# yl4579/StyleTTS2

Measured on AMD Instinct MI355X. Metric: audio-seconds/sec (RTF^-1) end-to-end, 10 s utterance batch, higher is better.
Workload: dtype f32 (convs/linears: f16 hi/lo split, 3 MFMA products, fp32 accumulate)

## Files before the change

include/st2.h:

```cpp
#ifndef ST2_H
#define ST2_H

#include <stdint.h>

#ifdef __cplusplus
extern "C" {
#endif

#define ST2_ABI_VERSION 23

int st2_abi_version(void);
const char* st2_last_error(void);
int st2_device_info(int dev, char* name, int cap);

#define ST2_STATUS_F16_RANGE 1
#define ST2_STATUS_LSTM_TIMEOUT 2
#define ST2_STATUS_DURATION_SUM 4
#define ST2_STATUS_LSTM_RECOVERED 8
#define ST2_STATUS_FRAME_CAPACITY 16
int st2_status(int clear);

enum st2_prologue {
  ST2_PRO_NONE = 0,
  ST2_PRO_LEAKY = 1,
  ST2_PRO_ADAIN_LEAKY = 2,
  ST2_PRO_ADAIN_SNAKE = 3,
  ST2_PRO_SNAKE = 4,
  ST2_PRO_COLNORM = 5
};
enum st2_epilogue_act {
  ST2_ACT_NONE = 0,
  ST2_ACT_GELU = 1,
  ST2_ACT_EXP_SIN = 2,
  ST2_ACT_TANH = 3,
  ST2_ACT_LEAKY = 4,
  ST2_ACT_GELU_TANH = 5
};

typedef struct st2_conv_desc {
  int32_t B, C_in, C_out, L_in, L_out, ks, dil, pad_left;
  const float* x; int64_t x_bs; int32_t x_cs;
  const float* wt; int32_t w_ld;
  const float* bias;
  float* y; int64_t y_bs; int32_t y_cs;
  int32_t pro;
  float slope;
  const float* stats;
  const float* gamma; const float* beta;
  int64_t gb_bs; int32_t gamma_plus_one;
  const float* alpha;
  const float* res;  int64_t res_bs;  int32_t res_cs;  int32_t res_shift;
  const float* res2; int64_t res2_bs; int32_t res2_cs;
  float div;
  int32_t act; int32_t act_split; float act_slope;
  const void* wq; int32_t wq_co_pad; int32_t wq_cin_pad;
  float x_scale;
  float out_scale;
  const float* w_row_scale;
  const void* xs; int32_t xs_cg; int32_t xs_lp; int32_t xs_halo;
  float* part; int32_t part_nt;
  int32_t part_cols;
  void* splitk_ws; int64_t splitk_ws_bytes;
  const int32_t* x_len; const int32_t* y_len;
} st2_conv_desc;

int st2_conv1d(const st2_conv_desc* d, void* stream);

int st2_conv1d_f16s(const st2_conv_desc* d, void* stream);
int64_t st2_conv1d_f16s_splitk_bytes(const st2_conv_desc* d);
int st2_conv1d_f16s_chunk(int ks);
int st2_conv1d_f16s_co_block(int C_out);
void st2_conv1d_f16s_set_variant(int variant);
void st2_conv1d_f16s_set_splitk(int max_slices, int min_chunks);
int st2_sizeof_conv_desc(void);

int st2_act_split(const float* x, int64_t x_bs, int32_t x_cs, int32_t B, int32_t C, int32_t L,
                  int32_t pro, float slope, const float* stats, const float* gamma, const float* beta, int64_t gb_bs,
                  int32_t gb_seg, int32_t gamma_plus_one, const float* alpha, float x_scale,
                  void* xs, int32_t xs_cg, int32_t Lp, int32_t halo, void* stream);
int st2_conv1d_xs(const st2_conv_desc* d, void* stream);
int st2_act_split_len(const float* x, int64_t x_bs, int32_t x_cs, int32_t B, int32_t C, int32_t L,
                      int32_t pro, float slope, const float* stats, const float* gamma, const float* beta, int64_t gb_bs,
                      int32_t gb_seg, int32_t gamma_plus_one, const float* alpha, float x_scale,
                      void* xs, int32_t xs_cg, int32_t Lp, int32_t halo, const int32_t* len, void* stream);
int st2_conv1d_xs_part_cols(const st2_conv_desc* d);
int st2_stats_finalize(const float* part, int32_t rows, int32_t nt, int32_t L, float eps, float* stats, int32_t cols, void* stream);
int st2_stats_finalize_len(const float* part, int32_t rows, int32_t nt, int32_t L, float eps, float* stats, int32_t cols,
                           const int32_t* len, int32_t len_div, void* stream);

int st2_conv1d_direct(const float* x, int64_t x_bs, int32_t x_cs,
                      const float* w, const float* bias,
                      float* y, int64_t y_bs, int32_t y_cs,
                      int32_t B, int32_t C_in, int32_t C_out, int32_t L_in, int32_t L_out,
                      int32_t ks, int32_t stride, int32_t pad, void* stream);
int st2_conv1d_direct_len(const float* x, int64_t x_bs, int32_t x_cs, const float* w, const float* bias,
                          float* y, int64_t y_bs, int32_t y_cs, int32_t B, int32_t C_in, int32_t C_out, int32_t L_in,
                          int32_t L_out, int32_t ks, int32_t stride, int32_t pad, const int32_t* x_len,
                          const int32_t* y_len, void* stream);

int st2_phase_split(const float* x, int64_t x_bs, int32_t x_cs, int32_t B, int32_t C, int32_t L_in,
                    int32_t stride, int32_t pad, float* xp, int64_t p_bs, int32_t p_cs, int32_t Lu, void* stream);

int st2_instnorm_stats(const float* x, int64_t x_bs, int32_t x_cs, int32_t B, int32_t C, int32_t L,
                       float eps, float* stats , void* stream);
int st2_instnorm_stats_len(const float* x, int64_t x_bs, int32_t x_cs, int32_t B, int32_t C, int32_t L,
                           float eps, float* stats, const int32_t* len, void* stream);

int st2_colnorm_stats(const float* x, int64_t x_bs, int32_t x_cs, int32_t B, int32_t C, int32_t L,
                      float eps, float* stats , void* stream);

int st2_style_fc(const float* s, int32_t B, int32_t K, const float* wt, const float* bias,
                 int32_t J, int32_t act, float* h, void* stream);

int st2_convt_interleave(const float* phases, int64_t p_bs, int32_t p_cs, int32_t Lq,
                         const float* bias, const float* add, int64_t a_bs, int32_t a_cs,
                         float* out, int64_t o_bs, int32_t o_cs,
                         int32_t B, int32_t C, int32_t stride, int32_t pad, int32_t L_raw,
                         int32_t reflect_left, void* stream);

int st2_convt_interleave_stats(const float* phases, int64_t p_bs, int32_t p_cs, int32_t Lq,
                               const float* bias, const float* add, int64_t a_bs, int32_t a_cs,
                               float* out, int64_t o_bs, int32_t o_cs,
                               int32_t B, int32_t C, int32_t stride, int32_t pad, int32_t L_raw,
                               int32_t reflect_left, float* part, int32_t part_nt, void* stream);
int st2_convt_interleave_stats_len(const float* phases, int64_t p_bs, int32_t p_cs, int32_t Lq,
                                   const float* bias, const float* add, int64_t a_bs, int32_t a_cs,
                                   float* out, int64_t o_bs, int32_t o_cs,
                                   int32_t B, int32_t C, int32_t stride, int32_t pad, int32_t L_raw,
                                   int32_t reflect_left, float* part, int32_t part_nt, const int32_t* q_len,
                                   const int32_t* out_len, void* stream);

int st2_adain_leaky_pool(const float* x, int64_t x_bs, int32_t x_cs,
                         const float* stats, const float* gamma, const float* beta, int64_t gb_bs,
                         float slope, const float* w, const float* bias,
                         float* y, int64_t y_bs, int32_t y_cs,
                         int32_t B, int32_t C, int32_t L, void* stream);
int st2_adain_leaky_pool_len(const float* x, int64_t x_bs, int32_t x_cs,
                             const float* stats, const float* gamma, const float* beta, int64_t gb_bs,
                             float slope, const float* w, const float* bias,
                             float* y, int64_t y_bs, int32_t y_cs,
                             int32_t B, int32_t C, int32_t L, const int32_t* len, void* stream);

int st2_har_source(const float* f0, int32_t B, int32_t F, int32_t U, int32_t H,
                   const float* noise, const float* lin_w, const float* lin_b,
                   float sine_amp, float noise_std, float voiced_threshold, float sample_rate,
                   float* phase_scratch, float* out, void* stream);
int st2_har_source_len(const float* f0, int32_t B, int32_t F, int32_t U, int32_t H,
                       const float* noise, const float* lin_w, const float* lin_b,
                       float sine_amp, float noise_std, float voiced_threshold, float sample_rate,
                       float* phase_scratch, float* out, const int32_t* f_len, void* stream);

int st2_stft_mag_phase(const float* x, int32_t B, int32_t L, int32_t n_fft, int32_t hop,
                       float* har, int64_t har_bs, int32_t har_cs, void* stream);
int st2_stft_mag_phase_len(const float* x, int32_t B, int32_t L, int32_t n_fft, int32_t hop,
                           float* har, int64_t har_bs, int32_t har_cs, const int32_t* len, void* stream);

int st2_istft(const float* sp, int64_t sp_bs, int32_t sp_cs, int32_t B, int32_t M,
              int32_t n_fft, int32_t hop, float* wave, int64_t wave_bs, void* stream);
int st2_istft_len(const float* sp, int64_t sp_bs, int32_t sp_cs, int32_t B, int32_t M,
                  int32_t n_fft, int32_t hop, float* wave, int64_t wave_bs, const int32_t* m_len, void* stream);
int st2_ragged_lengths(const int32_t* frames, int32_t B, int32_t T_max, int32_t n, const int32_t* coef, int32_t* out,
                       void* stream);

int st2_attention(const float* q, const float* k, const float* v, int64_t bs, int32_t cs,
                  float* o, int64_t o_bs, int32_t o_cs,
                  int32_t B, int32_t H, int32_t D, int32_t N, float scale, void* stream);

int st2_attention_keylen(const float* q, const float* k, const float* v, int64_t bs, int32_t cs,
                         float* o, int64_t o_bs, int32_t o_cs,
                         int32_t B, int32_t H, int32_t D, int32_t N, float scale, const int32_t* key_len, void* stream);

int st2_colnorm_apply(const float* x, int64_t x_bs, int32_t x_cs, const float* stats, const float* gamma,
                      const float* beta, int64_t gb_bs, int32_t gamma_plus_one, int32_t act, float slope,
                      const int32_t* len, float* y, int64_t y_bs, int32_t y_cs,
                      int32_t B, int32_t C, int32_t L, void* stream);

int st2_lstm_bidir(const float* G, int64_t g_bs, int32_t g_cs, const float* whh_t, const int32_t* lengths,
                   int32_t B, int32_t H, int32_t N, float* Y, int64_t y_bs, int32_t y_cs, void* stream);

int64_t st2_lstm_coop_scratch_bytes(int32_t B);
int st2_lstm_coop_set_exchange(int mode);
int st2_lstm_coop_set_spin_limit(int polls);
int st2_lstm_coop_set_block(int utterances);
int st2_lstm_bidir_coop(const float* G, int64_t g_bs, int32_t g_cs, const float* whh_t, const int32_t* lengths,
                        int32_t B, int32_t H, int32_t N, float* Y, int64_t y_bs, int32_t y_cs,
                        void* scratch, int64_t scratch_bytes, void* stream);
int st2_lstm_bidir_coop_recovering(const float* G, int64_t g_bs, int32_t g_cs, const float* whh_t, const int32_t* lengths,
                                   int32_t B, int32_t H, int32_t N, float* Y, int64_t y_bs, int32_t y_cs,
                                   void* scratch, int64_t scratch_bytes, void* stream);

int st2_add_chanvec(const float* x, int64_t x_bs, int32_t x_cs, const float* v, int64_t v_bs,
                    float* y, int64_t y_bs, int32_t y_cs, int32_t B, int32_t C, int32_t N, void* stream);
int st2_mean_tokens(const float* x, int64_t x_bs, int32_t x_cs, float* m, int64_t m_bs,
                    int32_t B, int32_t C, int32_t N, void* stream);
int st2_mean_tokens_len(const float* x, int64_t x_bs, int32_t x_cs, float* m, int64_t m_bs,
                        int32_t B, int32_t C, int32_t N, const int32_t* len, void* stream);
int st2_time_features(float t, const float* w, int32_t H2, int32_t B, float* out, void* stream);
int st2_tokens_to_channels(const float* e, int64_t e_bs, int32_t B, int32_t N, int32_t E, float* y, int64_t y_bs,
                           int32_t y_cs, void* stream);
int st2_broadcast_cols(const float* x, int64_t x_bs, float* y, int64_t y_bs, int32_t y_cs, int32_t B, int32_t C,
                       int32_t N, void* stream);
int st2_copy_ncl(const float* x, int64_t x_bs, int32_t x_cs, float* y, int64_t y_bs, int32_t y_cs, int32_t B, int32_t C,
                 int32_t L, void* stream);

int st2_embed_tokens(const int64_t* tokens, int32_t B, int32_t N, const float* table, int32_t V, int32_t E,
                     const float* add, const float* pos, const int32_t* len, float* y, int64_t y_bs, int32_t y_cs,
                     void* stream);
int st2_mask_tail(float* x, int64_t x_bs, int32_t x_cs, int32_t B, int32_t C, int32_t L, const int32_t* len, void* stream);

int st2_duration_head(const float* x, int64_t x_bs, int32_t x_cs, const float* w, const float* bias, int32_t B,
                      int32_t K, int32_t J, int32_t N, const int32_t* len, int32_t tail, int64_t* dur, float* dsum,
                      void* stream);
int st2_expand_by_durations(const float* x, int64_t x_bs, int32_t x_cs, const int64_t* dur, int32_t B, int32_t C,
                            int32_t N, int32_t T, int32_t shift, float* y, int64_t y_bs, int32_t y_cs, void* stream);
int st2_expand_by_durations_len(const float* x, int64_t x_bs, int32_t x_cs, const int64_t* dur, int32_t B, int32_t C,
                                int32_t N, int32_t T, int32_t shift, float* y, int64_t y_bs, int32_t y_cs, const int32_t* len,
                                void* stream);

int st2_frames_from_durations(const int64_t* dur, int32_t B, int32_t N, const int32_t* len, int32_t T_cap, int32_t* frames,
                              void* stream);

enum st2_pack_format { ST2_PACK_F32 = 0, ST2_PACK_S16 = 1 };
int st2_wave_pack(const float* wave, int64_t w_bs, const int32_t* frames, int32_t B, int32_t T_cap,
                  int32_t samples_per_frame, int32_t trim, int32_t fmt, void* out, int64_t out_capacity, int64_t* offsets,
                  void* stream);

int st2_stft_frames(const float* wave, int64_t w_bs, int32_t B, int32_t L, int32_t n_win, int32_t hop, int32_t shift,
                    float* frames, int64_t f_bs, int32_t f_cs, void* stream);
int st2_power_spectrum(const float* y, int64_t y_bs, int32_t y_cs, int32_t B, int32_t K, int32_t M, float* p,
                       int64_t p_bs, int32_t p_cs, void* stream);
int st2_log_norm(float* x, int64_t n, float eps, float mean, float stdv, void* stream);
int st2_dwconv3x3s2(const float* x, int64_t x_bs, int64_t x_hs, int32_t x_cs, const float* w, const float* bias,
                    int32_t B, int32_t C, int32_t H, int32_t W, float* y, int64_t y_bs, int64_t y_hs, int32_t y_cs,
                    void* stream);
int st2_avgpool2x2(const float* x, int64_t x_bs, int64_t x_hs, int32_t x_cs, int32_t B, int32_t C, int32_t H, int32_t W,
                   float* y, int64_t y_bs, int64_t y_hs, int32_t y_cs, void* stream);

int st2_axpbypcz(const float* x, float a, const float* y, float b, const float* z, float c,
                 float* out, int64_t n, void* stream);

typedef struct st2_engine st2_engine;

typedef struct st2_model_config {
  int32_t decoder_kind;
  int32_t dim_in;
  int32_t style_dim;
  int32_t upsample_initial_channel;
  int32_t n_upsamples;  int32_t upsample_rates[4];  int32_t upsample_kernel_sizes[4];
  int32_t n_resblock_kernels;  int32_t resblock_kernel_sizes[4];  int32_t resblock_dilations[4][3];
  int32_t gen_istft_n_fft, gen_istft_hop;
  int32_t multispeaker;
  int32_t dn_layers, dn_heads, dn_head_features, dn_multiplier;
  int32_t dn_channels;
  int32_t dn_embedding;
  int32_t dn_context_features;
  int32_t dn_max_length;
  int32_t pred_hidden;
  int32_t bert_layers;
  float bert_ln_eps;
} st2_model_config;

int st2_create(const st2_model_config* cfg, st2_engine** out);
int st2_destroy(st2_engine* e);
int st2_load_weights(st2_engine* e, const char* name, const float* data, const int64_t* shape, int32_t ndim);
int st2_finalize_weights(st2_engine* e, int32_t which);

typedef struct st2_decoder_taps {
  float* encode;
  float* front;
  float* har_source;
  float* har;
  float* stage[4];
  float* spec_phase;
} st2_decoder_taps;

int64_t st2_decoder_workspace_bytes(st2_engine* e, int32_t B, int32_t T);
int st2_decoder_forward(st2_engine* e, const float* asr, const float* f0, const float* n, const float* s,
                        const float* sine_noise, const float* har_inject, int32_t B, int32_t T, float* wave,
                        void* workspace, int64_t workspace_bytes, const st2_decoder_taps* taps, void* stream);
int st2_decoder_forward_ragged(st2_engine* e, const float* asr, const float* f0, const float* n, const float* s,
                               const float* sine_noise, const float* har_inject, const int32_t* frames, int32_t B,
                               int32_t T_max, float* wave, void* workspace, int64_t workspace_bytes,
                               const st2_decoder_taps* taps, void* stream);

#define ST2_SAMPLER_TABLE_COLS 11
int st2_sampler_table(int32_t steps, double sigma_min, double sigma_max, double rho, double sigma_data, double* table,
                      double* sigma0);
int64_t st2_sampler_workspace_bytes(st2_engine* e, int32_t B, int32_t N, int32_t steps, double embedding_scale);
int st2_sampler_run(st2_engine* e, const float* noise, const float* embedding, const float* features,
                    const float* step_noise, const int32_t* lengths, int32_t B, int32_t N, int32_t steps,
                    double embedding_scale, const double* table, double sigma0, float* out, void* workspace,
                    int64_t workspace_bytes, float* step_taps, void* stream);

int64_t st2_prosody_workspace_bytes(st2_engine* e, int32_t B, int32_t N, int32_t T);
int st2_prosody_forward(st2_engine* e, const float* d_cm, const float* t_en, const int64_t* durations, const float* s,
                        int32_t B, int32_t N, int32_t T, int32_t shift, float* asr, float* f0, float* n, void* workspace,
                        int64_t workspace_bytes, void* stream);
int st2_prosody_forward_ragged(st2_engine* e, const float* d_cm, const float* t_en, const int64_t* durations,
                               const float* s, const int32_t* frames, int32_t B, int32_t N, int32_t T_max, int32_t shift,
                               float* asr, float* f0, float* n, void* workspace, int64_t workspace_bytes, void* stream);

int64_t st2_text_workspace_bytes(st2_engine* e, int32_t B, int32_t N);
int st2_text_forward(st2_engine* e, const int64_t* tokens, const int32_t* lengths, int32_t B, int32_t N, float* t_en,
                     void* workspace, int64_t workspace_bytes, void* stream);

int64_t st2_duration_workspace_bytes(st2_engine* e, int32_t B, int32_t N);
int st2_duration_forward(st2_engine* e, const float* d_en, const float* s, const int32_t* lengths, int32_t B, int32_t N,
                         int32_t tail, float* d_cm, int64_t* durations, void* workspace, int64_t workspace_bytes,
                         void* stream);

int64_t st2_bert_workspace_bytes(st2_engine* e, int32_t B, int32_t N);
int st2_bert_forward(st2_engine* e, const int64_t* tokens, const int32_t* lengths, int32_t B, int32_t N, float* hidden_cm,
                     void* workspace, int64_t workspace_bytes, void* stream);

typedef struct st2_front_args {
  const int64_t* tokens;
  const int32_t* lengths;
  const float* noise;
  const float* step_noise;
  const float* ref_s;
  const float* s_prev;
  int32_t B, N, steps;
  int32_t tail;
  double embedding_scale;
  const double* table;
  double sigma0;
  double alpha, beta, t;
  float* t_en;
  float* d_cm;
  float* s;
  float* ref;
  float* s_pred_out;
  int64_t* durations;
  int32_t carry;
} st2_front_args;
int st2_sizeof_front_args(void);
int64_t st2_front_workspace_bytes(st2_engine* e, const st2_front_args* a);
int st2_front_forward(st2_engine* e, const st2_front_args* a, void* workspace, int64_t workspace_bytes, void* stream);

int64_t st2_style_workspace_bytes(st2_engine* e, int32_t which, int32_t B, int32_t n_mels, int32_t T);
int st2_style_forward(st2_engine* e, int32_t which, const float* mel, int32_t B, int32_t n_mels, int32_t T, float* style,
                      void* workspace, int64_t workspace_bytes, void* stream);

int st2_conv_timing(int enable);
int st2_conv_timing_read(double* rows, int32_t cap_rows);

int st2_conv_tune(int mode);
int st2_conv_tune_set(int32_t ks, int32_t C_in, int32_t C_out, int32_t L_out, int32_t B, int32_t variant);
int st2_conv_tune_read(double* rows, int32_t cap_rows);

#define ST2_HEADROOM_COLS 12
int st2_debug_headroom(int enable);
int st2_debug_headroom_read(double* rows, int32_t cap_rows);

#define ST2_CALIBRATION_COLS 5
int st2_calibrate(st2_engine* e, int32_t margin_bits, int32_t* n_clamped);
int st2_calibration_read(st2_engine* e, double* rows, int32_t cap_rows);
int st2_calibration_site_name(st2_engine* e, int32_t site, char* name, int32_t cap);
int st2_calibration_write(st2_engine* e, const float* scales, int32_t n);
float st2_calibration_scale(float max_abs, int32_t margin_bits);

int st2_probe_box(char* json, int32_t cap, int32_t level);

int st2_probe_cu_health(char* json, int32_t cap, uint32_t* mask_out, int32_t mask_words, int32_t* n_excluded);

int st2_probe_mfma_stream(int32_t kind, int32_t workgroups, int32_t iters, void* stream);

int st2_stream_create_cu_mask(const uint32_t* mask, int32_t n_words, void** stream);
int st2_stream_destroy(void* stream);

enum st2_backend_slot {
  ST2_BE_CONV1D_F16S = 0, ST2_BE_CONV1D_XS, ST2_BE_ACT_SPLIT, ST2_BE_STATS_FINALIZE, ST2_BE_CONV1D_DIRECT,
  ST2_BE_PHASE_SPLIT, ST2_BE_INSTNORM_STATS, ST2_BE_COLNORM_STATS, ST2_BE_STYLE_FC, ST2_BE_CONVT_INTERLEAVE_STATS,
  ST2_BE_ADAIN_LEAKY_POOL, ST2_BE_HAR_SOURCE, ST2_BE_STFT_MAG_PHASE, ST2_BE_ISTFT, ST2_BE_ATTENTION_KEYLEN,
  ST2_BE_ADD_CHANVEC, ST2_BE_MEAN_TOKENS_LEN, ST2_BE_AXPBYPCZ, ST2_BE_TIME_FEATURES, ST2_BE_TOKENS_TO_CHANNELS,
  ST2_BE_BROADCAST_COLS, ST2_BE_COPY_NCL, ST2_BE_EXPAND_BY_DURATIONS,
  ST2_BE_LSTM_BIDIR,
  ST2_BE_COLNORM_APPLY, ST2_BE_DURATION_HEAD, ST2_BE_MASK_TAIL, ST2_BE_EMBED_TOKENS, ST2_BE_DWCONV3X3S2, ST2_BE_AVGPOOL2X2,
  ST2_BE_DEV_ALLOC,
  ST2_BE_DEV_FREE,
  ST2_BE_UPLOAD,
  ST2_BACKEND_ENTRIES_V22,
  ST2_BE_ACT_SPLIT_LEN = ST2_BACKEND_ENTRIES_V22, ST2_BE_INSTNORM_STATS_LEN, ST2_BE_STATS_FINALIZE_LEN,
  ST2_BE_CONV1D_DIRECT_LEN, ST2_BE_ADAIN_LEAKY_POOL_LEN, ST2_BE_CONVT_INTERLEAVE_STATS_LEN, ST2_BE_HAR_SOURCE_LEN,
  ST2_BE_STFT_MAG_PHASE_LEN, ST2_BE_ISTFT_LEN, ST2_BE_RAGGED_LENGTHS, ST2_BE_EXPAND_BY_DURATIONS_LEN,
  ST2_BACKEND_ENTRIES
};
// ... 7 lines not shown
```

styletts2_amd/_lib.py:

```python
import ctypes as C
import os

import torch

_HERE = os.path.dirname(os.path.abspath(__file__))
LIB_PATH = os.path.join(_HERE, "libst2_hip.so")
ABI_VERSION = 23
HEADROOM_COLS, CALIBRATION_COLS = 12, 5

f32p = C.c_void_p

PRO_NONE, PRO_LEAKY, PRO_ADAIN_LEAKY, PRO_ADAIN_SNAKE, PRO_SNAKE, PRO_COLNORM = range(6)
STATUS_F16_RANGE, STATUS_LSTM_TIMEOUT, STATUS_DURATION_SUM, STATUS_LSTM_RECOVERED = 1, 2, 4, 8
STATUS_FRAME_CAPACITY = 16
PACK_F32, PACK_S16 = 0, 1
ACT_NONE, ACT_GELU, ACT_EXP_SIN, ACT_TANH, ACT_LEAKY, ACT_GELU_TANH = range(6)


class ConvDesc(C.Structure):
    _fields_ = [
        ("B", C.c_int32), ("C_in", C.c_int32), ("C_out", C.c_int32), ("L_in", C.c_int32),
        ("L_out", C.c_int32), ("ks", C.c_int32), ("dil", C.c_int32), ("pad_left", C.c_int32),
        ("x", f32p), ("x_bs", C.c_int64), ("x_cs", C.c_int32),
        ("wt", f32p), ("w_ld", C.c_int32),
        ("bias", f32p),
        ("y", f32p), ("y_bs", C.c_int64), ("y_cs", C.c_int32),
        ("pro", C.c_int32),
        ("slope", C.c_float),
        ("stats", f32p),
        ("gamma", f32p), ("beta", f32p),
        ("gb_bs", C.c_int64), ("gamma_plus_one", C.c_int32),
        ("alpha", f32p),
        ("res", f32p), ("res_bs", C.c_int64), ("res_cs", C.c_int32), ("res_shift", C.c_int32),
        ("res2", f32p), ("res2_bs", C.c_int64), ("res2_cs", C.c_int32),
        ("div", C.c_float),
        ("act", C.c_int32), ("act_split", C.c_int32), ("act_slope", C.c_float),
        ("wq", f32p), ("wq_co_pad", C.c_int32), ("wq_cin_pad", C.c_int32),
        ("x_scale", C.c_float), ("out_scale", C.c_float),
        ("w_row_scale", f32p),
        ("xs", f32p), ("xs_cg", C.c_int32), ("xs_lp", C.c_int32), ("xs_halo", C.c_int32),
        ("part", f32p), ("part_nt", C.c_int32), ("part_cols", C.c_int32),
        ("splitk_ws", f32p), ("splitk_ws_bytes", C.c_int64),
        ("x_len", C.c_void_p), ("y_len", C.c_void_p),
    ]


class ModelConfig(C.Structure):
    _fields_ = [
        ("decoder_kind", C.c_int32), ("dim_in", C.c_int32), ("style_dim", C.c_int32),
        ("upsample_initial_channel", C.c_int32),
        ("n_upsamples", C.c_int32), ("upsample_rates", C.c_int32 * 4), ("upsample_kernel_sizes", C.c_int32 * 4),
        ("n_resblock_kernels", C.c_int32), ("resblock_kernel_sizes", C.c_int32 * 4),
        ("resblock_dilations", (C.c_int32 * 3) * 4),
        ("gen_istft_n_fft", C.c_int32), ("gen_istft_hop", C.c_int32),
        ("multispeaker", C.c_int32),
        ("dn_layers", C.c_int32), ("dn_heads", C.c_int32), ("dn_head_features", C.c_int32),
        ("dn_multiplier", C.c_int32), ("dn_channels", C.c_int32), ("dn_embedding", C.c_int32),
        ("dn_context_features", C.c_int32), ("dn_max_length", C.c_int32),
        ("pred_hidden", C.c_int32),
        ("bert_layers", C.c_int32), ("bert_ln_eps", C.c_float),
    ]


class FrontArgs(C.Structure):
    _fields_ = [("tokens", C.c_void_p), ("lengths", C.c_void_p), ("noise", C.c_void_p), ("step_noise", C.c_void_p),
                ("ref_s", C.c_void_p), ("s_prev", C.c_void_p),
                ("B", C.c_int32), ("N", C.c_int32), ("steps", C.c_int32), ("tail", C.c_int32),
                ("embedding_scale", C.c_double), ("table", C.POINTER(C.c_double)), ("sigma0", C.c_double),
                ("alpha", C.c_double), ("beta", C.c_double), ("t", C.c_double),
                ("t_en", C.c_void_p), ("d_cm", C.c_void_p), ("s", C.c_void_p), ("ref", C.c_void_p),
                ("s_pred_out", C.c_void_p), ("durations", C.c_void_p), ("carry", C.c_int32)]


class DecoderTaps(C.Structure):
    _fields_ = [("encode", f32p), ("front", f32p), ("har_source", f32p), ("har", f32p), ("stage", f32p * 4),
                ("spec_phase", f32p)]


SAMPLER_TABLE_COLS = 11
BACKEND_SLOTS = ["conv1d_f16s", "conv1d_xs", "act_split", "stats_finalize", "conv1d_direct", "phase_split",
                 "instnorm_stats", "colnorm_stats", "style_fc", "convt_interleave_stats", "adain_leaky_pool",
                 "har_source", "stft_mag_phase", "istft", "attention_keylen", "add_chanvec", "mean_tokens_len",
                 "axpbypcz", "time_features", "tokens_to_channels", "broadcast_cols", "copy_ncl", "expand_by_durations",
                 "lstm_bidir", "colnorm_apply", "duration_head", "mask_tail", "embed_tokens", "dwconv3x3s2",
                 "avgpool2x2", "dev_alloc", "dev_free", "upload"]
BACKEND_SLOTS_RAGGED = ["act_split_len", "instnorm_stats_len", "stats_finalize_len", "conv1d_direct_len",
                        "adain_leaky_pool_len", "convt_interleave_stats_len", "har_source_len", "stft_mag_phase_len",
                        "istft_len", "ragged_lengths", "expand_by_durations_len"]

_SIGNATURES = {
    "st2_abi_version": (C.c_int, []),
    "st2_last_error": (C.c_char_p, []),
    "st2_device_info": (C.c_int, [C.c_int, C.c_char_p, C.c_int]),
    "st2_sizeof_conv_desc": (C.c_int, []),
    "st2_status": (C.c_int, [C.c_int]),
    "st2_conv1d": (C.c_int, [C.POINTER(ConvDesc), C.c_void_p]),
    "st2_conv1d_f16s": (C.c_int, [C.POINTER(ConvDesc), C.c_void_p]),
    "st2_conv1d_f16s_splitk_bytes": (C.c_int64, [C.POINTER(ConvDesc)]),
    "st2_conv1d_f16s_chunk": (C.c_int, [C.c_int]),
    "st2_conv1d_f16s_co_block": (C.c_int, [C.c_int]),
    "st2_conv1d_f16s_set_variant": (None, [C.c_int]),
    "st2_conv1d_xs": (C.c_int, [C.POINTER(ConvDesc), C.c_void_p]),
    "st2_act_split": (C.c_int, [f32p, C.c_int64, C.c_int32, C.c_int32, C.c_int32, C.c_int32, C.c_int32, C.c_float,
                                f32p, f32p, f32p, C.c_int64, C.c_int32, C.c_int32, f32p, C.c_float, f32p, C.c_int32,
                                C.c_int32, C.c_int32, C.c_void_p]),
    "st2_stats_finalize": (C.c_int, [f32p, C.c_int32, C.c_int32, C.c_int32, C.c_float, f32p, C.c_int32, C.c_void_p]),
    "st2_conv1d_direct": (C.c_int, [f32p, C.c_int64, C.c_int32, f32p, f32p, f32p, C.c_int64, C.c_int32,
                                    C.c_int32, C.c_int32, C.c_int32, C.c_int32, C.c_int32, C.c_int32, C.c_int32,
                                    C.c_int32, C.c_void_p]),
    "st2_phase_split": (C.c_int, [f32p, C.c_int64, C.c_int32, C.c_int32, C.c_int32, C.c_int32, C.c_int32, C.c_int32,
                                  f32p, C.c_int64, C.c_int32, C.c_int32, C.c_void_p]),
    "st2_instnorm_stats": (C.c_int, [f32p, C.c_int64, C.c_int32, C.c_int32, C.c_int32, C.c_int32, C.c_float, f32p,
                                     C.c_void_p]),
    "st2_colnorm_stats": (C.c_int, [f32p, C.c_int64, C.c_int32, C.c_int32, C.c_int32, C.c_int32, C.c_float, f32p,
                                    C.c_void_p]),
    "st2_style_fc": (C.c_int, [f32p, C.c_int32, C.c_int32, f32p, f32p, C.c_int32, C.c_int32, f32p, C.c_void_p]),
    "st2_convt_interleave": (C.c_int, [f32p, C.c_int64, C.c_int32, C.c_int32, f32p, f32p, C.c_int64, C.c_int32,
                                       f32p, C.c_int64, C.c_int32, C.c_int32, C.c_int32, C.c_int32, C.c_int32,
                                       C.c_int32, C.c_int32, C.c_void_p]),
    "st2_convt_interleave_stats": (C.c_int, [f32p, C.c_int64, C.c_int32, C.c_int32, f32p, f32p, C.c_int64, C.c_int32,
                                             f32p, C.c_int64, C.c_int32, C.c_int32, C.c_int32, C.c_int32, C.c_int32,
                                             C.c_int32, C.c_int32, f32p, C.c_int32, C.c_void_p]),
    "st2_adain_leaky_pool": (C.c_int, [f32p, C.c_int64, C.c_int32, f32p, f32p, f32p, C.c_int64, C.c_float, f32p,
                                       f32p, f32p, C.c_int64, C.c_int32, C.c_int32, C.c_int32, C.c_int32,
                                       C.c_void_p]),
    "st2_har_source": (C.c_int, [f32p, C.c_int32, C.c_int32, C.c_int32, C.c_int32, f32p, f32p, f32p, C.c_float,
                                 C.c_float, C.c_float, C.c_float, f32p, f32p, C.c_void_p]),
    "st2_stft_mag_phase": (C.c_int, [f32p, C.c_int32, C.c_int32, C.c_int32, C.c_int32, f32p, C.c_int64, C.c_int32,
                                     C.c_void_p]),
    "st2_istft": (C.c_int, [f32p, C.c_int64, C.c_int32, C.c_int32, C.c_int32, C.c_int32, C.c_int32, f32p, C.c_int64,
                            C.c_void_p]),
    "st2_attention": (C.c_int, [f32p, f32p, f32p, C.c_int64, C.c_int32, f32p, C.c_int64, C.c_int32, C.c_int32,
                                C.c_int32, C.c_int32, C.c_int32, C.c_float, C.c_void_p]),
    "st2_attention_keylen": (C.c_int, [f32p, f32p, f32p, C.c_int64, C.c_int32, f32p, C.c_int64, C.c_int32, C.c_int32,
                                       C.c_int32, C.c_int32, C.c_int32, C.c_float, C.c_void_p, C.c_void_p]),
    "st2_colnorm_apply": (C.c_int, [f32p, C.c_int64, C.c_int32, f32p, f32p, f32p, C.c_int64, C.c_int32, C.c_int32,
                                    C.c_float, C.c_void_p, f32p, C.c_int64, C.c_int32, C.c_int32, C.c_int32, C.c_int32,
                                    C.c_void_p]),
    "st2_lstm_bidir": (C.c_int, [f32p, C.c_int64, C.c_int32, f32p, C.c_void_p, C.c_int32, C.c_int32, C.c_int32, f32p,
                                 C.c_int64, C.c_int32, C.c_void_p]),
    "st2_lstm_coop_scratch_bytes": (C.c_int64, [C.c_int32]),
    "st2_lstm_coop_set_exchange": (C.c_int, [C.c_int]),
    "st2_lstm_coop_set_spin_limit": (C.c_int, [C.c_int]),
    "st2_lstm_coop_set_block": (C.c_int, [C.c_int]),
    "st2_lstm_bidir_coop": (C.c_int, [f32p, C.c_int64, C.c_int32, f32p, C.c_void_p, C.c_int32, C.c_int32, C.c_int32,
                                      f32p, C.c_int64, C.c_int32, C.c_void_p, C.c_int64, C.c_void_p]),
    "st2_lstm_bidir_coop_recovering": (C.c_int, [f32p, C.c_int64, C.c_int32, f32p, C.c_void_p, C.c_int32, C.c_int32, C.c_int32,
                                                 f32p, C.c_int64, C.c_int32, C.c_void_p, C.c_int64, C.c_void_p]),
    "st2_add_chanvec": (C.c_int, [f32p, C.c_int64, C.c_int32, f32p, C.c_int64, f32p, C.c_int64, C.c_int32,
                                  C.c_int32, C.c_int32, C.c_int32, C.c_void_p]),
    "st2_mean_tokens": (C.c_int, [f32p, C.c_int64, C.c_int32, f32p, C.c_int64, C.c_int32, C.c_int32, C.c_int32,
                                  C.c_void_p]),
    "st2_mean_tokens_len": (C.c_int, [f32p, C.c_int64, C.c_int32, f32p, C.c_int64, C.c_int32, C.c_int32, C.c_int32,
                                      C.c_void_p, C.c_void_p]),
    "st2_time_features": (C.c_int, [C.c_float, f32p, C.c_int32, C.c_int32, f32p, C.c_void_p]),
    "st2_tokens_to_channels": (C.c_int, [f32p, C.c_int64, C.c_int32, C.c_int32, C.c_int32, f32p, C.c_int64, C.c_int32,
                                         C.c_void_p]),
    "st2_broadcast_cols": (C.c_int, [f32p, C.c_int64, f32p, C.c_int64, C.c_int32, C.c_int32, C.c_int32, C.c_int32,
                                     C.c_void_p]),
    "st2_copy_ncl": (C.c_int, [f32p, C.c_int64, C.c_int32, f32p, C.c_int64, C.c_int32, C.c_int32, C.c_int32, C.c_int32,
                               C.c_void_p]),
    "st2_duration_head": (C.c_int, [f32p, C.c_int64, C.c_int32, f32p, f32p, C.c_int32, C.c_int32, C.c_int32, C.c_int32,
                                    C.c_void_p, C.c_int32, C.c_void_p, f32p, C.c_void_p]),
    "st2_expand_by_durations": (C.c_int, [f32p, C.c_int64, C.c_int32, C.c_void_p, C.c_int32, C.c_int32, C.c_int32,
                                          C.c_int32, C.c_int32, f32p, C.c_int64, C.c_int32, C.c_void_p]),
    "st2_create": (C.c_int, [C.POINTER(ModelConfig), C.POINTER(C.c_void_p)]),
    "st2_destroy": (C.c_int, [C.c_void_p]),
    "st2_load_weights": (C.c_int, [C.c_void_p, C.c_char_p, C.c_void_p, C.POINTER(C.c_int64), C.c_int32]),
    "st2_finalize_weights": (C.c_int, [C.c_void_p, C.c_int32]),
    "st2_decoder_workspace_bytes": (C.c_int64, [C.c_void_p, C.c_int32, C.c_int32]),
    "st2_decoder_forward": (C.c_int, [C.c_void_p, f32p, f32p, f32p, f32p, f32p, f32p, C.c_int32, C.c_int32, f32p,
                                      C.c_void_p, C.c_int64, C.POINTER(DecoderTaps), C.c_void_p]),
    "st2_embed_tokens": (C.c_int, [C.c_void_p, C.c_int32, C.c_int32, f32p, C.c_int32, C.c_int32, f32p, f32p, C.c_void_p, f32p,
                                   C.c_int64, C.c_int32, C.c_void_p]),
    "st2_bert_workspace_bytes": (C.c_int64, [C.c_void_p, C.c_int32, C.c_int32]),
    "st2_bert_forward": (C.c_int, [C.c_void_p, C.c_void_p, C.c_void_p, C.c_int32, C.c_int32, f32p, C.c_void_p, C.c_int64,
                                   C.c_void_p]),
    "st2_style_workspace_bytes": (C.c_int64, [C.c_void_p, C.c_int32, C.c_int32, C.c_int32, C.c_int32]),
    "st2_style_forward": (C.c_int, [C.c_void_p, C.c_int32, f32p, C.c_int32, C.c_int32, C.c_int32, f32p, C.c_void_p, C.c_int64,
                                    C.c_void_p]),
    "st2_sizeof_front_args": (C.c_int, []),
    "st2_front_workspace_bytes": (C.c_int64, [C.c_void_p, C.POINTER(FrontArgs)]),
    "st2_front_forward": (C.c_int, [C.c_void_p, C.POINTER(FrontArgs), C.c_void_p, C.c_int64, C.c_void_p]),
    "st2_text_workspace_bytes": (C.c_int64, [C.c_void_p, C.c_int32, C.c_int32]),
    "st2_text_forward": (C.c_int, [C.c_void_p, C.c_void_p, C.c_void_p, C.c_int32, C.c_int32, f32p, C.c_void_p, C.c_int64,
                                   C.c_void_p]),
    "st2_mask_tail": (C.c_int, [f32p, C.c_int64, C.c_int32, C.c_int32, C.c_int32, C.c_int32, C.c_void_p, C.c_void_p]),
    "st2_duration_workspace_bytes": (C.c_int64, [C.c_void_p, C.c_int32, C.c_int32]),
    "st2_duration_forward": (C.c_int, [C.c_void_p, f32p, f32p, C.c_void_p, C.c_int32, C.c_int32, C.c_int32, f32p,
                                       C.c_void_p, C.c_void_p, C.c_int64, C.c_void_p]),
    "st2_decoder_forward_ragged": (C.c_int, [C.c_void_p, f32p, f32p, f32p, f32p, f32p, f32p, C.c_void_p, C.c_int32,
                                             C.c_int32, f32p, C.c_void_p, C.c_int64, C.c_void_p, C.c_void_p]),
    "st2_prosody_forward_ragged": (C.c_int, [C.c_void_p, f32p, f32p, C.c_void_p, f32p, C.c_void_p, C.c_int32, C.c_int32,
                                             C.c_int32, C.c_int32, f32p, f32p, f32p, C.c_void_p, C.c_int64, C.c_void_p]),
    "st2_act_split_len": (C.c_int, [f32p, C.c_int64, C.c_int32, C.c_int32, C.c_int32, C.c_int32, C.c_int32, C.c_float,
                                    f32p, f32p, f32p, C.c_int64, C.c_int32, C.c_int32, f32p, C.c_float, f32p, C.c_int32,
                                    C.c_int32, C.c_int32, C.c_void_p, C.c_void_p]),
    "st2_stats_finalize_len": (C.c_int, [f32p, C.c_int32, C.c_int32, C.c_int32, C.c_float, f32p, C.c_int32, C.c_void_p,
                                         C.c_int32, C.c_void_p]),
    "st2_instnorm_stats_len": (C.c_int, [f32p, C.c_int64, C.c_int32, C.c_int32, C.c_int32, C.c_int32, C.c_float, f32p,
                                         C.c_void_p, C.c_void_p]),
    "st2_conv1d_direct_len": (C.c_int, [f32p, C.c_int64, C.c_int32, f32p, f32p, f32p, C.c_int64, C.c_int32, C.c_int32,
                                        C.c_int32, C.c_int32, C.c_int32, C.c_int32, C.c_int32, C.c_int32, C.c_int32,
                                        C.c_void_p, C.c_void_p, C.c_void_p]),
    "st2_convt_interleave_stats_len": (C.c_int, [f32p, C.c_int64, C.c_int32, C.c_int32, f32p, f32p, C.c_int64, C.c_int32,
                                                 f32p, C.c_int64, C.c_int32, C.c_int32, C.c_int32, C.c_int32, C.c_int32,
                                                 C.c_int32, C.c_int32, f32p, C.c_int32, C.c_void_p, C.c_void_p,
                                                 C.c_void_p]),
    "st2_adain_leaky_pool_len": (C.c_int, [f32p, C.c_int64, C.c_int32, f32p, f32p, f32p, C.c_int64, C.c_float, f32p,
                                           f32p, f32p, C.c_int64, C.c_int32, C.c_int32, C.c_int32, C.c_int32, C.c_void_p,
                                           C.c_void_p]),
    "st2_har_source_len": (C.c_int, [f32p, C.c_int32, C.c_int32, C.c_int32, C.c_int32, f32p, f32p, f32p, C.c_float,
                                     C.c_float, C.c_float, C.c_float, f32p, f32p, C.c_void_p, C.c_void_p]),
    "st2_stft_mag_phase_len": (C.c_int, [f32p, C.c_int32, C.c_int32, C.c_int32, C.c_int32, f32p, C.c_int64, C.c_int32,
                                         C.c_void_p, C.c_void_p]),
    "st2_istft_len": (C.c_int, [f32p, C.c_int64, C.c_int32, C.c_int32, C.c_int32, C.c_int32, C.c_int32, f32p, C.c_int64,
                                C.c_void_p, C.c_void_p]),
    "st2_expand_by_durations_len": (C.c_int, [f32p, C.c_int64, C.c_int32, C.c_void_p, C.c_int32, C.c_int32, C.c_int32,
                                              C.c_int32, C.c_int32, f32p, C.c_int64, C.c_int32, C.c_void_p, C.c_void_p]),
    "st2_ragged_lengths": (C.c_int, [C.c_void_p, C.c_int32, C.c_int32, C.c_int32, C.POINTER(C.c_int32), C.c_void_p,
                                     C.c_void_p]),
    "st2_frames_from_durations": (C.c_int, [C.c_void_p, C.c_int32, C.c_int32, C.c_void_p, C.c_int32, C.c_void_p, C.c_void_p]),
    "st2_wave_pack": (C.c_int, [f32p, C.c_int64, C.c_void_p, C.c_int32, C.c_int32, C.c_int32, C.c_int32, C.c_int32, C.c_void_p,
                                C.c_int64, C.c_void_p, C.c_void_p]),
    "st2_prosody_workspace_bytes": (C.c_int64, [C.c_void_p, C.c_int32, C.c_int32, C.c_int32]),
    "st2_prosody_forward": (C.c_int, [C.c_void_p, f32p, f32p, C.c_void_p, f32p, C.c_int32, C.c_int32, C.c_int32, C.c_int32,
                                      f32p, f32p, f32p, C.c_void_p, C.c_int64, C.c_void_p]),
    "st2_sampler_table": (C.c_int, [C.c_int32, C.c_double, C.c_double, C.c_double, C.c_double, C.POINTER(C.c_double),
                                    C.POINTER(C.c_double)]),
    "st2_sampler_workspace_bytes": (C.c_int64, [C.c_void_p, C.c_int32, C.c_int32, C.c_int32, C.c_double]),
    "st2_sampler_run": (C.c_int, [C.c_void_p, f32p, f32p, f32p, f32p, C.c_void_p, C.c_int32, C.c_int32, C.c_int32,
                                  C.c_double, C.POINTER(C.c_double), C.c_double, f32p, C.c_void_p, C.c_int64, f32p,
                                  C.c_void_p]),
    "st2_conv_timing": (C.c_int, [C.c_int]),
    "st2_conv_timing_read": (C.c_int, [C.POINTER(C.c_double), C.c_int32]),
    "st2_conv_tune": (C.c_int, [C.c_int]),
    "st2_conv_tune_set": (C.c_int, [C.c_int32, C.c_int32, C.c_int32, C.c_int32, C.c_int32, C.c_int32]),
    "st2_conv_tune_read": (C.c_int, [C.POINTER(C.c_double), C.c_int32]),
    "st2_probe_box": (C.c_int, [C.c_char_p, C.c_int32, C.c_int32]),
    "st2_probe_cu_health": (C.c_int, [C.c_char_p, C.c_int32, C.POINTER(C.c_uint32), C.c_int32, C.POINTER(C.c_int32)]),
    "st2_probe_mfma_stream": (C.c_int, [C.c_int32, C.c_int32, C.c_int32, C.c_void_p]),
    "st2_debug_headroom": (C.c_int, [C.c_int]),
    "st2_debug_headroom_read": (C.c_int, [C.POINTER(C.c_double), C.c_int32]),
    "st2_conv1d_xs_part_cols": (C.c_int, [C.POINTER(ConvDesc)]),
    "st2_conv1d_f16s_set_splitk": (None, [C.c_int, C.c_int]),
    "st2_calibrate": (C.c_int, [C.c_void_p, C.c_int32, C.POINTER(C.c_int32)]),
    "st2_calibration_read": (C.c_int, [C.c_void_p, C.POINTER(C.c_double), C.c_int32]),
    "st2_calibration_site_name": (C.c_int, [C.c_void_p, C.c_int32, C.c_char_p, C.c_int32]),
    "st2_calibration_write": (C.c_int, [C.c_void_p, C.POINTER(C.c_float), C.c_int32]),
    "st2_calibration_scale": (C.c_float, [C.c_float, C.c_int32]),
    "st2_stream_create_cu_mask": (C.c_int, [C.POINTER(C.c_uint32), C.c_int32, C.POINTER(C.c_void_p)]),
    "st2_stream_destroy": (C.c_int, [C.c_void_p]),
    "st2_debug_set_backend": (C.c_int, [C.POINTER(C.c_void_p), C.c_int32]),
    "st2_stft_frames": (C.c_int, [f32p, C.c_int64, C.c_int32, C.c_int32, C.c_int32, C.c_int32, C.c_int32, f32p,
                                  C.c_int64, C.c_int32, C.c_void_p]),
    "st2_power_spectrum": (C.c_int, [f32p, C.c_int64, C.c_int32, C.c_int32, C.c_int32, C.c_int32, f32p, C.c_int64,
                                     C.c_int32, C.c_void_p]),
    "st2_log_norm": (C.c_int, [f32p, C.c_int64, C.c_float, C.c_float, C.c_float, C.c_void_p]),
    "st2_dwconv3x3s2": (C.c_int, [f32p, C.c_int64, C.c_int64, C.c_int32, f32p, f32p, C.c_int32, C.c_int32, C.c_int32,
                                  C.c_int32, f32p, C.c_int64, C.c_int64, C.c_int32, C.c_void_p]),
    "st2_avgpool2x2": (C.c_int, [f32p, C.c_int64, C.c_int64, C.c_int32, C.c_int32, C.c_int32, C.c_int32, C.c_int32, f32p,
                                 C.c_int64, C.c_int64, C.c_int32, C.c_void_p]),
    "st2_axpbypcz": (C.c_int, [f32p, C.c_float, f32p, C.c_float, f32p, C.c_float, f32p, C.c_int64, C.c_void_p]),
}

EXPORTS = tuple(_SIGNATURES)
_lib = None


class St2Error(RuntimeError):
    pass


def load():
    global _lib
    if _lib is not None:
        return _lib
    if not os.path.exists(LIB_PATH):
        raise St2Error("libst2_hip.so is not built (%s missing). Run `python -m styletts2_amd._build`; "
                       "there is no CPU fallback." % LIB_PATH)
    try:
        lib = C.CDLL(LIB_PATH)
    except OSError as e:
        raise St2Error("cannot load %s: %s" % (LIB_PATH, e)) from e
    for name, (res, args) in _SIGNATURES.items():
        try:
            fn = getattr(lib, name)
        except AttributeError as e:
            raise St2Error("libst2_hip.so does not export %s" % name) from e
        fn.restype = res
        fn.argtypes = args
    if lib.st2_abi_version() != ABI_VERSION:
        raise St2Error("ABI mismatch: library %d, binding %d" % (lib.st2_abi_version(), ABI_VERSION))
    if lib.st2_sizeof_conv_desc() != C.sizeof(ConvDesc):
        raise St2Error("st2_conv_desc layout mismatch: library %d B, binding %d B"
                       % (lib.st2_sizeof_conv_desc(), C.sizeof(ConvDesc)))
    if lib.st2_sizeof_front_args() != C.sizeof(FrontArgs):
        raise St2Error("st2_front_args layout mismatch: library %d B, binding %d B"
                       % (lib.st2_sizeof_front_args(), C.sizeof(FrontArgs)))
    _lib = lib
    return lib


def check(status, what):
    if status != 0:
        msg = load().st2_last_error()
        raise St2Error("%s failed: %s" % (what, msg.decode() if msg else "unknown error"))
```

styletts2_amd/csrc/st2_actsplit.hip:

```cpp
#include "st2_common.h"
#include "st2_act.h"
#include <algorithm>
#include <cstring>
#include <type_traits>
#include <vector>

namespace {

struct ActArgs {
  const float* x; int64_t x_bs; int x_cs;
  int C, L;
  float slope;
  const float* stats; const float* gamma; const float* beta; int64_t gb_bs; int gb_seg; int gamma_plus_one;
  const float* alpha;
  float x_scale;
  st2_h8* xs; int xs_cg, Lp, halo;
  const int32_t* len;
  int* status;
};

#ifndef ST2_ACT_NT
#define ST2_ACT_NT 3
#endif
template <int PRO>
__global__ __launch_bounds__(256) void act_split_kernel(const ActArgs a) {
  const int pos = blockIdx.x * 256 + threadIdx.x;
  if (pos >= a.Lp) return;
  const int cg = blockIdx.y;
  const int b = blockIdx.z;
  const int l = pos - a.halo;
  const int Lb = a.len ? min(a.len[b], a.L) : a.L;
  const bool lok = l >= 0 && l < Lb;
  const int lc = min(max(l, 0), a.L - 1);
  const float* xb = a.x + (int64_t)b * a.x_bs + lc;
  float v[8];
#pragma unroll
  for (int e = 0; e < 8; ++e) {
    const int ci = min(cg * 8 + e, a.C - 1);
#if ST2_ACT_NT & 1
    v[e] = __builtin_nontemporal_load(&xb[(int64_t)ci * a.x_cs]);
#else
    v[e] = xb[(int64_t)ci * a.x_cs];
#endif
  }
  float cmean = 0.f, crstd = 1.f;
  if constexpr (PRO == ST2_PRO_COLNORM) {
    const float* st = a.stats + ((int64_t)b * a.L + lc) * 2;
    cmean = st[0];
    crstd = st[1];
  }
  st2_h8 hi, lo;
  bool sat = false;
#pragma unroll
  for (int e = 0; e < 8; ++e) {
    const int ci = cg * 8 + e;
    const int cc = min(ci, a.C - 1);
    float u = v[e];
    if constexpr (PRO == ST2_PRO_LEAKY) {
      u = leaky(u, a.slope);
    } else if constexpr (PRO == ST2_PRO_ADAIN_LEAKY || PRO == ST2_PRO_ADAIN_SNAKE) {
      const float* st = a.stats + ((int64_t)b * a.C + cc) * 2;
      const float g = 1.0f + a.gamma[(int64_t)b * a.gb_bs + cc];
      const float bt = a.beta[(int64_t)b * a.gb_bs + cc];
      float w = (u - st[0]) * st[1];
      w = g * w + bt;
      if constexpr (PRO == ST2_PRO_ADAIN_LEAKY) {
        u = leaky(w, a.slope);
      } else {
        const float al = a.alpha[cc];
        u = snake(w, al, 1.0f / al);
      }
    } else if constexpr (PRO == ST2_PRO_SNAKE) {
      const float al = a.alpha[cc];
      u = snake(u, al, 1.0f / al);
    } else if constexpr (PRO == ST2_PRO_COLNORM) {
      const int64_t row = a.gb_seg > 0 ? (int64_t)(lc / a.gb_seg) : (int64_t)b;
      const float g0 = a.gamma[row * a.gb_bs + cc];
      const float g = a.gamma_plus_one ? 1.0f + g0 : g0;
      const float bt = a.beta[row * a.gb_bs + cc];
      const float w = (u - cmean) * crstd;
      u = w * g + bt;
    }
    u = (lok && ci < a.C) ? u * a.x_scale : 0.f;
    const float uc = st2_clamp_f16(u);
    sat |= uc != u;
    const _Float16 h = (_Float16)uc;
    hi[e] = h;
    lo[e] = (_Float16)(uc - (float)h);
  }
  if (__any(sat) && (threadIdx.x & 63) == 0) st2_raise_status(a.status, ST2_STATUS_F16_RANGE);
  const int64_t plane = (int64_t)a.xs_cg * a.Lp;
  st2_h8* dst = a.xs + ((int64_t)b * 2 * a.xs_cg + cg) * a.Lp + pos;
#if ST2_ACT_NT & 2
  __builtin_nontemporal_store(hi, &dst[0]);
  __builtin_nontemporal_store(lo, &dst[plane]);
#else
  dst[0] = hi;
  dst[plane] = lo;
#endif
}

__global__ __launch_bounds__(256) void stats_finalize_kernel(const float* __restrict__ part, int rows, int nt, int L_max,
                                                             float eps, float* __restrict__ stats, int cols,
                                                             const int32_t* __restrict__ len, int len_div) {
  const int lane = threadIdx.x & 63;
  const int row = blockIdx.x * 4 + (threadIdx.x >> 6);
  if (row >= rows) return;
  const int L = len ? min(max(len[row / len_div], 1), L_max) : L_max;
  const float2* p = reinterpret_cast<const float2*>(part) + (int64_t)row * nt;
  const float* sh = part + (int64_t)rows * nt * 2 + (int64_t)row * nt;
  const int ns = min(nt, (L + cols - 1) / cols);
  double wsum = 0.0;
  for (int i = lane; i < ns; i += 64) {
    const int n = min(cols, L - i * cols);
    wsum += (double)n * (double)sh[i] + (double)p[i].x;
  }
  wsum = st2_wave_sum(wsum);
  const double mean = __shfl(wsum, 0, 64) / (double)L;
  double m2 = 0.0;
  for (int i = lane; i < ns; i += 64) {
    const int n = min(cols, L - i * cols);
    const double s1 = (double)p[i].x, s2 = (double)p[i].y;
    const double mi = (double)sh[i] + s1 / (double)n;
    m2 += (s2 - s1 * s1 / (double)n) + (double)n * (mi - mean) * (mi - mean);
  }
  m2 = st2_wave_sum(m2);
  if (lane == 0) {
    double var = m2 / (double)L;
    if (var < 0.0) var = 0.0;
    stats[(int64_t)row * 2 + 0] = (float)mean;
    stats[(int64_t)row * 2 + 1] = (float)(1.0 / sqrt(var + (double)eps));
  }
}

struct HeadroomSums {
  unsigned max_bits, pad;
  double su2, se2, ssub;
};
__global__ __launch_bounds__(256) void xs_probe_kernel(const st2_h8* __restrict__ xs, int64_t slots_per_item, int64_t item_stride,
                                                       HeadroomSums* out) {
  const st2_h8* hi_p = xs + (int64_t)blockIdx.y * item_stride;
  const st2_h8* lo_p = hi_p + slots_per_item;
  float m = 0.f;
  double su2 = 0.0, se2 = 0.0, ssub = 0.0;
  for (int64_t i = (int64_t)blockIdx.x * 256 + threadIdx.x; i < slots_per_item; i += (int64_t)gridDim.x * 256) {
    const st2_h8 h = hi_p[i], l = lo_p[i];
#pragma unroll
    for (int e = 0; e < 8; ++e) {
      const float hf = (float)h[e], lf = (float)l[e];
      m = fmaxf(m, fabsf(hf));
      if (hf == 0.f && lf == 0.f) continue;
      const float u = hf + lf;
      const float al = fabsf(lf);
      const bool sub = al < 6.103515625e-05f;
      int ex = -14;
      if (!sub) {
        (void)frexpf(al, &ex);
        ex -= 1;
      }
      const float ulp = ldexpf(1.0f, ex - 10);
      su2 += (double)u * u;
      se2 += (double)ulp * ulp * (1.0 / 12.0);
      if (sub) ssub += (double)u * u;
    }
  }
  for (int off = 32; off > 0; off >>= 1) m = fmaxf(m, __shfl_down(m, off, 64));
  su2 = st2_wave_sum(su2);
  se2 = st2_wave_sum(se2);
  ssub = st2_wave_sum(ssub);
  if ((threadIdx.x & 63) == 0) {
    atomicMax(&out->max_bits, __float_as_uint(m));
    atomicAdd(&out->su2, su2);
    atomicAdd(&out->se2, se2);
    atomicAdd(&out->ssub, ssub);
  }
}

struct HeadroomRecord {
  int kind, pro, B, C, L;
  float x_scale;
  const void* engine;
  int site;
};
bool g_headroom = false;
std::vector<HeadroomRecord> g_hr;
HeadroomSums* g_hr_dev = nullptr;
constexpr int HR_CAP = 4096;
void* g_hr_scratch = nullptr;
size_t g_hr_scratch_bytes = 0;
thread_local const void* t_site_engine = nullptr;
thread_local int t_site = -1;

void headroom_record(int kind, const ActArgs& a, int B, hipStream_t s) {
  if ((int)g_hr.size() >= HR_CAP || !g_hr_dev) return;
  hipStreamCaptureStatus cs = hipStreamCaptureStatusNone;
  if (hipStreamIsCapturing(s, &cs) != hipSuccess || cs != hipStreamCaptureStatusNone) {
    (void)hipGetLastError();
    return;
  }
  const int64_t plane = (int64_t)a.xs_cg * a.Lp;
  hipLaunchKernelGGL(xs_probe_kernel, dim3((unsigned)std::min<int64_t>((plane + 255) / 256, 1024), B), dim3(256), 0, s, a.xs, plane,
                     2 * plane, g_hr_dev + g_hr.size());
  g_hr.push_back({kind, 0, B, a.C, a.L, a.x_scale, t_site_engine, t_site});
}

template <int PRO>
void launch_act(const ActArgs& a, int B, hipStream_t s) {
  hipLaunchKernelGGL((act_split_kernel<PRO>), dim3(st2_cdiv(a.Lp, 256), a.xs_cg, B), dim3(256), 0, s, a);
}

}

extern "C" int st2_act_split(const float* x, int64_t x_bs, int32_t x_cs, int32_t B, int32_t C, int32_t L, int32_t pro,
                             float slope, const float* stats, const float* gamma, const float* beta, int64_t gb_bs,
                             int32_t gb_seg, int32_t gamma_plus_one, const float* alpha, float x_scale, void* xs, int32_t xs_cg,
                             int32_t Lp, int32_t halo, void* stream) {
  return st2_act_split_len(x, x_bs, x_cs, B, C, L, pro, slope, stats, gamma, beta, gb_bs, gb_seg, gamma_plus_one, alpha, x_scale,
                           xs, xs_cg, Lp, halo, nullptr, stream);
}

extern "C" int st2_act_split_len(const float* x, int64_t x_bs, int32_t x_cs, int32_t B, int32_t C, int32_t L, int32_t pro,
                                 float slope, const float* stats, const float* gamma, const float* beta, int64_t gb_bs,
                                 int32_t gb_seg, int32_t gamma_plus_one, const float* alpha, float x_scale, void* xs,
                                 int32_t xs_cg, int32_t Lp, int32_t halo, const int32_t* len, void* stream) {
  ST2_REQUIRE(x && xs && B > 0 && C > 0 && L > 0, "st2_act_split: bad arguments");
  ST2_REQUIRE(B <= 65535 && xs_cg <= 65535, "st2_act_split: grid too large");
  ST2_REQUIRE(xs_cg * 8 >= C, "st2_act_split: xs_cg=%d groups cannot hold C=%d channels", xs_cg, C);
  ST2_REQUIRE(halo >= 0 && Lp >= L + halo, "st2_act_split: Lp=%d too small for L=%d + halo=%d", Lp, L, halo);
  ST2_REQUIRE((reinterpret_cast<uintptr_t>(xs) & 15) == 0, "st2_act_split: xs must be 16-byte aligned");
  ST2_REQUIRE(pro >= ST2_PRO_NONE && pro <= ST2_PRO_COLNORM, "st2_act_split: prologue %d not supported", pro);
  if (pro == ST2_PRO_ADAIN_LEAKY || pro == ST2_PRO_ADAIN_SNAKE || pro == ST2_PRO_COLNORM)
    ST2_REQUIRE(stats && gamma && beta, "st2_act_split: prologue %d needs stats/gamma/beta", pro);
  if (pro == ST2_PRO_ADAIN_SNAKE || pro == ST2_PRO_SNAKE) ST2_REQUIRE(alpha, "st2_act_split: snake needs alpha");
  ST2_REQUIRE(x_scale > 0.f, "st2_act_split: x_scale must be set");
  ST2_REQUIRE(gb_seg >= 0 && (gb_seg == 0 || pro == ST2_PRO_COLNORM), "st2_act_split: gb_seg=%d is for ST2_PRO_COLNORM", gb_seg);
  ActArgs a;
  a.x = x; a.x_bs = x_bs; a.x_cs = x_cs; a.C = C; a.L = L; a.slope = slope;
  a.stats = stats; a.gamma = gamma; a.beta = beta; a.gb_bs = gb_bs; a.gb_seg = gb_seg; a.gamma_plus_one = gamma_plus_one;
  a.alpha = alpha; a.x_scale = x_scale;
  a.xs = reinterpret_cast<st2_h8*>(xs); a.xs_cg = xs_cg; a.Lp = Lp; a.halo = halo;
  a.len = len;
  ST2_REQUIRE(!len || pro != ST2_PRO_COLNORM, "st2_act_split_len: per-row lengths are not defined for ST2_PRO_COLNORM");
  a.status = st2_status_device_ptr();
  hipStream_t s = reinterpret_cast<hipStream_t>(stream);
  switch (pro) {
    case ST2_PRO_LEAKY: launch_act<ST2_PRO_LEAKY>(a, B, s); break;
    case ST2_PRO_ADAIN_LEAKY: launch_act<ST2_PRO_ADAIN_LEAKY>(a, B, s); break;
    case ST2_PRO_ADAIN_SNAKE: launch_act<ST2_PRO_ADAIN_SNAKE>(a, B, s); break;
    case ST2_PRO_SNAKE: launch_act<ST2_PRO_SNAKE>(a, B, s); break;
    case ST2_PRO_COLNORM: launch_act<ST2_PRO_COLNORM>(a, B, s); break;
    default: launch_act<ST2_PRO_NONE>(a, B, s); break;
  }
  ST2_CHECK_LAUNCH("st2_act_split");
  if (g_headroom) {
    headroom_record(0, a, B, s);
    if (!g_hr.empty()) g_hr.back().pro = pro;
  }
  return 0;
}

int st2_headroom_of_fused_conv(const st2_conv_desc& d, hipStream_t s) {
  if (!g_headroom || !d.x) return 0;
  {
    hipStreamCaptureStatus cs = hipStreamCaptureStatusNone;
    if (hipStreamIsCapturing(s, &cs) != hipSuccess || cs != hipStreamCaptureStatusNone) {
      (void)hipGetLastError();
      return 0;
    }
  }
  const int cg = (d.C_in + 31) / 32 * 4, halo = 0;
  const int Lp = (d.L_in + 7) / 8 * 8;
  const size_t bytes = (size_t)d.B * 2 * cg * Lp * 16;
  if (bytes > g_hr_scratch_bytes) {
    if (g_hr_scratch) (void)hipFree(g_hr_scratch);
    g_hr_scratch = nullptr;
    g_hr_scratch_bytes = 0;
    if (hipMalloc(&g_hr_scratch, bytes) != hipSuccess) {
      (void)hipGetLastError();
      return 0;
    }
    g_hr_scratch_bytes = bytes;
  }
  const size_t before = g_hr.size();
  const int rc = st2_act_split(d.x, d.x_bs, d.x_cs, d.B, d.C_in, d.L_in, d.pro, d.slope, d.stats, d.gamma, d.beta, d.gb_bs, 0,
                               d.gamma_plus_one, d.alpha, d.x_scale, g_hr_scratch, cg, Lp, halo, s);
  if (rc == 0 && g_hr.size() == before + 1) g_hr.back().kind = 1;
  return rc;
}

extern "C" int st2_debug_headroom(int enable) {
  if (enable) {
    g_hr.clear();
    if (!g_hr_dev && hipMalloc(&g_hr_dev, HR_CAP * sizeof(HeadroomSums)) != hipSuccess) {
      (void)hipGetLastError();
      g_hr_dev = nullptr;
      st2_set_error("st2_debug_headroom: cannot allocate the record buffer");
      return 1;
    }
    if (hipMemset(g_hr_dev, 0, HR_CAP * sizeof(HeadroomSums)) != hipSuccess) {
      st2_set_error("st2_debug_headroom: %s", hipGetErrorString(hipGetLastError()));
      return 1;
    }
  } else if (g_hr_scratch) {
    (void)hipDeviceSynchronize();
    (void)hipFree(g_hr_scratch);
    g_hr_scratch = nullptr;
    g_hr_scratch_bytes = 0;
  }
  g_headroom = enable != 0;
  return 0;
}

void st2_headroom_set_site(const void* engine, int site) {
  t_site_engine = engine;
  t_site = site;
}

extern "C" int st2_debug_headroom_read(double* rows, int32_t cap_rows) {
  ST2_REQUIRE(!g_headroom, "st2_debug_headroom_read: stop the recording first (st2_debug_headroom(0))");
  const int n = (int)g_hr.size();
  if (!rows || n == 0) return n;
  std::vector<HeadroomSums> h(n);
  if (hipDeviceSynchronize() != hipSuccess ||
      hipMemcpy(h.data(), g_hr_dev, n * sizeof(HeadroomSums), hipMemcpyDeviceToHost) != hipSuccess) {
    st2_set_error("st2_debug_headroom_read: %s", hipGetErrorString(hipGetLastError()));
    return -1;
  }
  for (int i = 0; i < n && i < cap_rows; ++i) {
    float m;
    memcpy(&m, &h[i].max_bits, 4);
    double* r = rows + (int64_t)i * ST2_HEADROOM_COLS;
    r[0] = g_hr[i].kind; r[1] = g_hr[i].pro; r[2] = g_hr[i].B; r[3] = g_hr[i].C; r[4] = g_hr[i].L; r[5] = g_hr[i].x_scale;
    r[6] = m; r[7] = m / 65504.0;
    r[8] = h[i].su2 > 0.0 ? sqrt(h[i].se2 / h[i].su2) : 0.0;
    r[9] = h[i].su2 > 0.0 ? h[i].ssub / h[i].su2 : 0.0;
    r[10] = g_hr[i].site;
    r[11] = (double)(uintptr_t)g_hr[i].engine;
  }
  return n;
}

extern "C" int st2_stats_finalize(const float* part, int32_t rows, int32_t nt, int32_t L, float eps, float* stats, int32_t cols,
                                  void* stream) {
  return st2_stats_finalize_len(part, rows, nt, L, eps, stats, cols, nullptr, 1, stream);
}

extern "C" int st2_stats_finalize_len(const float* part, int32_t rows, int32_t nt, int32_t L, float eps, float* stats,
                                      int32_t cols, const int32_t* len, int32_t len_div, void* stream) {
  ST2_REQUIRE(part && stats && rows > 0 && nt > 0 && L > 0, "st2_stats_finalize: bad arguments");
  ST2_REQUIRE(!len || (len_div > 0 && rows % len_div == 0), "st2_stats_finalize_len: len_div=%d does not divide rows=%d", len_div,
              rows);
  ST2_REQUIRE(cols > 0 && (int64_t)nt * cols >= L, "st2_stats_finalize: %d slots of %d columns do not cover L=%d", nt, cols, L);
  ST2_REQUIRE((reinterpret_cast<uintptr_t>(part) & 7) == 0, "st2_stats_finalize: part must be 8-byte aligned");
  hipStream_t s = reinterpret_cast<hipStream_t>(stream);
  hipLaunchKernelGGL(stats_finalize_kernel, dim3(st2_cdiv(rows, 4)), dim3(256), 0, s, part, rows, nt, L, eps, stats, cols, len,
                     len_div);
  ST2_CHECK_LAUNCH("st2_stats_finalize");
  return 0;
}
```

styletts2_amd/csrc/st2_common.h:

```cpp
#pragma once
#include <hip/hip_runtime.h>
#include <stdint.h>
#include <atomic>
#include "st2.h"

void st2_set_error(const char* fmt, ...);
int st2_stream_cu_count(void* stream);
void st2_headroom_set_site(const void* engine, int site);
int* st2_status_device_ptr();

__device__ __forceinline__ void st2_raise_status(int* status, int bit) {
  if (status) __hip_atomic_store(status + (bit == ST2_STATUS_F16_RANGE ? 0 : (bit == ST2_STATUS_LSTM_TIMEOUT ? 1 :
                                           (bit == ST2_STATUS_DURATION_SUM ? 2 :
                                            (bit == ST2_STATUS_LSTM_RECOVERED ? 3 : 4)))), bit,
                                 __ATOMIC_RELAXED, __HIP_MEMORY_SCOPE_SYSTEM);
}

#define ST2_REQUIRE(cond, ...)            \
  do {                                    \
    if (!(cond)) {                        \
      st2_set_error(__VA_ARGS__);         \
      return 1;                           \
    }                                     \
  } while (0)

#define ST2_CHECK_LAUNCH(name)                                   \
  do {                                                           \
    hipError_t e__ = hipGetLastError();                          \
    if (e__ != hipSuccess) {                                     \
      st2_set_error("%s: %s", name, hipGetErrorString(e__));     \
      return 1;                                                  \
    }                                                            \
  } while (0)

static inline int st2_cdiv(int64_t a, int64_t b) { return (int)((a + b - 1) / b); }

template <class F>
static inline void st2_once_per_device(std::atomic<uint64_t>& mask, F&& set_attr) {
  int dev = 0;
  const bool known = hipGetDevice(&dev) == hipSuccess && dev >= 0 && dev < 64;
  if (known && (mask.load(std::memory_order_acquire) & (1ull << dev))) return;
  set_attr();
  if (known) mask.fetch_or(1ull << dev, std::memory_order_release);
}

__device__ __forceinline__ double st2_wave_sum(double v) {
#pragma unroll
  for (int off = 32; off > 0; off >>= 1) v += __shfl_down(v, off, 64);
  return v;
}
__device__ __forceinline__ float st2_wave_sum(float v) {
#pragma unroll
  for (int off = 32; off > 0; off >>= 1) v += __shfl_down(v, off, 64);
  return v;
}
```

styletts2_amd/csrc/st2_engine.hip:

```cpp
#include <math.h>
#include <stdio.h>
#include <string.h>

#include <algorithm>
#include <cmath>
#include <string>
#include <unordered_map>
#include <vector>

#include "st2_common.h"

namespace {

struct Backend {
  decltype(&st2_conv1d_f16s) conv1d_f16s;
  decltype(&st2_conv1d_xs) conv1d_xs;
  decltype(&st2_act_split) act_split;
  decltype(&st2_stats_finalize) stats_finalize;
  decltype(&st2_conv1d_direct) conv1d_direct;
  decltype(&st2_phase_split) phase_split;
  decltype(&st2_instnorm_stats) instnorm_stats;
  decltype(&st2_colnorm_stats) colnorm_stats;
  decltype(&st2_style_fc) style_fc;
  decltype(&st2_convt_interleave_stats) convt_interleave_stats;
// ... 431 lines not shown
      return -1;
    }
    return blob.add_f32(t->data);
  }
  int64_t lin_t(const std::string& name, int64_t out = -1, int64_t in = -1) {
    const HostTensor* t = get(name, {out, in});
    if (!t) return -1;
    if (t->shape.size() != 2) { fail(name + " (2-D expected)"); return -1; }
    const int64_t O = t->shape[0], I = t->shape[1];
    std::vector<float> v((size_t)(O * I));
    for (int64_t o = 0; o < O; ++o)
      for (int64_t i = 0; i < I; ++i) v[(size_t)(i * O + o)] = t->data[(size_t)(o * I + i)];
    return blob.add_f32(v);
  }
  SplitW conv_w(const std::string& name, int co = -1, int ci = -1, int ks = -1) {
    const HostTensor* t = get(name, {co, ci, ks});
    if (!t) return SplitW();
    if (t->shape.size() < 2) { fail(name + " has shape " + shape_str(t->shape) + ", a conv / linear weight is at least 2-D"); return SplitW(); }
    const int C_out = (int)t->shape[0], C_in = (int)t->shape[1], k = t->shape.size() > 2 ? (int)t->shape[2] : 1;
    return pack_split(blob, name, t->data.data(), C_out, C_in, k);
  }
  PConv conv(const std::string& prefix, bool bias = true, int co = -1, int ci = -1, int ks = -1) {
    PConv c;
    c.w = conv_w(prefix + ".weight", co, ci, ks);
    c.c_out = c.w.C_out;
    c.ks = c.w.ks;
    if (bias && has(prefix + ".bias")) c.bias = vec(prefix + ".bias", c.w.C_out > 0 ? c.w.C_out : -1);
    return c;
  }
};

struct Bank {
  std::vector<const HostTensor*> ws, bs;
  std::vector<int> chans;
  std::vector<std::string> names;
  int J = 0;
  int add(Packer& pk, const std::string& prefix, int channels) {
    names.push_back(prefix + ".fc.weight");
    ws.push_back(pk.get(prefix + ".fc.weight"));
    bs.push_back(pk.get(prefix + ".fc.bias"));
    chans.push_back(channels);
    const int off = J;
    J += 2 * channels;
    return off;
  }
  void pack(Packer& pk, int style_dim, int64_t* wt_off, int64_t* b_off) {
    std::vector<float> wt((size_t)style_dim * J), b((size_t)J);
    int off = 0;
    for (size_t m = 0; m < ws.size(); ++m) {
      const int n = 2 * chans[m];
      if (!ws[m] || !bs[m]) return;
      if (ws[m]->numel() != (int64_t)n * style_dim || bs[m]->numel() != n) {
        pk.fail("AdaIN fc " + names[m] + " has shape " + Packer::shape_str(ws[m]->shape) + " / bias " + Packer::shape_str(bs[m]->shape) +
                ", the model configuration needs [" + std::to_string(n) + ", " + std::to_string(style_dim) + "]");
        return;
      }
      for (int j = 0; j < n; ++j) {
        for (int k = 0; k < style_dim; ++k) wt[(size_t)k * J + off + j] = ws[m]->data[(size_t)j * style_dim + k];
        b[(size_t)off + j] = bs[m]->data[(size_t)j];
      }
      off += n;
    }
    *wt_off = pk.blob.add_f32(wt);
    *b_off = pk.blob.add_f32(b);
  }
};

PResBlock1 pack_resblock1(Packer& pk, const std::string& prefix, int channels, int ks, const int* dil) {
  PResBlock1 r;
  r.channels = channels;
  r.ks = ks;
  for (int i = 0; i < 3; ++i) {
    const std::string si = std::to_string(i);
    r.dil[i] = dil[i];
    r.c1[i] = pk.conv(prefix + ".convs1." + si, true, channels, channels, ks);
    r.c2[i] = pk.conv(prefix + ".convs2." + si, true, channels, channels, ks);
    r.a1[i] = pk.vec(prefix + ".alpha1." + si, channels);
    r.a2[i] = pk.vec(prefix + ".alpha2." + si, channels);
  }
  return r;
}

PAdainResBlk pack_adain_resblk(Packer& pk, const std::string& prefix, int dim_in, int dim_out, bool upsample) {
  PAdainResBlk r;
  r.dim_in = dim_in; r.dim_out = dim_out; r.upsample = upsample; r.learned_sc = dim_in != dim_out;
  r.conv1 = pk.conv(prefix + ".conv1", true, dim_out, dim_in, 3);
  r.conv2 = pk.conv(prefix + ".conv2", true, dim_out, dim_out, 3);
  if (r.learned_sc) r.sc = pk.conv(prefix + ".conv1x1", false, dim_out, dim_in, 1);
  if (upsample) {
    r.pool_w = pk.vec(prefix + ".pool.weight", (int64_t)dim_in * 3);
    r.pool_b = pk.vec(prefix + ".pool.bias", dim_in);
  }
  return r;
}

int prod_from(const int32_t* v, int lo, int hi) {
  int p = 1;
  for (int i = lo; i < hi; ++i) p *= v[i];
  return p;
}

int pack_decoder(st2_engine& e, Blob& blob, std::string* err) {
  const st2_model_config& cfg = e.cfg;
  Packer pk{e, blob};
  PDecoder d;
  Bank bank;
  const std::string D = "decoder.";
  const int sty = cfg.style_dim, Cin = cfg.dim_in;
  d.encode = pack_adain_resblk(pk, D + "encode", Cin + 2, 1024, false);
  d.encode.n1 = bank.add(pk, D + "encode.norm1", Cin + 2);
  d.encode.n2 = bank.add(pk, D + "encode.norm2", 1024);
  for (int i = 0; i < 4; ++i) {
    const std::string p = D + "decode." + std::to_string(i);
    const bool up = i == 3;
    d.decode[i] = pack_adain_resblk(pk, p, 1024 + 2 + 64, up ? 512 : 1024, up);
    d.decode[i].n1 = bank.add(pk, p + ".norm1", 1024 + 2 + 64);
    d.decode[i].n2 = bank.add(pk, p + ".norm2", up ? 512 : 1024);
  }
  d.f0_w = pk.vec(D + "F0_conv.weight", 3); d.f0_b = pk.vec(D + "F0_conv.bias", 1);
  d.n_w = pk.vec(D + "N_conv.weight", 3);   d.n_b = pk.vec(D + "N_conv.bias", 1);
  d.asr_res = pk.conv(D + "asr_res.0", true, 64, Cin, 1);

  PGenerator& g = d.gen;
  const std::string G = D + "generator.";
  const int nu = cfg.n_upsamples, nk = cfg.n_resblock_kernels;
  const bool ist = cfg.decoder_kind == 0;
  const int c0 = cfg.upsample_initial_channel;
  g.lin_w = pk.vec(G + "m_source.l_linear.weight", 9);
  g.lin_b = pk.vec(G + "m_source.l_linear.bias", 1);
  static const int dil135[3] = {1, 3, 5};
  for (int i = 0; i < nu; ++i) g.channels.push_back(c0 >> (i + 1));
  for (int i = 0; i < nu; ++i) {
    const bool last = i + 1 == nu;
    PResBlock1 r = pack_resblock1(pk, G + "noise_res." + std::to_string(i), g.channels[i], last ? 11 : 7, dil135);
    g.noise_res.push_back(r);
  }
  for (int i = 0; i < nu; ++i)
    for (int k = 0; k < nk; ++k) {
      PResBlock1 r = pack_resblock1(pk, G + "resblocks." + std::to_string(i * nk + k), g.channels[i],
                                    cfg.resblock_kernel_sizes[k], cfg.resblock_dilations[k]);
      g.resblocks.push_back(r);
    }
  for (auto* list : {&g.noise_res, &g.resblocks}) {
    const std::string pre = list == &g.noise_res ? G + "noise_res." : G + "resblocks.";
    for (size_t i = 0; i < list->size(); ++i) {
      PResBlock1& r = (*list)[i];
      for (int j = 0; j < 3; ++j) r.ad1[j] = bank.add(pk, pre + std::to_string(i) + ".adain1." + std::to_string(j), r.channels);
      for (int j = 0; j < 3; ++j) r.ad2[j] = bank.add(pk, pre + std::to_string(i) + ".adain2." + std::to_string(j), r.channels);
    }
  }
  if (pk.ok) bank.pack(pk, sty, &d.bank_wt, &d.bank_b);
  d.J = bank.J;
  for (int i = 0; i < nu; ++i) {
    const int stride_f0 = i + 1 < nu ? prod_from(cfg.upsample_rates, i + 1, nu) : 1;
    const HostTensor* w = pk.get(G + "noise_convs." + std::to_string(i) + ".weight", {g.channels[i], -1, -1});
    g.noise_stride.push_back(stride_f0);
    if (w && w->shape.size() != 3) { pk.fail(G + "noise_convs." + std::to_string(i) + ".weight must be 3-D"); w = nullptr; }
    if (w) {
      const int C_out = (int)w->shape[0], C_in = (int)w->shape[1], K = (int)w->shape[2];
      if (stride_f0 > 1) {
        if (K != 2 * stride_f0) { *err = "noise_convs kernel must be 2*stride"; return 1; }
        std::vector<float> wp = polyphase_strided(w->data.data(), C_out, C_in, stride_f0);
        g.noise_wt.push_back(pack_split(blob, G + "noise_convs." + std::to_string(i) + ".weight", wp.data(), C_out, C_in * stride_f0, 2));
      } else {
        g.noise_wt.push_back(pack_split(blob, G + "noise_convs." + std::to_string(i) + ".weight", w->data.data(), C_out, C_in, K));
      }
    } else {
      g.noise_wt.push_back(SplitW());
    }
    g.noise_b.push_back(pk.vec(G + "noise_convs." + std::to_string(i) + ".bias", g.channels[i]));
  }
  for (int i = 0; i < nu; ++i) {
    const int u = cfg.upsample_rates[i];
    const HostTensor* w = pk.get(G + "ups." + std::to_string(i) + ".weight", {c0 >> i, c0 >> (i + 1), -1});
    if (w && w->shape.size() != 3) { pk.fail(G + "ups." + std::to_string(i) + ".weight must be 3-D"); w = nullptr; }
    if (w) {
      const int C_in = (int)w->shape[0], C_out = (int)w->shape[1], K = (int)w->shape[2];
      if (K != 2 * u) { *err = "ups kernel must be 2*stride"; return 1; }
      std::vector<float> wp = polyphase_convt(w->data.data(), C_in, C_out, u);
      g.ups_wt.push_back(pack_split(blob, G + "ups." + std::to_string(i) + ".weight", wp.data(), u * C_out, C_in, 2));
    } else {
      g.ups_wt.push_back(SplitW());
    }
    g.ups_b.push_back(pk.vec(G + "ups." + std::to_string(i) + ".bias", c0 >> (i + 1)));
  }
  g.post = pk.conv(G + "conv_post", true, ist ? cfg.gen_istft_n_fft + 2 : 1, g.channels.back(), 7);
  if (!ist)
    for (int i = 0; i <= nu; ++i) g.alphas.push_back(pk.vec(G + "alphas." + std::to_string(i), c0 >> i));
  if (!pk.ok) {
    *err = "decoder weights (missing or malformed): " + pk.missing;
    return 1;
  }
  d.ready = true;
  e.dec = d;
  return 0;
}

int pack_denoiser(st2_engine& e, Blob& blob, std::string* err) {
  const st2_model_config& cfg = e.cfg;
  Packer pk{e, blob};
  PDenoiser d;
  const std::string N = "denoiser.";
  d.features = cfg.dn_channels + cfg.dn_embedding;
  d.time_w = pk.vec(N + "to_time.0.0.weights");
  d.time_lin = pk.lin_t(N + "to_time.0.1.weight"); d.time_b = pk.vec(N + "to_time.0.1.bias");
  d.map0 = pk.lin_t(N + "to_mapping.0.weight");    d.map0_b = pk.vec(N + "to_mapping.0.bias");
  d.map2 = pk.lin_t(N + "to_mapping.2.weight");    d.map2_b = pk.vec(N + "to_mapping.2.bias");
  const int F = d.features;
  if (cfg.multispeaker) {
    d.feat = pk.lin_t(N + "to_features.0.weight"); d.feat_b = pk.vec(N + "to_features.0.bias");
    const int Fc = cfg.dn_context_features, J = cfg.dn_layers * 4 * F;
    std::vector<float> wt((size_t)Fc * J), b((size_t)J);
    int off = 0;
    for (int i = 0; i < cfg.dn_layers; ++i)
      for (const char* nm : {".attention.norm", ".attention.norm_context"}) {
        const HostTensor* w = pk.get(N + "blocks." + std::to_string(i) + nm + ".fc.weight", {2 * F, Fc});
        const HostTensor* bb = pk.get(N + "blocks." + std::to_string(i) + nm + ".fc.bias", {2 * F});
        if (w && bb)
          for (int j = 0; j < 2 * F; ++j) {
            for (int k = 0; k < Fc; ++k) wt[(size_t)k * J + off + j] = w->data[(size_t)j * Fc + k];
            b[(size_t)off + j] = bb->data[(size_t)j];
          }
        off += 2 * F;
      }
    d.ada_wt = blob.add_f32(wt);
    d.ada_b = blob.add_f32(b);
  }
  for (int i = 0; i < cfg.dn_layers; ++i) {
    const std::string B = N + "blocks." + std::to_string(i);
    PBlock b;
    if (!cfg.multispeaker) {
      b.n_w = pk.vec(B + ".attention.norm.weight", F);          b.n_b = pk.vec(B + ".attention.norm.bias", F);
      b.nc_w = pk.vec(B + ".attention.norm_context.weight", F); b.nc_b = pk.vec(B + ".attention.norm_context.bias", F);
    }
    const int HD = cfg.dn_heads * cfg.dn_head_features, FM = F * cfg.dn_multiplier;
    b.q = pk.conv_w(B + ".attention.to_q.weight", HD, F, 1);
    b.kv = pk.conv_w(B + ".attention.to_kv.weight", 2 * HD, F, 1);
    b.o = pk.conv_w(B + ".attention.attention.to_out.weight", F, HD, 1); b.o_b = pk.vec(B + ".attention.attention.to_out.bias", F);
    b.f1 = pk.conv_w(B + ".feed_forward.0.weight", FM, F, 1);            b.f1_b = pk.vec(B + ".feed_forward.0.bias", FM);
    b.f1_out = b.f1.C_out;
    b.f2 = pk.conv_w(B + ".feed_forward.2.weight", F, FM, 1);            b.f2_b = pk.vec(B + ".feed_forward.2.bias", F);
    d.blocks.push_back(b);
  }
  {
    const HostTensor* w = pk.get(N + "to_out.1.weight", {cfg.dn_channels, F, 1});
    if (w) {
      const int O = (int)w->shape[0], I = (int)w->shape[1];
      std::vector<float> v((size_t)O * I);
      for (int o = 0; o < O; ++o)
        for (int i = 0; i < I; ++i) v[(size_t)i * O + o] = w->data[(size_t)o * I + i];
      d.out_t = blob.add_f32(v);
    }
    d.out_b = pk.vec(N + "to_out.1.bias", cfg.dn_channels);
  }
  d.fixed = pk.vec(N + "fixed_embedding.embedding.weight", (int64_t)cfg.dn_max_length * cfg.dn_embedding);
  if (!pk.ok) {
    *err = "denoiser weights (missing or malformed): " + pk.missing;
    return 1;
  }
  d.ready = true;
  e.dn = d;
  return 0;
}

struct ConvOpt {
  int dil = 1, pad_left = 0;
  const float* bias = nullptr;
  int pro = ST2_PRO_NONE;
  float slope = 0.f;
  const float* stats = nullptr;
  const float* gamma = nullptr;
  const float* beta = nullptr;
  int64_t gb_bs = 0;
  int gb_seg = 0;
  int gamma_plus_one = 0;
  const float* alpha = nullptr;
  View res; int res_shift = 0;
  View res2;
  float div = 1.0f;
  int act = ST2_ACT_NONE, act_split = 0;
  float act_slope = 0.f;
  float* stats_out = nullptr;
};

float x_scale_for(int pro) {
  return (pro == ST2_PRO_ADAIN_LEAKY || pro == ST2_PRO_ADAIN_SNAKE || pro == ST2_PRO_COLNORM) ? 8.0f : 1.0f;
}
int xs_row_slots(int L) { return XS_HALO + (std::max(L, 1) + 1 + 511) / 512 * 512 + 96; }

void finalize_stats(Ctx& c, float* part, const View& y, int nt, float* stats, int cols) {
  if (y.len)
    RUN(c, g_be.stats_finalize_len(part, y.B * y.C, nt, y.L, 1e-5f, stats, cols, y.len, y.C, c.stream));
  else
    RUN(c, g_be.stats_finalize(part, y.B * y.C, nt, y.L, 1e-5f, stats, cols, c.stream));
}

void instnorm_stats(Ctx& c, const View& x, float* stats) {
  if (x.len)
    RUN(c, g_be.instnorm_stats_len(x.p, x.bs, x.cs, x.B, x.C, x.L, 1e-5f, stats, x.len, c.stream));
  else
    RUN(c, g_be.instnorm_stats(x.p, x.bs, x.cs, x.B, x.C, x.L, 1e-5f, stats, c.stream));
}

void conv(Ctx& c, const st2_engine& e, const View& x, const SplitW& w, const View& y, const ConvOpt& o) {
  st2_conv_desc d;
  memset(&d, 0, sizeof(d));
  d.B = x.B; d.C_in = x.C; d.C_out = y.C; d.L_in = x.L; d.L_out = y.L; d.ks = w.ks; d.dil = o.dil; d.pad_left = o.pad_left;
  d.wq = e.P<const void>(w.wq); d.wq_co_pad = w.co_pad; d.wq_cin_pad = w.cin_pad;
  d.x_scale = e.x_scale(w.site, x_scale_for(o.pro));
  d.out_scale = 1.0f / d.x_scale;
  if (!c.dry) st2_headroom_set_site(&e, w.site);
  d.w_row_scale = e.F(w.row_scale);
  d.bias = o.bias;
  d.y = y.p; d.y_bs = y.bs; d.y_cs = y.cs;
  if (o.res.ok()) { d.res = o.res.p; d.res_bs = o.res.bs; d.res_cs = o.res.cs; d.res_shift = o.res_shift; }
  if (o.res2.ok()) { d.res2 = o.res2.p; d.res2_bs = o.res2.bs; d.res2_cs = o.res2.cs; }
  d.div = o.div;
  d.act = o.act; d.act_split = o.act_split; d.act_slope = o.act_slope;
  d.x_len = x.len; d.y_len = y.len;
  if (w.C_in != x.C || w.C_out != y.C) {
    if (c.rc == 0) { st2_set_error("engine: conv weight is %d->%d, call has %d->%d", w.C_in, w.C_out, x.C, y.C); c.rc = 1; }
    return;
  }
  const bool prefer_fused = o.pro != ST2_PRO_NONE && (x.C <= FUSED_MAX_C || (w.ks <= 3 && x.C <= FUSED_K3_MAX_C));
  const bool use_xs = o.pad_left <= XS_HALO && x.L >= XS_MIN_L && (o.pro != ST2_PRO_NONE || x.C >= XS_MIN_C_PLAIN) &&
                      !prefer_fused;
  const int64_t mark = c.a.off;
  if (use_xs) {
    const int cg = (x.C + 31) / 32 * 32 / 8;
    const int Lp = xs_row_slots(x.L);
    void* xs = c.a.alloc((int64_t)x.B * 2 * cg * Lp * 16);
    if (x.len)
      RUN(c, g_be.act_split_len(x.p, x.bs, x.cs, x.B, x.C, x.L, o.pro, o.slope, o.stats, o.gamma, o.beta, o.gb_bs, o.gb_seg,
                                o.gamma_plus_one, o.alpha, d.x_scale, xs, cg, Lp, XS_HALO, x.len, c.stream));
    else
      RUN(c, g_be.act_split(x.p, x.bs, x.cs, x.B, x.C, x.L, o.pro, o.slope, o.stats, o.gamma, o.beta, o.gb_bs, o.gb_seg,
                            o.gamma_plus_one, o.alpha, d.x_scale, xs, cg, Lp, XS_HALO, c.stream));
    d.xs = xs; d.xs_cg = cg; d.xs_lp = Lp; d.xs_halo = XS_HALO;
    float* part = nullptr;
    int nt = 0;
    if (o.stats_out) {
      const int pc = st2_conv1d_xs_part_cols(&d);
      nt = (y.L + pc - 1) / pc;
      part = c.a.f32((int64_t)y.B * y.C * nt * 3);
      d.part = part; d.part_nt = nt; d.part_cols = pc;
    }
    RUN(c, g_be.conv1d_xs(&d, c.stream));
    if (o.stats_out) finalize_stats(c, part, y, nt, o.stats_out, d.part_cols);
  } else {
    if (o.gb_seg > 0) {
      if (c.rc == 0) { st2_set_error("engine: a per-segment affine (gb_seg) needs the act_split + xs path"); c.rc = 1; }
      return;
    }
    d.x = x.p; d.x_bs = x.bs; d.x_cs = x.cs;
    d.pro = o.pro; d.slope = o.slope;
    d.stats = o.stats; d.gamma = o.gamma; d.beta = o.beta; d.gb_bs = o.gb_bs; d.gamma_plus_one = o.gamma_plus_one;
    d.alpha = o.alpha;
    float* part = nullptr;
    int nt = 0;
    if (o.stats_out) {
      nt = (y.L + 127) / 128;
      part = c.a.f32((int64_t)y.B * y.C * nt * 3);
      d.part = part; d.part_nt = nt;
    } else {
      const int64_t skb = st2_conv1d_f16s_splitk_bytes(&d);
      if (skb > 0) {
        d.splitk_ws = c.a.alloc(skb);
        d.splitk_ws_bytes = skb;
      }
    }
    RUN(c, g_be.conv1d_f16s(&d, c.stream));
    if (o.stats_out) finalize_stats(c, part, y, nt, o.stats_out, 128);
  }
  c.a.off = mark;
  if (!c.dry) st2_headroom_set_site(nullptr, -1);
}

float* new_stats(Ctx& c, int B, int C) { return c.a.f32((int64_t)B * C * 2); }

int64_t ragged_table_bytes(int B, int n) { return ((int64_t)n * B * 4 + 255) & ~(int64_t)255; }

#include "st2_plan_decoder.inc"
#include "st2_plan_sampler.inc"
#include "st2_plan_prosody.inc"
#include "st2_plan_duration.inc"
#include "st2_plan_text.inc"
#include "st2_plan_front.inc"
#include "st2_plan_style.inc"

}

extern "C" int st2_debug_set_backend(void* const* table, int32_t entries) {
  if (!table) {
    g_be = kHipBackend;
    return 0;
  }
  ST2_REQUIRE(entries == ST2_BACKEND_ENTRIES || entries == ST2_BACKEND_ENTRIES_V22,
              "st2_debug_set_backend: %d entries, expected %d (or %d: the slots before ABI v23)", entries,
              (int)ST2_BACKEND_ENTRIES, (int)ST2_BACKEND_ENTRIES_V22);
  for (int i = 0; i < entries; ++i) ST2_REQUIRE(table[i] != nullptr, "st2_debug_set_backend: entry %d is null", i);
#define SLOT(field, slot) g_be.field = reinterpret_cast<decltype(g_be.field)>(table[slot])
  SLOT(conv1d_f16s, ST2_BE_CONV1D_F16S); SLOT(conv1d_xs, ST2_BE_CONV1D_XS); SLOT(act_split, ST2_BE_ACT_SPLIT);
  SLOT(stats_finalize, ST2_BE_STATS_FINALIZE); SLOT(conv1d_direct, ST2_BE_CONV1D_DIRECT);
  SLOT(phase_split, ST2_BE_PHASE_SPLIT); SLOT(instnorm_stats, ST2_BE_INSTNORM_STATS);
  SLOT(colnorm_stats, ST2_BE_COLNORM_STATS); SLOT(style_fc, ST2_BE_STYLE_FC);
  SLOT(convt_interleave_stats, ST2_BE_CONVT_INTERLEAVE_STATS); SLOT(adain_leaky_pool, ST2_BE_ADAIN_LEAKY_POOL);
  SLOT(har_source, ST2_BE_HAR_SOURCE); SLOT(stft_mag_phase, ST2_BE_STFT_MAG_PHASE); SLOT(istft, ST2_BE_ISTFT);
  SLOT(attention_keylen, ST2_BE_ATTENTION_KEYLEN); SLOT(add_chanvec, ST2_BE_ADD_CHANVEC);
  SLOT(mean_tokens_len, ST2_BE_MEAN_TOKENS_LEN); SLOT(axpbypcz, ST2_BE_AXPBYPCZ);
  SLOT(time_features, ST2_BE_TIME_FEATURES); SLOT(tokens_to_channels, ST2_BE_TOKENS_TO_CHANNELS);
  SLOT(broadcast_cols, ST2_BE_BROADCAST_COLS); SLOT(copy_ncl, ST2_BE_COPY_NCL);
  SLOT(expand_by_durations, ST2_BE_EXPAND_BY_DURATIONS); SLOT(lstm_bidir, ST2_BE_LSTM_BIDIR);
  SLOT(colnorm_apply, ST2_BE_COLNORM_APPLY); SLOT(duration_head, ST2_BE_DURATION_HEAD); SLOT(mask_tail, ST2_BE_MASK_TAIL);
  SLOT(embed_tokens, ST2_BE_EMBED_TOKENS); SLOT(dwconv3x3s2, ST2_BE_DWCONV3X3S2); SLOT(avgpool2x2, ST2_BE_AVGPOOL2X2);
  SLOT(dev_alloc, ST2_BE_DEV_ALLOC); SLOT(dev_free, ST2_BE_DEV_FREE); SLOT(upload, ST2_BE_UPLOAD);
  const Backend& h = kHipBackend;
  g_be.act_split_len = h.act_split_len; g_be.instnorm_stats_len = h.instnorm_stats_len;
  g_be.stats_finalize_len = h.stats_finalize_len; g_be.conv1d_direct_len = h.conv1d_direct_len;
  g_be.adain_leaky_pool_len = h.adain_leaky_pool_len; g_be.convt_interleave_stats_len = h.convt_interleave_stats_len;
  g_be.har_source_len = h.har_source_len; g_be.stft_mag_phase_len = h.stft_mag_phase_len; g_be.istft_len = h.istft_len;
  g_be.ragged_lengths = h.ragged_lengths; g_be.expand_by_durations_len = h.expand_by_durations_len;
  if (entries == ST2_BACKEND_ENTRIES) {
    SLOT(act_split_len, ST2_BE_ACT_SPLIT_LEN); SLOT(instnorm_stats_len, ST2_BE_INSTNORM_STATS_LEN);
    SLOT(stats_finalize_len, ST2_BE_STATS_FINALIZE_LEN); SLOT(conv1d_direct_len, ST2_BE_CONV1D_DIRECT_LEN);
    SLOT(adain_leaky_pool_len, ST2_BE_ADAIN_LEAKY_POOL_LEN);
    SLOT(convt_interleave_stats_len, ST2_BE_CONVT_INTERLEAVE_STATS_LEN); SLOT(har_source_len, ST2_BE_HAR_SOURCE_LEN);
    SLOT(stft_mag_phase_len, ST2_BE_STFT_MAG_PHASE_LEN); SLOT(istft_len, ST2_BE_ISTFT_LEN);
    SLOT(ragged_lengths, ST2_BE_RAGGED_LENGTHS); SLOT(expand_by_durations_len, ST2_BE_EXPAND_BY_DURATIONS_LEN);
  }
#undef SLOT
  return 0;
}

extern "C" int st2_create(const st2_model_config* cfg, st2_engine** out) {
  ST2_REQUIRE(cfg && out, "st2_create: null argument");
  ST2_REQUIRE(check_cfg(*cfg), "st2_create: invalid model configuration");
  st2_engine* e = new (std::nothrow) st2_engine();
  ST2_REQUIRE(e, "st2_create: out of memory");
  e->cfg = *cfg;
  *out = e;
  return 0;
}

extern "C" int st2_destroy(st2_engine* e) {
  if (!e) return 0;
  if (e->wbase) g_be.dev_free(e->wbase);
  delete e;
  return 0;
}

extern "C" int st2_load_weights(st2_engine* e, const char* name, const float* data, const int64_t* shape, int32_t ndim) {
  ST2_REQUIRE(e && name && data && shape && ndim >= 0 && ndim <= 4, "st2_load_weights: bad arguments");
  HostTensor t;
  int64_t n = 1;
  for (int i = 0; i < ndim; ++i) {
    ST2_REQUIRE(shape[i] > 0, "st2_load_weights: %s has a non-positive dimension", name);
    t.shape.push_back(shape[i]);
    n *= shape[i];
  }
  t.data.assign(data, data + n);
  e->host[std::string(name)] = std::move(t);
  return 0;
}

struct PackedSet {
  PDecoder dec;
  PDenoiser dn;
  PPredictor pred;
  PDuration dur;
  PText text;
  PBert bert;
  PStyleEnc style[2];
  int64_t zeros = -1;
  std::vector<ConvSite> sites;
  std::vector<float> site_scale, site_seen;
};

namespace {
PackedSet packed_of(const st2_engine& e) {
  PackedSet p;
  p.sites = e.sites; p.site_scale = e.site_scale; p.site_seen = e.site_seen;
  p.dec = e.dec; p.dn = e.dn; p.pred = e.pred; p.dur = e.dur; p.text = e.text; p.bert = e.bert;
  p.style[0] = e.style[0]; p.style[1] = e.style[1]; p.zeros = e.zeros;
  return p;
}
void commit_packed(st2_engine& e, const PackedSet& p) {
  e.sites = p.sites; e.site_scale = p.site_scale; e.site_seen = p.site_seen;
  e.dec = p.dec; e.dn = p.dn; e.pred = p.pred; e.dur = p.dur; e.text = p.text; e.bert = p.bert;
  e.style[0] = p.style[0]; e.style[1] = p.style[1]; e.zeros = p.zeros;
}
}

extern "C" int st2_finalize_weights(st2_engine* e, int32_t which) {
  ST2_REQUIRE(e && (which & 63) != 0, "st2_finalize_weights: bad arguments");
  const PackedSet saved = packed_of(*e);
  Blob blob;
  std::string err;
  auto pack_all = [&]() -> int {
    if (which & 1) { if (pack_decoder(*e, blob, &err)) return 1; }
    else e->dec.ready = false;
    if (which & 2) { if (pack_denoiser(*e, blob, &err)) return 1; }
    else e->dn.ready = false;
    if (which & 4) { if (pack_predictor(*e, blob, &err)) return 1; }
    else e->pred.ready = false;
    e->dur.ready = false;
    if ((which & 4) && e->host.count("predictor.text_encoder.lstms.0.weight_ih_l0"))
      if (pack_duration(*e, blob, &err)) return 1;
    if (which & 8) { if (pack_text(*e, blob, &err)) return 1; }
    else e->text.ready = false;
    if (which & 16) { if (pack_bert(*e, blob, &err)) return 1; }
    else e->bert.ready = false;
    e->style[0].ready = e->style[1].ready = false;
    if (which & 32) {
      int found = 0;
      for (int k = 0; k < 2; ++k)
        if (e->host.count(std::string(k == 0 ? "style_encoder." : "predictor_encoder.") + "shared.0.weight")) {
          if (pack_style(*e, blob, k, &err)) return 1;
          ++found;
        }
      if (!found) { err = "no style_encoder.* / predictor_encoder.* parameters were loaded"; return 1; }
      e->zeros = blob.add_f32(std::vector<float>((size_t)STYLE_ZEROS, 0.0f));
    }
    return 0;
  };
  if (pack_all() != 0) {
    commit_packed(*e, saved);
    st2_set_error("st2_finalize_weights: %s", err.c_str());
    return 1;
  }
  const int64_t bytes = (int64_t)blob.host.size();
  void* p = g_be.dev_alloc(bytes);
  if (!p) {
    commit_packed(*e, saved);
    st2_set_error("st2_finalize_weights: device allocation of %lld B failed", (long long)bytes);
    return 1;
  }
  if (g_be.upload(p, blob.host.data(), bytes) != 0) {
    g_be.dev_free(p);
    commit_packed(*e, saved);
    st2_set_error("st2_finalize_weights: upload failed");
    return 1;
  }
  if (e->wbase) g_be.dev_free(e->wbase);
  e->wbase = static_cast<char*>(p);
  e->wbytes = bytes;
  e->sites = blob.sites;
  e->site_scale.assign(e->sites.size(), 0.f);
  e->site_seen.assign(e->sites.size(), 0.f);
  return 0;
}

extern "C" float st2_calibration_scale(float max_abs, int32_t margin_bits) {
  if (!(max_abs > 0.f) || !std::isfinite(max_abs)) return 0.f;
  margin_bits = std::min(std::max(margin_bits, 0), 10);
  int ex = 0;
  (void)frexpf(max_abs, &ex);
  return ldexpf(1.0f, std::min(std::max(16 - margin_bits - ex, -60), 60));
}

extern "C" int st2_calibrate(st2_engine* e, int32_t margin_bits, int32_t* n_clamped) {
  if (!e) { st2_set_error("st2_calibrate: null engine"); return -1; }
  const int n = st2_debug_headroom_read(nullptr, 0);
  if (n < 0) return -1;
  std::vector<double> rows((size_t)std::max(n, 1) * ST2_HEADROOM_COLS);
  if (n > 0 && st2_debug_headroom_read(rows.data(), n) < 0) return -1;
  const double me = (double)(uintptr_t)e;
  std::vector<float> seen(e->sites.size(), 0.f);
  std::vector<char> free_range(e->sites.size(), 0);
  int clamped = 0;
  for (int i = 0; i < n; ++i) {
    const double* r = rows.data() + (size_t)i * ST2_HEADROOM_COLS;
    const int site = (int)r[10];
    if (r[11] != me || site < 0 || site >= (int)seen.size() || !(r[5] > 0.0)) continue;
    if (r[6] >= 65504.0) ++clamped;
    seen[(size_t)site] = std::max(seen[(size_t)site], (float)(r[6] / r[5]));
    if (x_scale_for((int)r[1]) == 1.0f) free_range[(size_t)site] = 1;
  }
  e->site_scale.resize(e->sites.size(), 0.f);
  e->site_seen.resize(e->sites.size(), 0.f);
  int set = 0;
  for (size_t i = 0; i < seen.size(); ++i) {
    if (!(seen[i] > 0.f)) continue;
    e->site_seen[i] = std::max(e->site_seen[i], seen[i]);
    e->site_scale[i] = st2_calibration_scale(e->site_seen[i], margin_bits + (free_range[i] ? 2 : 0));
    ++set;
  }
  if (n_clamped) *n_clamped = clamped;
  return set;
}

extern "C" int st2_calibration_read(st2_engine* e, double* rows, int32_t cap_rows) {
  if (!e) return -1;
  const int n = (int)e->sites.size();
  for (int i = 0; rows && i < n && i < cap_rows; ++i) {
    double* r = rows + (size_t)i * ST2_CALIBRATION_COLS;
    r[0] = e->sites[(size_t)i].C_in; r[1] = e->sites[(size_t)i].C_out; r[2] = e->sites[(size_t)i].ks;
    r[3] = i < (int)e->site_scale.size() ? e->site_scale[(size_t)i] : 0.0;
    r[4] = i < (int)e->site_seen.size() ? e->site_seen[(size_t)i] : 0.0;
  }
  return n;
}

extern "C" int st2_calibration_site_name(st2_engine* e, int32_t site, char* name, int32_t cap) {
  ST2_REQUIRE(e && name && cap > 0 && site >= 0 && site < (int)e->sites.size(), "st2_calibration_site_name: bad arguments");
  snprintf(name, (size_t)cap, "%s", e->sites[(size_t)site].name.c_str());
  return 0;
}

extern "C" int st2_calibration_write(st2_engine* e, const float* scales, int32_t n) {
  ST2_REQUIRE(e && (n == 0 || scales) && n >= 0, "st2_calibration_write: bad arguments");
  if (n == 0) {
    e->site_scale.assign(e->sites.size(), 0.f);
    e->site_seen.assign(e->sites.size(), 0.f);
    return 0;
  }
  ST2_REQUIRE(n == (int)e->sites.size(), "st2_calibration_write: %d scales for %d conv sites (another model layout?)", n,
              (int)e->sites.size());
  for (int i = 0; i < n; ++i) {
    int ex = 0;
    const bool pow2 = scales[i] == 0.f || (scales[i] > 0.f && std::isfinite(scales[i]) && frexpf(scales[i], &ex) == 0.5f);
    ST2_REQUIRE(pow2, "st2_calibration_write: scale %d = %g is not a power of two (0 = by rule)", i, (double)scales[i]);
  }
  e->site_scale.assign(scales, scales + n);
  e->site_seen.assign(e->sites.size(), 0.f);
  return 0;
}

extern "C" int64_t st2_decoder_workspace_bytes(st2_engine* e, int32_t B, int32_t T) {
  if (!e || !e->dec.ready || B <= 0 || T <= 0) return -1;
  Ctx c;
  c.dry = true;
  c.a.dry = true;
  decoder_plan(c, *e, nullptr, nullptr, nullptr, nullptr, nullptr, nullptr, B, T, nullptr, nullptr);
  return c.a.peak + 256 + ragged_table_bytes(B, 16);
}

extern "C" int st2_decoder_forward(st2_engine* e, const float* asr, const float* f0, const float* n, const float* s,
                                   const float* sine_noise, const float* har_inject, int32_t B, int32_t T, float* wave,
                                   void* workspace, int64_t workspace_bytes, const st2_decoder_taps* taps, void* stream) {
  ST2_REQUIRE(e && e->dec.ready, "st2_decoder_forward: decoder weights not finalized");
  ST2_REQUIRE(asr && f0 && n && s && wave && workspace && B > 0 && T > 0, "st2_decoder_forward: bad arguments");
  ST2_REQUIRE(sine_noise || har_inject, "st2_decoder_forward: sine_noise (or har_inject) is required");
  ST2_REQUIRE((reinterpret_cast<uintptr_t>(workspace) & 255) == 0, "st2_decoder_forward: workspace must be 256-byte aligned");
  Ctx c;
  c.stream = stream;
  c.a.base = static_cast<char*>(workspace);
  c.a.cap = workspace_bytes;
  const int rc = decoder_plan(c, *e, asr, f0, n, s, sine_noise, har_inject, B, T, wave, taps);
  ST2_REQUIRE(!c.a.overflow, "st2_decoder_forward: workspace of %lld B is too small (need %lld B, see "
              "st2_decoder_workspace_bytes)", (long long)workspace_bytes, (long long)c.a.peak);
  return rc;
}

extern "C" int st2_decoder_forward_ragged(st2_engine* e, const float* asr, const float* f0, const float* n, const float* s,
                                          const float* sine_noise, const float* har_inject, const int32_t* frames, int32_t B,
                                          int32_t T_max, float* wave, void* workspace, int64_t workspace_bytes,
                                          const st2_decoder_taps* taps, void* stream) {
  ST2_REQUIRE(frames, "st2_decoder_forward_ragged: frames (int32 [B] on the device) is required");
  ST2_REQUIRE(B > 0 && T_max > 0, "st2_decoder_forward_ragged: bad geometry B=%d T_max=%d", B, T_max);
  ST2_REQUIRE(e && e->dec.ready, "st2_decoder_forward_ragged: decoder weights not finalized");
  ST2_REQUIRE(asr && f0 && n && s && wave && workspace, "st2_decoder_forward_ragged: bad arguments");
  ST2_REQUIRE(sine_noise || har_inject, "st2_decoder_forward_ragged: sine_noise (or har_inject) is required");
  ST2_REQUIRE(!taps, "st2_decoder_forward_ragged: taps are not supported (pass NULL)");
  ST2_REQUIRE((reinterpret_cast<uintptr_t>(workspace) & 255) == 0,
              "st2_decoder_forward_ragged: workspace must be 256-byte aligned");
  Ctx c;
  c.stream = stream;
  c.a.base = static_cast<char*>(workspace);
  c.a.cap = workspace_bytes;
  const int rc = decoder_plan(c, *e, asr, f0, n, s, sine_noise, har_inject, B, T_max, wave, taps, frames);
  ST2_REQUIRE(!c.a.overflow, "st2_decoder_forward_ragged: workspace of %lld B is too small (need %lld B, see "
              "st2_decoder_workspace_bytes)", (long long)workspace_bytes, (long long)c.a.peak);
  return rc;
}

extern "C" int64_t st2_text_workspace_bytes(st2_engine* e, int32_t B, int32_t N) {
  if (!e || !e->text.ready || B <= 0 || N <= 0) return -1;
  Ctx c;
  c.dry = true;
  c.a.dry = true;
  text_plan(c, *e, nullptr, nullptr, B, N, nullptr);
  return c.a.peak + 256;
}

extern "C" int st2_text_forward(st2_engine* e, const int64_t* tokens, const int32_t* lengths, int32_t B, int32_t N,
                                float* t_en, void* workspace, int64_t workspace_bytes, void* stream) {
  ST2_REQUIRE(e && e->text.ready, "st2_text_forward: text-encoder weights not finalized");
  ST2_REQUIRE(tokens && t_en && workspace && B > 0 && N > 0, "st2_text_forward: bad arguments");
  ST2_REQUIRE((reinterpret_cast<uintptr_t>(workspace) & 255) == 0, "st2_text_forward: workspace must be 256-byte aligned");
  Ctx c;
  c.stream = stream;
  c.a.base = static_cast<char*>(workspace);
  c.a.cap = workspace_bytes;
  const int rc = text_plan(c, *e, tokens, lengths, B, N, t_en);
  ST2_REQUIRE(!c.a.overflow, "st2_text_forward: workspace of %lld B is too small (need %lld B, see st2_text_workspace_bytes)",
              (long long)workspace_bytes, (long long)c.a.peak);
  return rc;
}

extern "C" int64_t st2_bert_workspace_bytes(st2_engine* e, int32_t B, int32_t N) {
  if (!e || !e->bert.ready || B <= 0 || N <= 0) return -1;
  Ctx c;
  c.dry = true;
// ... 242 lines not shown
```

styletts2_amd/csrc/st2_plan_decoder.inc:

```

struct DecRun {
  Ctx& c;
  const st2_engine& e;
  const float* h;
  int J;
  const int32_t* lenT = nullptr;
  const int32_t* len2T = nullptr;
  const float* gamma(int off) const { return h + off; }
  const float* beta(int off, int channels) const { return h + off + channels; }
};

View run_resblock1(DecRun& r, const PResBlock1& p, View x, const float* x_stats, View mrf_acc, bool mrf_last, int n_mrf,
                   View out) {
  Ctx& c = r.c;
  const int C = p.channels, ks = p.ks, B = x.B, L = x.L;
  const float* st = x_stats;
  if (!st) {
    float* s0 = new_stats(c, B, C);
    instnorm_stats(c, x, s0);
    st = s0;
  }
  View xt = new_ncl(c, B, C, L).with_len(x.len);
  View ping[2] = {new_ncl(c, B, C, L).with_len(x.len), new_ncl(c, B, C, L).with_len(x.len)};
  float* st2 = new_stats(c, B, C);
  float* stn[2] = {new_stats(c, B, C), new_stats(c, B, C)};
  for (int i = 0; i < 3; ++i) {
    const int d = p.dil[i];
    ConvOpt o1;
    o1.dil = d; o1.pad_left = (ks * d - d) / 2; o1.bias = r.e.F(p.c1[i].bias); o1.pro = ST2_PRO_ADAIN_SNAKE;
    o1.stats = st; o1.gamma = r.gamma(p.ad1[i]); o1.beta = r.beta(p.ad1[i], C); o1.gb_bs = r.J;
    o1.alpha = r.e.F(p.a1[i]); o1.stats_out = st2;
    conv(c, r.e, x, p.c1[i].w, xt, o1);
    const bool last = i == 2;
    ConvOpt o2;
    o2.dil = 1; o2.pad_left = (ks - 1) / 2; o2.bias = r.e.F(p.c2[i].bias); o2.pro = ST2_PRO_ADAIN_SNAKE;
    o2.stats = st2; o2.gamma = r.gamma(p.ad2[i]); o2.beta = r.beta(p.ad2[i], C); o2.gb_bs = r.J;
    o2.alpha = r.e.F(p.a2[i]); o2.res = x;
    if (last) {
      o2.res2 = mrf_acc;
      o2.div = mrf_last ? (float)n_mrf : 1.0f;
      conv(c, r.e, xt, p.c2[i].w, out, o2);
      x = out;
    } else {
      o2.stats_out = stn[i & 1];
      conv(c, r.e, xt, p.c2[i].w, ping[i & 1], o2);
      x = ping[i & 1];
      st = stn[i & 1];
    }
  }
  return x;
}

void run_adain_resblk(DecRun& r, const PAdainResBlk& p, const View& x, const View& out_in) {
  Ctx& c = r.c;
  const int B = x.B, L = x.L;
  const int64_t mark = c.a.off;
  const int32_t* len_o = x.len;
  if (x.len && p.upsample) {
    if (x.len != r.lenT && c.rc == 0) { st2_set_error("engine: ragged up-sampling block on rows of unknown length"); c.rc = 1; }
    len_o = r.len2T;
  }
  const View out = out_in.with_len(len_o);
  float* st1 = new_stats(c, B, p.dim_in);
  instnorm_stats(c, x.rows(0, p.dim_in), st1);
  float* st2 = new_stats(c, B, p.dim_out);
  const int Lo = p.upsample ? 2 * L : L;
  View t1 = new_ncl(c, B, p.dim_out, Lo).with_len(len_o);
  if (p.upsample) {
    View u = new_ncl(c, B, p.dim_in, 2 * L).with_len(len_o);
    if (x.len)
      RUN(c, g_be.adain_leaky_pool_len(x.p, x.bs, x.cs, st1, r.gamma(p.n1), r.beta(p.n1, p.dim_in), r.J, 0.2f,
                                       r.e.F(p.pool_w), r.e.F(p.pool_b), u.p, u.bs, u.cs, B, p.dim_in, L, x.len, c.stream));
    else
      RUN(c, g_be.adain_leaky_pool(x.p, x.bs, x.cs, st1, r.gamma(p.n1), r.beta(p.n1, p.dim_in), r.J, 0.2f,
                                   r.e.F(p.pool_w), r.e.F(p.pool_b), u.p, u.bs, u.cs, B, p.dim_in, L, c.stream));
    ConvOpt o;
    o.pad_left = 1; o.bias = r.e.F(p.conv1.bias); o.stats_out = st2;
    conv(c, r.e, u, p.conv1.w, t1, o);
  } else {
    ConvOpt o;
    o.pad_left = 1; o.bias = r.e.F(p.conv1.bias); o.pro = ST2_PRO_ADAIN_LEAKY; o.slope = 0.2f; o.stats = st1;
    o.gamma = r.gamma(p.n1); o.beta = r.beta(p.n1, p.dim_in); o.gb_bs = r.J; o.stats_out = st2;
    conv(c, r.e, x, p.conv1.w, t1, o);
  }
  View sc = x;
  if (p.learned_sc) {
    sc = new_ncl(c, B, p.dim_out, L).with_len(x.len);
    ConvOpt o;
    conv(c, r.e, x, p.sc.w, sc, o);
  }
  ConvOpt o;
  o.pad_left = 1; o.bias = r.e.F(p.conv2.bias); o.pro = ST2_PRO_ADAIN_LEAKY; o.slope = 0.2f; o.stats = st2;
  o.gamma = r.gamma(p.n2); o.beta = r.beta(p.n2, p.dim_out); o.gb_bs = r.J; o.res = sc;
  o.res_shift = p.upsample ? 1 : 0;
  o.div = (float)sqrt(2.0);
  conv(c, r.e, t1, p.conv2.w, out, o);
  c.a.off = mark;
}

void tap(Ctx& c, const View& v, float* dst) {
  if (!dst) return;
  RUN(c, g_be.copy_ncl(v.p, v.bs, v.cs, dst, (int64_t)v.C * v.L, v.L, v.B, v.C, v.L, c.stream));
}

struct DecLens {
  enum { T1 = 0, T2, SAMPLES, HAR, STAGE0 };
  std::vector<int32_t> coef;
  int add(long long mul, long long a, long long div = 1) {
    coef.push_back((int32_t)mul); coef.push_back((int32_t)a); coef.push_back((int32_t)div);
    return (int)coef.size() / 3 - 1;
  }
};

int decoder_plan(Ctx& c, const st2_engine& e, const float* asr_p, const float* f0_p, const float* n_p, const float* s_p,
                 const float* sine_noise, const float* har_inject, int B, int T, float* wave,
                 const st2_decoder_taps* taps, const int32_t* frames = nullptr) {
  const st2_model_config& cfg = e.cfg;
  const PDecoder& d = e.dec;
  const PGenerator& g = d.gen;
  const bool ist = cfg.decoder_kind == 0;
  const int Cin = cfg.dim_in, nu = cfg.n_upsamples, nk = cfg.n_resblock_kernels;
  const int T2 = 2 * T;
  st2_decoder_taps notaps;
  memset(&notaps, 0, sizeof(notaps));
  if (!taps) taps = &notaps;

  const int hop_ = cfg.gen_istft_hop;
  const int up_ = prod_from(cfg.upsample_rates, 0, nu) * (ist ? hop_ : 1);
  const int32_t* lens = nullptr;
  auto len_of = [&](int i) -> const int32_t* { return lens ? lens + (int64_t)i * B : nullptr; };
  if (frames) {
    if (nu > 4) { st2_set_error("engine: ragged decoder supports up to 4 up-sampling stages"); return 1; }
    static_assert(DecLens::STAGE0 + 3 * 4 <= 16, "st2_decoder_workspace_bytes sizes a table of 16 lengths");
    DecLens dl;
    dl.add(1, 0); dl.add(2, 0); dl.add(2LL * up_, 0);
    if (ist) dl.add(2LL * up_, hop_, hop_);
    else dl.add(2LL * up_, 0);
    long long m = 2, a = 0;
    long long hm = 2LL * up_ / (ist ? hop_ : 1), ha = ist ? 1 : 0;
    for (int i = 0; i < nu; ++i) {
      const int u = cfg.upsample_rates[i], k = cfg.upsample_kernel_sizes[i];
      const int pad = ist ? (k - u) / 2 : u / 2 + u % 2;
      const int extra = ist ? 0 : u % 2;
      const int refl = (ist && i + 1 == nu) ? 1 : 0;
      const long long m_o = m * u, a_o = (a - 1) * u - 2 * pad + k + extra + refl;
      dl.add(m_o, a_o);
      dl.add(m, a + 1);
      const int sf = g.noise_stride[i];
      if (sf > 1) {
        const int pf = (sf + 1) / 2;
        dl.add(hm, ha + 2 * pf - 2 * sf + sf + sf, sf);
      } else {
        dl.add(hm, ha);
      }
      m = m_o; a = a_o;
    }
    int32_t* tab = static_cast<int32_t*>(c.a.alloc((int64_t)dl.coef.size() / 3 * B * 4));
    RUN(c, g_be.ragged_lengths(frames, B, T, (int)dl.coef.size() / 3, dl.coef.data(), tab, c.stream));
    lens = tab;
  }

  float* h = c.a.f32((int64_t)B * d.J);
  RUN(c, g_be.style_fc(s_p, B, cfg.style_dim, e.F(d.bank_wt), e.F(d.bank_b), d.J, ST2_ACT_NONE, h, c.stream));
  DecRun r{c, e, h, d.J};
  r.lenT = len_of(DecLens::T1);
  r.len2T = len_of(DecLens::T2);

  View asr = wrap(asr_p, B, Cin, T).with_len(r.lenT);
  View f0 = wrap(f0_p, B, 1, T2).with_len(r.len2T), nn = wrap(n_p, B, 1, T2).with_len(r.len2T);
  View cat = new_ncl(c, B, 1024 + 64 + 2, T, false).with_len(r.lenT);
  View cat0 = new_ncl(c, B, Cin + 2, T, false).with_len(r.lenT);
  RUN(c, g_be.copy_ncl(asr.p, asr.bs, asr.cs, cat0.p, cat0.bs, cat0.cs, B, Cin, T, c.stream));
  {
    View a = cat0.rows(Cin, Cin + 1), b = cat0.rows(Cin + 1, Cin + 2);
    if (frames) {
      RUN(c, g_be.conv1d_direct_len(f0.p, f0.bs, f0.cs, e.F(d.f0_w), e.F(d.f0_b), a.p, a.bs, a.cs, B, 1, 1, T2, T, 3, 2, 1,
                                    f0.len, nullptr, c.stream));
      RUN(c, g_be.conv1d_direct_len(nn.p, nn.bs, nn.cs, e.F(d.n_w), e.F(d.n_b), b.p, b.bs, b.cs, B, 1, 1, T2, T, 3, 2, 1,
                                    nn.len, nullptr, c.stream));
    } else {
      RUN(c, g_be.conv1d_direct(f0.p, f0.bs, f0.cs, e.F(d.f0_w), e.F(d.f0_b), a.p, a.bs, a.cs, B, 1, 1, T2, T, 3, 2, 1, c.stream));
      RUN(c, g_be.conv1d_direct(nn.p, nn.bs, nn.cs, e.F(d.n_w), e.F(d.n_b), b.p, b.bs, b.cs, B, 1, 1, T2, T, 3, 2, 1, c.stream));
    }
    View src = cat0.rows(Cin, Cin + 2), dst = cat.rows(1088, 1090);
    RUN(c, g_be.copy_ncl(src.p, src.bs, src.cs, dst.p, dst.bs, dst.cs, B, 2, T, c.stream));
  }
  {
    ConvOpt o;
    o.bias = e.F(d.asr_res.bias);
    conv(c, e, asr, d.asr_res.w, cat.rows(1024, 1088), o);
  }
  run_adain_resblk(r, d.encode, cat0, cat.rows(0, 1024));
  tap(c, cat.rows(0, 1024), taps->encode);
  View x = new_ncl(c, B, 512, T2).with_len(r.len2T);
  for (int i = 0; i < 4; ++i) {
    if (d.decode[i].upsample)
      run_adain_resblk(r, d.decode[i], cat, x);
    else
      run_adain_resblk(r, d.decode[i], cat, cat.rows(0, 1024));
  }
  tap(c, x, taps->front);

  int up_scale = prod_from(cfg.upsample_rates, 0, nu) * (ist ? cfg.gen_istft_hop : 1);
  const int L = T2 * up_scale;
  const int n_fft = cfg.gen_istft_n_fft, hop = cfg.gen_istft_hop;
  View har;
  if (har_inject) {
    har = ist ? wrap(har_inject, B, n_fft + 2, L / hop + 1) : wrap(har_inject, B, 1, L);
  } else {
    float* scratch = c.a.f32((int64_t)B * 9 * T2);
    float* hs = c.a.f32((int64_t)B * L);
    if (frames)
      RUN(c, g_be.har_source_len(f0_p, B, T2, up_scale, 9, sine_noise, e.F(g.lin_w), e.F(g.lin_b), 0.1f, 0.003f, 10.0f,
                                 24000.0f, scratch, hs, r.len2T, c.stream));
    else
      RUN(c, g_be.har_source(f0_p, B, T2, up_scale, 9, sine_noise, e.F(g.lin_w), e.F(g.lin_b), 0.1f, 0.003f, 10.0f,
                             24000.0f, scratch, hs, c.stream));
    if (taps->har_source) RUN(c, g_be.copy_ncl(hs, L, L, taps->har_source, L, L, B, 1, L, c.stream));
    if (ist) {
      har = new_ncl(c, B, n_fft + 2, L / hop + 1, false);
      if (frames)
        RUN(c, g_be.stft_mag_phase_len(hs, B, L, n_fft, hop, har.p, har.bs, har.cs, len_of(DecLens::SAMPLES), c.stream));
      else
        RUN(c, g_be.stft_mag_phase(hs, B, L, n_fft, hop, har.p, har.bs, har.cs, c.stream));
    } else {
      har = wrap(hs, B, 1, L);
    }
  }
  har = har.with_len(len_of(DecLens::HAR));
  if (ist) tap(c, har, taps->har);

  for (int i = 0; i < nu; ++i) {
    const int u = cfg.upsample_rates[i], k = cfg.upsample_kernel_sizes[i], C = g.channels[i];
    const bool last = i + 1 == nu;
    const int L_in = x.L;
    int pad, L_raw;
    if (ist) {
      pad = (k - u) / 2;
      L_raw = (L_in - 1) * u - 2 * ((k - u) / 2) + k;
    } else {
      pad = u / 2 + u % 2;
      L_raw = (L_in - 1) * u - 2 * (u / 2 + u % 2) + k + u % 2;
    }
    const bool reflect = ist && last;
    const int L_out = L_raw + (reflect ? 1 : 0);
    const int32_t* len_o = len_of(DecLens::STAGE0 + 3 * i);
    View x_next = new_ncl(c, B, C, L_out).with_len(len_o);
    const int64_t stage_mark = c.a.off;
    View xs_src = new_ncl(c, B, C, L_out).with_len(len_o);
    {
      const int64_t m = c.a.off;
      View xs0 = new_ncl(c, B, C, L_out).with_len(len_o);
      const int stride_f0 = g.noise_stride[i];
      ConvOpt o;
      o.bias = e.F(g.noise_b[i]);
      if (stride_f0 > 1) {
        const int pad_f0 = (stride_f0 + 1) / 2;
        const int L_ns = (har.L + 2 * pad_f0 - 2 * stride_f0) / stride_f0 + 1;
        View harp = new_ncl(c, B, har.C * stride_f0, L_ns + 1, false).with_len(len_of(DecLens::STAGE0 + 3 * i + 2));
        RUN(c, g_be.phase_split(har.p, har.bs, har.cs, B, har.C, har.L, stride_f0, pad_f0, harp.p, harp.bs, harp.cs,
                                L_ns + 1, c.stream));
        if (L_ns != L_out && c.rc == 0) { st2_set_error("engine: noise conv length %d != stage length %d", L_ns, L_out); c.rc = 1; }
        conv(c, e, harp, g.noise_wt[i], xs0, o);
      } else {
        conv(c, e, har, g.noise_wt[i], xs0, o);
      }
      View nul;
      run_resblock1(r, g.noise_res[i], xs0, nullptr, nul, false, nk, xs_src);
      c.a.off = m;
    }
    View xu = new_ncl(c, B, C, L_out).with_len(len_o);
    float* st = new_stats(c, B, C);
    {
      const int64_t m = c.a.off;
      View Y = new_ncl(c, B, u * C, L_in + 1).with_len(len_of(DecLens::STAGE0 + 3 * i + 1));
      ConvOpt o;
      o.pad_left = 1;
      if (ist) { o.pro = ST2_PRO_LEAKY; o.slope = 0.1f; } else { o.pro = ST2_PRO_SNAKE; o.alpha = e.F(g.alphas[i]); }
      conv(c, e, x, g.ups_wt[i], Y, o);
      const int nt = (L_out + CVT_TILE - 1) / CVT_TILE;
      float* part = c.a.f32((int64_t)B * C * nt * 3);
      if (frames)
        RUN(c, g_be.convt_interleave_stats_len(Y.p, Y.bs, Y.cs, L_in + 1, e.F(g.ups_b[i]), xs_src.p, xs_src.bs, xs_src.cs,
                                               xu.p, xu.bs, xu.cs, B, C, u, pad, L_raw, reflect ? 1 : 0, part, nt, Y.len,
                                               len_o, c.stream));
      else
        RUN(c, g_be.convt_interleave_stats(Y.p, Y.bs, Y.cs, L_in + 1, e.F(g.ups_b[i]), xs_src.p, xs_src.bs, xs_src.cs,
                                           xu.p, xu.bs, xu.cs, B, C, u, pad, L_raw, reflect ? 1 : 0, part, nt, c.stream));
      finalize_stats(c, part, xu, nt, st, CVT_TILE);
      c.a.off = m;
    }
    View acc[2] = {new_ncl(c, B, C, L_out).with_len(len_o), new_ncl(c, B, C, L_out).with_len(len_o)};
    View prev;
    for (int j = 0; j < nk; ++j) {
      const int64_t m = c.a.off;
      const bool lastk = j + 1 == nk;
      View out = lastk ? x_next : acc[j & 1];
      run_resblock1(r, g.resblocks[(size_t)i * nk + j], xu, st, prev, lastk, nk, out);
      prev = out;
      c.a.off = m;
    }
    x = x_next;
    c.a.off = stage_mark;
    if (i < 4) tap(c, x, taps->stage[i]);
  }
  if (ist) {
    const int nb = n_fft / 2 + 1;
    View sp = new_ncl(c, B, n_fft + 2, x.L, false).with_len(x.len);
    ConvOpt o;
    o.pad_left = 3; o.bias = e.F(g.post.bias); o.pro = ST2_PRO_LEAKY; o.slope = 0.01f; o.act = ST2_ACT_EXP_SIN;
    o.act_split = nb;
    conv(c, e, x, g.post.w, sp, o);
    tap(c, sp, taps->spec_phase);
    if (frames)
      RUN(c, g_be.istft_len(sp.p, sp.bs, sp.cs, B, x.L, n_fft, hop, wave, (int64_t)hop * (x.L - 1), x.len, c.stream));
    else
      RUN(c, g_be.istft(sp.p, sp.bs, sp.cs, B, x.L, n_fft, hop, wave, (int64_t)hop * (x.L - 1), c.stream));
  } else {
    View w = wrap(wave, B, 1, x.L).with_len(x.len);
    ConvOpt o;
    o.pad_left = 3; o.bias = e.F(g.post.bias); o.pro = ST2_PRO_SNAKE; o.alpha = e.F(g.alphas[(size_t)nu]);
    o.act = ST2_ACT_TANH;
    conv(c, e, x, g.post.w, w, o);
    if (frames) RUN(c, g_be.mask_tail(w.p, w.bs, w.cs, B, 1, w.L, w.len, c.stream));
  }
  return c.rc;
}
```

styletts2_amd/csrc/st2_plan_sampler.inc:

```

struct Sess {
  Ctx& c;
  const st2_engine& e;
  int B, N;
  bool merged;
  const int32_t* key_len;
  View bases[2];
  int nbases;
  const float* feat_map;
  const float* ada;
  double scale;
};

View dn_alloc(Sess& s, int C) {
  View v;
  v.B = s.B; v.C = C; v.L = s.N;
  v.p = s.c.a.f32((int64_t)s.B * C * s.N);
  if (s.merged) { v.bs = s.N; v.cs = s.B * s.N; } else { v.bs = (int64_t)C * s.N; v.cs = s.N; }
  return v;
}
View dn_cv(const Sess& s, const View& t) {
  if (!s.merged) return t;
  View v = t;
  v.B = 1; v.L = s.B * s.N; v.bs = (int64_t)t.C * v.L; v.cs = v.L;
  return v;
}

const float* dn_mapping(Sess& s, float c_noise) {
  Ctx& c = s.c;
  const st2_engine& e = s.e;
  const PDenoiser& d = e.dn;
  const int F = d.features, H2 = e.cfg.dn_channels / 2;
  float* four = c.a.f32((int64_t)s.B * (1 + 2 * H2));
  RUN(c, g_be.time_features(c_noise, e.F(d.time_w), H2, s.B, four, c.stream));
  float* m = c.a.f32((int64_t)s.B * F);
  RUN(c, g_be.style_fc(four, s.B, 1 + 2 * H2, e.F(d.time_lin), e.F(d.time_b), F, ST2_ACT_GELU, m, c.stream));
  if (s.feat_map) {
    float* m2 = c.a.f32((int64_t)s.B * F);
    RUN(c, g_be.axpbypcz(m, 1.0f, s.feat_map, 1.0f, nullptr, 0.0f, m2, (int64_t)s.B * F, c.stream));
    m = m2;
  }
  float* m3 = c.a.f32((int64_t)s.B * F);
  RUN(c, g_be.style_fc(m, s.B, F, e.F(d.map0), e.F(d.map0_b), F, ST2_ACT_GELU, m3, c.stream));
  float* m4 = c.a.f32((int64_t)s.B * F);
  RUN(c, g_be.style_fc(m3, s.B, F, e.F(d.map2), e.F(d.map2_b), F, ST2_ACT_GELU, m4, c.stream));
  return m4;
}

void dn_run(Sess& s, View base, const float* x, const float* m, float* out) {
  Ctx& c = s.c;
  const st2_engine& e = s.e;
  const PDenoiser& d = e.dn;
  const st2_model_config& cfg = e.cfg;
  const int B = s.B, N = s.N, Fz = d.features, C = cfg.dn_channels;
  const int mid = cfg.dn_heads * cfg.dn_head_features;
  const int64_t mark = c.a.off;
  View b0 = base.rows(0, C);
  RUN(c, g_be.broadcast_cols(x, C, b0.p, b0.bs, b0.cs, B, C, N, c.stream));
  View X = dn_alloc(s, Fz);
  RUN(c, g_be.add_chanvec(base.p, base.bs, base.cs, m, Fz, X.p, X.bs, X.cs, B, Fz, N, c.stream));
  const int nblk = (int)d.blocks.size();
  for (int i = 0; i < nblk; ++i) {
    const PBlock& b = d.blocks[(size_t)i];
    float* st = c.a.f32((int64_t)B * N * 2);
    RUN(c, g_be.colnorm_stats(X.p, X.bs, X.cs, B, Fz, N, 1e-5f, st, c.stream));
    View qkv = dn_alloc(s, 3 * mid);
    ConvOpt o1, o2;
    o1.pro = o2.pro = ST2_PRO_COLNORM;
    o1.stats = o2.stats = st;
    if (cfg.multispeaker) {
      const int64_t J = (int64_t)nblk * 4 * Fz;
      const float* a = s.ada + (int64_t)4 * Fz * i;
      o1.gamma = a;          o1.beta = a + Fz;     o1.gb_bs = J; o1.gamma_plus_one = 1;
      o2.gamma = a + 2 * Fz; o2.beta = a + 3 * Fz; o2.gb_bs = J; o2.gamma_plus_one = 1;
    } else {
      o1.gamma = e.F(b.n_w);  o1.beta = e.F(b.n_b);
      o2.gamma = e.F(b.nc_w); o2.beta = e.F(b.nc_b);
    }
    const bool seg = cfg.multispeaker && s.merged && B > 1 && (int64_t)B * N >= XS_MIN_L && Fz > FUSED_K3_MAX_C;
    if (seg) o1.gb_seg = o2.gb_seg = N;
    const bool per_utt = cfg.multispeaker && !seg;
    View Xv = per_utt ? X : dn_cv(s, X), qv = per_utt ? qkv : dn_cv(s, qkv);
    conv(c, e, Xv, b.q, qv.rows(0, mid), o1);
    conv(c, e, Xv, b.kv, qv.rows(mid, 3 * mid), o2);
    View att = dn_alloc(s, mid);
    View q = qkv.rows(0, mid), k = qkv.rows(mid, 2 * mid), v = qkv.rows(2 * mid, 3 * mid);
    RUN(c, g_be.attention_keylen(q.p, k.p, v.p, q.bs, q.cs, att.p, att.bs, att.cs, B, cfg.dn_heads, cfg.dn_head_features,
                                 N, (float)pow((double)cfg.dn_head_features, -0.5), s.key_len, c.stream));
    View X1 = dn_alloc(s, Fz), hmid = dn_alloc(s, b.f1_out), X2 = dn_alloc(s, Fz);
    ConvOpt oo;
    oo.bias = e.F(b.o_b); oo.res = dn_cv(s, X);
    conv(c, e, dn_cv(s, att), b.o, dn_cv(s, X1), oo);
    ConvOpt of1;
    of1.bias = e.F(b.f1_b); of1.act = ST2_ACT_GELU;
    conv(c, e, dn_cv(s, X1), b.f1, dn_cv(s, hmid), of1);
    ConvOpt of2;
    of2.bias = e.F(b.f2_b); of2.res = dn_cv(s, X1);
    conv(c, e, dn_cv(s, hmid), b.f2, dn_cv(s, X2), of2);
    if (i + 1 < nblk) {
      View Xn = dn_alloc(s, Fz);
      RUN(c, g_be.add_chanvec(X2.p, X2.bs, X2.cs, m, Fz, Xn.p, Xn.bs, Xn.cs, B, Fz, N, c.stream));
      X = Xn;
    } else {
      X = X2;
    }
  }
  float* mean = c.a.f32((int64_t)B * Fz);
  RUN(c, g_be.mean_tokens_len(X.p, X.bs, X.cs, mean, Fz, B, Fz, N, s.key_len, c.stream));
  RUN(c, g_be.style_fc(mean, B, Fz, e.F(d.out_t), e.F(d.out_b), C, ST2_ACT_NONE, out, c.stream));
  c.a.off = mark;
}

void dn_denoise(Sess& s, const float* x, const double* w4, float* out) {
  Ctx& c = s.c;
  const int C = s.e.cfg.dn_channels;
  const int64_t n = (int64_t)s.B * C;
  const int64_t mark = c.a.off;
  const float c_skip = (float)w4[0], c_out = (float)w4[1], c_in = (float)w4[2], c_noise = (float)w4[3];
  float* x_in = c.a.f32(n);
  RUN(c, g_be.axpbypcz(x, c_in, nullptr, 0.f, nullptr, 0.f, x_in, n, c.stream));
  const float* m = dn_mapping(s, c_noise);
  float* pred = c.a.f32(n);
  dn_run(s, s.bases[0], x_in, m, pred);
  if (s.nbases > 1) {
    float* pm = c.a.f32(n);
    dn_run(s, s.bases[1], x_in, m, pm);
    float* mix = c.a.f32(n);
    RUN(c, g_be.axpbypcz(pm, (float)(1.0 - s.scale), pred, (float)s.scale, nullptr, 0.f, mix, n, c.stream));
    pred = mix;
  }
  RUN(c, g_be.axpbypcz(x, c_skip, pred, c_out, nullptr, 0.f, out, n, c.stream));
  c.a.off = mark;
}

int sampler_plan(Ctx& c, const st2_engine& e, const float* noise, const float* embedding, const View* emb_cm,
                 const float* features, const float* step_noise, const int32_t* lengths, int B, int N, int steps, double scale,
                 const double* table, double sigma0, float* out, float* step_taps) {
  const st2_model_config& cfg = e.cfg;
  const PDenoiser& d = e.dn;
  const int C = cfg.dn_channels, E = cfg.dn_embedding, Fz = d.features;
  Sess s{c, e, B, N, true, lengths, {}, 1, nullptr, nullptr, scale};
  s.bases[0] = dn_alloc(s, Fz);
  {
    View dst = s.bases[0].rows(C, Fz);
    if (emb_cm)
      RUN(c, g_be.copy_ncl(emb_cm->p, emb_cm->bs, emb_cm->cs, dst.p, dst.bs, dst.cs, B, E, N, c.stream));
    else
      RUN(c, g_be.tokens_to_channels(embedding, (int64_t)N * E, B, N, E, dst.p, dst.bs, dst.cs, c.stream));
  }
  if (scale != 1.0) {
    s.nbases = 2;
    s.bases[1] = dn_alloc(s, Fz);
    View dst = s.bases[1].rows(C, Fz);
    RUN(c, g_be.tokens_to_channels(e.F(d.fixed), 0, B, N, E, dst.p, dst.bs, dst.cs, c.stream));
  }
  if (cfg.multispeaker) {
    if (!features) { st2_set_error("st2_sampler_run: the multispeaker denoiser needs `features`"); return 1; }
    float* fm = c.a.f32((int64_t)B * Fz);
    RUN(c, g_be.style_fc(features, B, cfg.dn_context_features, e.F(d.feat), e.F(d.feat_b), Fz, ST2_ACT_GELU, fm, c.stream));
    const int J = cfg.dn_layers * 4 * Fz;
    float* ada = c.a.f32((int64_t)B * J);
    RUN(c, g_be.style_fc(features, B, cfg.dn_context_features, e.F(d.ada_wt), e.F(d.ada_b), J, ST2_ACT_NONE, ada, c.stream));
    s.feat_map = fm;
    s.ada = ada;
  }
  const int64_t n = (int64_t)B * C;
  float* xa = c.a.f32(n);
  float* xb = c.a.f32(n);
  float* x = xa;
  RUN(c, g_be.axpbypcz(noise, (float)sigma0, nullptr, 0.f, nullptr, 0.f, x, n, c.stream));
  for (int i = 0; i + 1 < steps; ++i) {
    const double* row = table + (int64_t)i * ST2_SAMPLER_TABLE_COLS;
    const int64_t mark = c.a.off;
    float* den = c.a.f32(n);
    dn_denoise(s, x, row + 0, den);
    const double k = row[8];
    float* x_mid = c.a.f32(n);
    RUN(c, g_be.axpbypcz(x, (float)(1.0 + k), den, (float)(-k), nullptr, 0.f, x_mid, n, c.stream));
    float* den_mid = c.a.f32(n);
    dn_denoise(s, x_mid, row + 4, den_mid);
    const double k2 = row[9];
    float* d_mid = c.a.f32(n);
    RUN(c, g_be.axpbypcz(x_mid, (float)k2, den_mid, (float)(-k2), nullptr, 0.f, d_mid, n, c.stream));
    float* xn = (x == xa) ? xb : xa;
    RUN(c, g_be.axpbypcz(x, 1.0f, d_mid, 1.0f, step_noise + (int64_t)i * n, (float)row[10], xn, n, c.stream));
    x = xn;
    if (step_taps) RUN(c, g_be.axpbypcz(x, 1.0f, nullptr, 0.f, nullptr, 0.f, step_taps + (int64_t)i * n, n, c.stream));
    c.a.off = mark;
  }
  RUN(c, g_be.axpbypcz(x, 1.0f, nullptr, 0.f, nullptr, 0.f, out, n, c.stream));
  return c.rc;
}
```

styletts2_amd/decoder.py:

```python
import math

import torch
import torch.nn as nn

from .layers import transient_state
from . import ops
from . import weights as W
from .layers import (AdaINParams, AdaINResBlock1Params, AdainResBlk1dParams, PlainConv1d, PlainLinear, WNConv1d,
                     WNConvTranspose1d)

LRELU_SLOPE = 0.1


class StyleBank:

    def __init__(self):
        self._mods, self._off = [], {}
        self.J = 0

    def add(self, adain: AdaINParams):
        self._off[id(adain)] = (self.J, adain.channels)
        self._mods.append(adain)
        self.J += 2 * adain.channels

    def pack(self, device):
        self.wt = torch.cat([m.fc.weight.detach().t() for m in self._mods], dim=1).contiguous().float().to(device)
        self.bias = torch.cat([m.fc.bias.detach() for m in self._mods]).contiguous().float().to(device)

    def run(self, s):
        return ops.style_fc(s.contiguous(), self.wt, self.bias)

    def gb(self, h, adain):
        off, c = self._off[id(adain)]
        return h[:, off:off + c], h[:, off + c:off + 2 * c]


def _dev(t, device):
    return t.detach().float().contiguous().to(device)


class _PackedConv:
    def __init__(self, conv: WNConv1d, device):
        self.wt = W.pack_conv_auto(conv.folded().float()).to(device)
        self.bias = _dev(conv.bias, device) if conv.bias is not None else None
        self.c_out, self.ks = conv.c_out, conv.ks


class _PackedResBlock1:
    def __init__(self, p: AdaINResBlock1Params, device):
        self.p = p
        self.c1 = [_PackedConv(c, device) for c in p.convs1]
        self.c2 = [_PackedConv(c, device) for c in p.convs2]
        self.a1 = [_dev(a.reshape(-1), device) for a in p.alpha1]
        self.a2 = [_dev(a.reshape(-1), device) for a in p.alpha2]


def run_resblock1(pk: _PackedResBlock1, bank: StyleBank, h, x, x_stats=None, mrf_acc=None, mrf_last=False,
                  n_mrf=3, out=None):
    p = pk.p
    C, ks = p.channels, p.ks
    nsteps = len(p.dilation)
    st = x_stats if x_stats is not None else ops.instnorm_stats(x)
    for i, d in enumerate(p.dilation):
        g1, b1 = bank.gb(h, p.adain1[i])
        xt, st2 = ops.conv1d(x, pk.c1[i].wt, C, ks, dil=d, pad_left=(ks * d - d) // 2, bias=pk.c1[i].bias,
                             pro=ops.PRO_ADAIN_SNAKE, stats=st, gamma=g1, beta=b1, alpha=pk.a1[i], want_stats=True)
        g2, b2 = bank.gb(h, p.adain2[i])
        last = i == nsteps - 1
        kw = dict(dil=1, pad_left=(ks - 1) // 2, bias=pk.c2[i].bias, pro=ops.PRO_ADAIN_SNAKE, stats=st2, gamma=g2,
                  beta=b2, alpha=pk.a2[i], res=x)
        if last:
            x = ops.conv1d(xt, pk.c2[i].wt, C, ks, res2=mrf_acc, div=float(n_mrf) if mrf_last else 1.0, out=out, **kw)
        else:
            x, st = ops.conv1d(xt, pk.c2[i].wt, C, ks, want_stats=True, **kw)
    return x


class _PackedAdainResBlk:
    def __init__(self, p: AdainResBlk1dParams, device):
        self.p = p
        self.conv1 = _PackedConv(p.conv1, device)
        self.conv2 = _PackedConv(p.conv2, device)
        self.sc = _PackedConv(p.conv1x1, device) if p.learned_sc else None
        if p.upsample:
            self.pool_w = _dev(p.pool.folded().reshape(p.dim_in, 3), device)
            self.pool_b = _dev(p.pool.bias, device)


def run_adain_resblk(pk: _PackedAdainResBlk, bank: StyleBank, h, x, out=None):
    p = pk.p
    st1 = ops.instnorm_stats(x)
    g1, b1 = bank.gb(h, p.norm1)
    if p.upsample:
        u = ops.adain_leaky_pool(x, st1, g1, b1, 0.2, pk.pool_w, pk.pool_b)
        t1, st2 = ops.conv1d(u, pk.conv1.wt, p.dim_out, 3, pad_left=1, bias=pk.conv1.bias, want_stats=True)
    else:
        t1, st2 = ops.conv1d(x, pk.conv1.wt, p.dim_out, 3, pad_left=1, bias=pk.conv1.bias, pro=ops.PRO_ADAIN_LEAKY,
                             slope=0.2, stats=st1, gamma=g1, beta=b1, want_stats=True)
    g2, b2 = bank.gb(h, p.norm2)
    sc = ops.conv1d(x, pk.sc.wt, p.dim_out, 1) if pk.sc is not None else x
    return ops.conv1d(t1, pk.conv2.wt, p.dim_out, 3, pad_left=1, bias=pk.conv2.bias, pro=ops.PRO_ADAIN_LEAKY,
                      slope=0.2, stats=st2, gamma=g2, beta=b2, res=sc, res_shift=1 if p.upsample else 0,
                      div=math.sqrt(2), out=out)


class _SourceModule(nn.Module):

    def __init__(self, harmonics):
        super().__init__()
        self.l_linear = PlainLinear(harmonics, 1)


class Generator(nn.Module):

    HARMONICS = 9

    def __init__(self, kind, style_dim, resblock_kernel_sizes, upsample_rates, upsample_initial_channel,
                 resblock_dilation_sizes, upsample_kernel_sizes, gen_istft_n_fft=None, gen_istft_hop_size=None):
        super().__init__()
        assert kind in ("istftnet", "hifigan")
        self.kind = kind
        self.rates, self.up_ks = list(upsample_rates), list(upsample_kernel_sizes)
        self.num_kernels, self.num_upsamples = len(resblock_kernel_sizes), len(upsample_rates)
        self.n_fft, self.hop = gen_istft_n_fft, gen_istft_hop_size
        c0 = upsample_initial_channel
        self.channels = [c0 // (2 ** (i + 1)) for i in range(self.num_upsamples)]
        self.m_source = _SourceModule(self.HARMONICS)
        src_ch = (self.n_fft + 2) if kind == "istftnet" else 1
        self.noise_convs, self.noise_res, self.ups, self.resblocks = (nn.ModuleList(), nn.ModuleList(),
                                                                      nn.ModuleList(), nn.ModuleList())
        for i, (u, k) in enumerate(zip(self.rates, self.up_ks)):
            c_cur = self.channels[i]
            self.ups.append(WNConvTranspose1d(c0 // (2 ** i), c_cur, k, c_cur))
            if i + 1 < self.num_upsamples:
                stride_f0 = int(math.prod(self.rates[i + 1:]))
                self.noise_convs.append(PlainConv1d(src_ch, c_cur, stride_f0 * 2))
                self.noise_res.append(AdaINResBlock1Params(c_cur, 7, (1, 3, 5), style_dim))
            else:
                self.noise_convs.append(PlainConv1d(src_ch, c_cur, 1))
                self.noise_res.append(AdaINResBlock1Params(c_cur, 11, (1, 3, 5), style_dim))
        if kind == "hifigan":
            self.alphas = nn.ParameterList([nn.Parameter(torch.ones(1, c0, 1))] +
                                           [nn.Parameter(torch.ones(1, c, 1)) for c in self.channels])
        for i in range(self.num_upsamples):
            for k, d in zip(resblock_kernel_sizes, resblock_dilation_sizes):
                self.resblocks.append(AdaINResBlock1Params(self.channels[i], k, tuple(d), style_dim))
        self.conv_post = WNConv1d(self.channels[-1], (self.n_fft + 2) if kind == "istftnet" else 1, 7)
        self.upsample_scale = int(math.prod(self.rates)) * (self.hop if kind == "istftnet" else 1)

    def register(self, bank: StyleBank):
        for rb in list(self.noise_res) + list(self.resblocks):
            for a in list(rb.adain1) + list(rb.adain2):
                bank.add(a)

    def pack(self, device):
        pk = type("PackedGenerator", (), {})()
        pk.lin_w = _dev(self.m_source.l_linear.weight.reshape(-1), device)
        pk.lin_b = _dev(self.m_source.l_linear.bias.reshape(-1), device)
        pk.noise_wt, pk.noise_stride = [], []
        for i, c in enumerate(self.noise_convs):
            stride_f0 = int(math.prod(self.rates[i + 1:])) if i + 1 < self.num_upsamples else 1
            w = c.weight.detach().float()
            if stride_f0 > 1:
                w = W.polyphase_strided_conv(w, stride_f0)
            pk.noise_wt.append(W.pack_conv_auto(w).to(device))
            pk.noise_stride.append(stride_f0)
        pk.noise_b = [_dev(c.bias, device) for c in self.noise_convs]
        pk.noise_res = [_PackedResBlock1(r, device) for r in self.noise_res]
        pk.resblocks = [_PackedResBlock1(r, device) for r in self.resblocks]
        pk.ups_wt = [W.pack_conv_auto(W.polyphase_convt(u.folded().float(), r)).to(device)
                     for u, r in zip(self.ups, self.rates)]
        pk.ups_b = [_dev(u.bias, device) for u in self.ups]
        pk.post = _PackedConv(self.conv_post, device)
        if self.kind == "hifigan":
            pk.alphas = [_dev(a.reshape(-1), device) for a in self.alphas]
        return pk

    def _mrf(self, pk, bank, h, x, st, i):
        n = self.num_kernels
        blocks = pk.resblocks[i * n:(i + 1) * n]
        acc = None
        for j in range(n):
            acc = run_resblock1(blocks[j], bank, h, x, x_stats=st, mrf_acc=acc, mrf_last=(j == n - 1), n_mrf=n)
        return acc

    def run(self, pk, bank, h, x, f0_curve, noise=None, har=None, taps=None):
        B = x.shape[0]
        L = f0_curve.shape[1] * self.upsample_scale
        ist = self.kind == "istftnet"
        if har is None:
            if noise is None:
                noise = torch.randn(B, L, self.HARMONICS, device=x.device, dtype=torch.float32)
            har_source = ops.har_source(f0_curve.contiguous(), self.upsample_scale, noise, pk.lin_w, pk.lin_b,
                                        sine_amp=0.1, noise_std=0.003, voiced_threshold=10.0, sample_rate=24000.0)
            har = ops.stft_mag_phase(har_source, self.n_fft, self.hop) if ist else har_source.unsqueeze(1)
            if taps is not None:
                taps["har_source"] = har_source
        if taps is not None:
            taps["har"] = har
        for i in range(self.num_upsamples):
            u, k, C = self.rates[i], self.up_ks[i], self.channels[i]
            last = i == self.num_upsamples - 1
            stride_f0 = pk.noise_stride[i]
            if stride_f0 > 1:
                pad_f0 = (stride_f0 + 1) // 2
                L_ns = (har.shape[2] + 2 * pad_f0 - 2 * stride_f0) // stride_f0 + 1
                harp = ops.phase_split(har, stride_f0, pad_f0, L_ns + 1)
                xs = ops.conv1d(harp, pk.noise_wt[i], C, 2, pad_left=0, L_out=L_ns, bias=pk.noise_b[i])
            else:
                xs = ops.conv1d(har, pk.noise_wt[i], C, 1, bias=pk.noise_b[i])
            xs = run_resblock1(pk.noise_res[i], bank, h, xs)
            L_in = x.shape[2]
            if ist:
                pad, L_raw = (k - u) // 2, (L_in - 1) * u - 2 * ((k - u) // 2) + k
                pro = dict(pro=ops.PRO_LEAKY, slope=LRELU_SLOPE)
            else:
                pad, L_raw = u // 2 + u % 2, (L_in - 1) * u - 2 * (u // 2 + u % 2) + k + u % 2
                pro = dict(pro=ops.PRO_SNAKE, alpha=pk.alphas[i])
            Y = ops.conv1d(x, pk.ups_wt[i], u * C, 2, pad_left=1, L_out=L_in + 1, **pro)
            x, st = ops.convt_interleave(Y, C, u, pad, L_raw, bias=pk.ups_b[i], add=xs, reflect_left=(ist and last),
                                         want_stats=True)
            x = self._mrf(pk, bank, h, x, st, i)
            if taps is not None:
                taps["stage%d" % i] = x
        if ist:
            nb = self.n_fft // 2 + 1
            sp = ops.conv1d(x, pk.post.wt, self.n_fft + 2, 7, pad_left=3, bias=pk.post.bias, pro=ops.PRO_LEAKY,
                            slope=0.01, act=ops.ACT_EXP_SIN, act_split=nb)
            if taps is not None:
                taps["spec_phase"] = sp
            return ops.istft(sp, self.n_fft, self.hop)
        return ops.conv1d(x, pk.post.wt, 1, 7, pad_left=3, bias=pk.post.bias, pro=ops.PRO_SNAKE,
                          alpha=pk.alphas[self.num_upsamples], act=ops.ACT_TANH)


@transient_state
class Decoder(nn.Module):

    def __init__(self, dim_in=512, F0_channel=512, style_dim=64, dim_out=80, resblock_kernel_sizes=(3, 7, 11),
                 upsample_rates=(10, 6), upsample_initial_channel=512,
                 resblock_dilation_sizes=((1, 3, 5), (1, 3, 5), (1, 3, 5)), upsample_kernel_sizes=(20, 12),
                 gen_istft_n_fft=20, gen_istft_hop_size=5, kind="istftnet"):
        super().__init__()
        self.kind, self.dim_in = kind, dim_in
        self.encode = AdainResBlk1dParams(dim_in + 2, 1024, style_dim)
        self.decode = nn.ModuleList([AdainResBlk1dParams(1024 + 2 + 64, 1024, style_dim) for _ in range(3)] +
                                    [AdainResBlk1dParams(1024 + 2 + 64, 512, style_dim, upsample=True)])
        self.F0_conv = WNConv1d(1, 1, 3)
        self.N_conv = WNConv1d(1, 1, 3)
        self.asr_res = nn.Sequential(WNConv1d(dim_in, 64, 1))
        if kind == "istftnet":
            self.generator = Generator(kind, style_dim, resblock_kernel_sizes, upsample_rates,
                                       upsample_initial_channel, resblock_dilation_sizes, upsample_kernel_sizes,
                                       gen_istft_n_fft, gen_istft_hop_size)
        else:
            self.generator = Generator(kind, style_dim, resblock_kernel_sizes, upsample_rates,
                                       upsample_initial_channel, resblock_dilation_sizes, upsample_kernel_sizes)
        self._pk = None

    def __setattr__(self, name, value):
        if name == "_pk" and value is None:
            old = self.__dict__.get("_eng")
            if old is not None:
                from . import engine
                engine.replaced(old, "decoder")
            object.__setattr__(self, "_eng", None)
        super().__setattr__(name, value)

    def _apply(self, fn, *a, **k):
        self._pk = None
        return super()._apply(fn, *a, **k)

    def load_state_dict(self, state_dict, *a, **k):
        self._pk = None
        return super().load_state_dict(W.strip_module_prefix(state_dict), *a, **k)

    def _load_from_state_dict(self, *a, **k):
        self._pk = None
        return super()._load_from_state_dict(*a, **k)

    def refresh(self):
        self._pk = None

    def _prepare(self, device):
        pk = type("PackedDecoder", (), {})()
        pk.device = device
        bank = StyleBank()
        for blk in [self.encode] + list(self.decode):
            bank.add(blk.norm1)
            bank.add(blk.norm2)
        self.generator.register(bank)
        bank.pack(device)
        pk.bank = bank
        pk.encode = _PackedAdainResBlk(self.encode, device)
        pk.decode = [_PackedAdainResBlk(b, device) for b in self.decode]
        pk.f0_w, pk.f0_b = _dev(self.F0_conv.folded(), device), _dev(self.F0_conv.bias, device)
        pk.n_w, pk.n_b = _dev(self.N_conv.folded(), device), _dev(self.N_conv.bias, device)
        pk.asr_res = _PackedConv(self.asr_res[0], device)
        pk.gen = self.generator.pack(device)
        self._pk = pk
        return pk

    @torch.no_grad()
    def forward(self, asr, F0_curve, N, s, noise=None, har=None, taps=None, frames=None):
        if self.training:
            raise RuntimeError("the MI355X engine is inference-only; call .eval() (reference: istftnet.py:500-508 "
                               "is the training-only F0/N smoothing)")
        dev = asr.device
        from . import engine
        if asr.is_cuda and engine.plan_mode() == "engine" and W.conv_precision() == "f16s":
            eng = self._eng
            if eng is None or not engine.same_device(eng, dev):
                engine.replaced(eng, "decoder")
                eng = self._eng = engine.build_decoder_engine(self, dev)
            return eng.decoder_forward(asr, F0_curve, N, s, noise=noise, har=har, taps=taps, frames=frames)
        if frames is not None:
            raise RuntimeError("Decoder.forward(frames=...): the ragged decoder exists only in the C++ engine "
                               "(plan_mode 'engine', f16s convs on a HIP device)")
        pk = self._pk if (self._pk is not None and self._pk.device == dev) else self._prepare(dev)
        bank = pk.bank
        asr = asr.float().contiguous()
        B, Cin, T = asr.shape
        h = bank.run(s.float())
        F0_curve = F0_curve.float().contiguous()
        N = N.float().contiguous()
        cat = torch.empty((B, 1024 + 64 + 2, T), device=dev, dtype=torch.float32)
        cat0 = torch.empty((B, Cin + 2, T), device=dev, dtype=torch.float32)
        ops.copy_ncl(asr, cat0[:, :Cin])
        ops.conv1d_direct(F0_curve.unsqueeze(1), pk.f0_w, pk.f0_b, 2, 1, out=cat0[:, Cin:Cin + 1])
        ops.conv1d_direct(N.unsqueeze(1), pk.n_w, pk.n_b, 2, 1, out=cat0[:, Cin + 1:Cin + 2])
        ops.copy_ncl(cat0[:, Cin:Cin + 2], cat[:, 1088:1090])
        ops.conv1d(asr, pk.asr_res.wt, 64, 1, bias=pk.asr_res.bias, out=cat[:, 1024:1088])
        run_adain_resblk(pk.encode, bank, h, cat0, out=cat[:, :1024])
        if taps is not None:
            taps["encode"] = cat[:, :1024].clone()
        x = None
        for i, blk in enumerate(pk.decode):
            if blk.p.upsample:
                x = run_adain_resblk(blk, bank, h, cat)
            else:
                run_adain_resblk(blk, bank, h, cat, out=cat[:, :1024])
        if taps is not None:
            taps["front"] = x
        return self.generator.run(pk.gen, bank, h, x, F0_curve, noise=noise, har=har, taps=taps)
```

styletts2_amd/ops.py:

```python
import ctypes as C
import json
import warnings

import torch

from . import _hooks, _lib
from .weights import F16S_X_SCALE, SplitConvWeight
from ._lib import (ACT_EXP_SIN, ACT_GELU, ACT_GELU_TANH, ACT_LEAKY, ACT_NONE, ACT_TANH, PRO_ADAIN_LEAKY, PRO_ADAIN_SNAKE,
                   PRO_COLNORM, PRO_LEAKY, PRO_NONE, PRO_SNAKE, ConvDesc)


def _stream():
    return C.c_void_p(torch.cuda.current_stream().cuda_stream)


_AUX_STREAMS = {}


def aux_stream(dev, priority=0, index=0):
    dev = torch.device(dev)
    key = (dev.index if dev.index is not None else torch.cuda.current_device(), int(priority), int(index))
    if key not in _AUX_STREAMS:
        _AUX_STREAMS[key] = torch.cuda.Stream(dev, priority=int(priority))
    return _AUX_STREAMS[key]


_PROBE_BUF = {}


def wait_blocks(waiter, victim, spin_cycles=3_000_000, mode="wait"):
    dev = victim.device
    key = dev.index
    if key not in _PROBE_BUF:
        _PROBE_BUF[key] = (torch.zeros(64, device=dev), torch.cuda.Stream(dev))
    buf, spin = _PROBE_BUF[key]
    for st in (waiter, victim, spin):
        with torch.cuda.stream(st):
            buf.add_(0.0)
    torch.cuda.synchronize(dev)
    e_spin, e_tiny = torch.cuda.Event(), torch.cuda.Event()
    src = waiter if mode == "kernel" else spin
    with torch.cuda.stream(src):
        torch.cuda._sleep(int(spin_cycles))
        e_spin.record(src)
    if mode != "kernel":
        waiter.wait_event(e_spin)
    with torch.cuda.stream(victim):
        buf.add_(1.0)
        e_tiny.record(victim)
    while not e_tiny.query():
        pass
    blocked = e_spin.query()
    torch.cuda.synchronize(dev)
    return bool(blocked)


def _chk(t, name, ndim=None):
    if t is None:
        return
    if not t.is_cuda:
        raise _lib.St2Error("%s must live on a HIP device (got %s); the engine has no CPU path" % (name, t.device))
    if t.dtype != torch.float32:
        raise _lib.St2Error("%s must be float32 (got %s)" % (name, t.dtype))
    if ndim is not None and t.dim() != ndim:
        raise _lib.St2Error("%s must be %d-D (got shape %s)" % (name, ndim, tuple(t.shape)))
    if t.dim() > 0 and t.shape[-1] > 1 and t.stride(-1) != 1:
        raise _lib.St2Error("%s must have unit stride along its last axis" % name)


def _ptr(t):
    return 0 if t is None else t.data_ptr()


def _chk_len(t, name, n, like):
    if t is None:
        return 0
    if not torch.is_tensor(t) or t.dtype != torch.int32:
        raise _lib.St2Error("%s must be an int32 tensor (got %s)" % (name, t.dtype if torch.is_tensor(t) else type(t).__name__))
    if t.numel() != n or not t.is_contiguous():
        raise _lib.St2Error("%s must be a contiguous tensor of %d entries (got shape %s)" % (name, n, tuple(t.shape)))
    if not t.is_cuda or not torch.is_tensor(like) or t.device != like.device:
        raise _lib.St2Error("%s must live on the device of the tensor it describes (%s, got %s)" % (
            name, like.device if torch.is_tensor(like) else None, t.device))
    return t.data_ptr()


def _nb(t, ndim=3):
    return t.shape[0] if torch.is_tensor(t) and t.dim() == ndim else -1


def _bs_cs(t):
    return t.stride(0), t.stride(1)


_PRO_NORM = (PRO_ADAIN_LEAKY, PRO_ADAIN_SNAKE, PRO_COLNORM)
_PRO_SNAKE = (PRO_ADAIN_SNAKE, PRO_SNAKE)


def _chk_prologue(pro, B, Cc, L, stats, gamma, beta, alpha, gb_seg):
    gbs = 0
    if pro in _PRO_NORM:
        _chk(stats, "stats", 3)
        _chk(gamma, "gamma", 2)
        _chk(beta, "beta", 2)
        want = (B, L, 2) if pro == PRO_COLNORM else (B, Cc, 2)
        assert tuple(stats.shape) == want and stats.is_contiguous(), (stats.shape, want)
        assert gamma.shape[1] == Cc and beta.shape[1] == Cc
        gbs = gamma.stride(0) if gamma.shape[0] > 1 else 0
        bbs = beta.stride(0) if beta.shape[0] > 1 else 0
        if gb_seg:
            assert pro == PRO_COLNORM and B == 1 and gamma.shape[0] * gb_seg >= L and beta.shape[0] == gamma.shape[0]
            assert gbs == bbs
        else:
            assert gamma.shape[0] in (1, B) and beta.shape[0] == gamma.shape[0] and gbs == bbs
    if pro in _PRO_SNAKE:
        _chk(alpha, "alpha", 1)
        assert alpha.numel() == Cc and alpha.is_contiguous()
    return gbs


def _chk_split_weight(wt, C_in, C_out, ks):
    if (wt.C_in, wt.C_out, wt.ks) != (C_in, C_out, ks) or not wt.wq.is_cuda or not wt.wq.is_contiguous():
        raise _lib.St2Error("split weight is for (C_in=%d, C_out=%d, ks=%d) on %s, call has (%d, %d, %d)" % (
            wt.C_in, wt.C_out, wt.ks, wt.wq.device, C_in, C_out, ks))


def x_scale_for(pro):
    return F16S_X_SCALE if pro in _PRO_NORM else 1.0


def calibrated_x_scale(max_abs, margin_bits=3):
    return float(_lib.load().st2_calibration_scale(float(max_abs), int(margin_bits)))


def status(clear=False):
    return _lib.load().st2_status(1 if clear else 0)


lstm_recoveries = 0
frame_capacity_hits = 0


def check_status(ignore=0):
    st = status(clear=True)
    if st > 0:
        st &= ~int(ignore)
    if st > 0 and st & _lib.STATUS_LSTM_RECOVERED:
        global lstm_recoveries
        lstm_recoveries += 1
        warnings.warn("a cooperative BiLSTM group was not co-resident in time; the call was re-run on the single-CU kernel "
                      "in-stream (results valid; ST2_STATUS_LSTM_RECOVERED)", RuntimeWarning, stacklevel=2)
        st &= ~_lib.STATUS_LSTM_RECOVERED
    if st > 0 and st & _lib.STATUS_FRAME_CAPACITY:
        global frame_capacity_hits
        frame_capacity_hits += 1
        warnings.warn("an utterance needed more frames than the capacity given with the call (`max_frames`) and was synthesised "
                      "truncated to it; the other rows of its batch are unaffected; retry that row with a larger capacity "
                      "(ST2_STATUS_FRAME_CAPACITY)", RuntimeWarning, stacklevel=2)
        st &= ~(_lib.STATUS_FRAME_CAPACITY | _lib.STATUS_DURATION_SUM)
    if st <= 0:
        return
    msgs = []
    if st & _lib.STATUS_F16_RANGE:
        msgs.append("a split-f16 conv operand exceeded the f16 range (|x * x_scale| > 65504) and was clamped: the "
                    "result is finite but wrong; calibrate the operand scales for this checkpoint (pipeline.calibrate / st2_calibrate) and "
                    "check it with tools/validate_checkpoint.py, which names the conv site and its headroom")
    if st & _lib.STATUS_LSTM_TIMEOUT:
        msgs.append("a cooperative BiLSTM group timed out (its workgroups were not co-resident in time) on a launch without "
                    "the recovery pass: outputs of that call are invalid")
    if st & _lib.STATUS_DURATION_SUM:
        msgs.append("a row of the supplied durations does not sum to the frame count given with it (`total_frames`): the "
                    "alignment of that call repeated its last phoneme")
    raise _lib.St2Error("device-side status 0x%x: %s" % (st, "; ".join(msgs)))


class conv_autotune:

    def __init__(self, reset=False):
        self.reset = reset

    def __enter__(self):
        lib = _lib.load()
        if self.reset:
            _lib.check(lib.st2_conv_tune(-1), "st2_conv_tune")
        _lib.check(lib.st2_conv_tune(1), "st2_conv_tune")
        return self

    def __exit__(self, *exc):
        torch.cuda.synchronize()
        _lib.check(_lib.load().st2_conv_tune(0), "st2_conv_tune")
        return False


TUNE_VARIANT_BITS = {1: "128x256 tiles, 2 wg/CU", 2: "XCD-aware tile order"}


def tune_variant_name(v):
    if v < 0:
        return "rule"
    names = [n for b, n in TUNE_VARIANT_BITS.items() if v & b]
    return " + ".join(names) if names else "128x128 tiles, 3 wg/CU, dispatch order"


def conv_tune_table():
    lib = _lib.load()
    n = lib.st2_conv_tune_read(None, 0)
    rows = (C.c_double * (24 * max(n, 1)))()
    n = min(n, lib.st2_conv_tune_read(rows, n))
    out = []
    for i in range(n):
        r = rows[24 * i:24 * i + 24]
        cands = [{"variant": int(r[8 + 2 * j]), "name": tune_variant_name(int(r[8 + 2 * j])), "ms": round(r[9 + 2 * j], 5)}
                 for j in range(int(r[7]))]
        out.append({"ks": int(r[0]), "C_in": int(r[1]), "C_out": int(r[2]), "L": int(r[3]), "B": int(r[4]),
                    "chosen": int(r[6]), "chosen_name": tune_variant_name(int(r[6])), "candidates": cands})
    return out


def conv_tune_set(ks, C_in, C_out, L_out, B, variant):
    _lib.check(_lib.load().st2_conv_tune_set(ks, C_in, C_out, L_out, B, variant), "st2_conv_tune_set")


def probe_cu_health():
    buf = C.create_string_buffer(16384)
    mask = (C.c_uint32 * 16)()
    n = C.c_int32(0)
    _lib.check(_lib.load().st2_probe_cu_health(buf, len(buf), mask, 16, C.byref(n)), "st2_probe_cu_health")
    rep = json.loads(buf.value.decode())
    words = (rep["cus"] + 31) // 32
    return rep, [int(mask[i]) for i in range(words)], int(n.value)


class headroom:

    def __enter__(self):
        _lib.check(_lib.load().st2_debug_headroom(1), "st2_debug_headroom")
        self.rows = []
        return self

    def __exit__(self, *exc):
        lib = _lib.load()
        torch.cuda.synchronize()
        _lib.check(lib.st2_debug_headroom(0), "st2_debug_headroom")
        n = lib.st2_debug_headroom_read(None, 0)
        W = _lib.HEADROOM_COLS
        buf = (C.c_double * (W * max(n, 1)))()
        n = min(n, lib.st2_debug_headroom_read(buf, n))
        pro_names = ["none", "leaky", "adain+leaky", "adain+snake", "snake", "layernorm"]
        for i in range(max(n, 0)):
            r = buf[W * i:W * i + W]
            self.rows.append({"index": i, "kind": "fused conv" if int(r[0]) else "act_split", "pro": pro_names[int(r[1])],
                              "B": int(r[2]), "C": int(r[3]), "L": int(r[4]), "x_scale": r[5], "max_abs": r[6], "frac": r[7],
                              "rel_err": r[8], "sub_share": r[9], "site": int(r[10]), "engine": int(r[11])})
        return False


def probe_box(level=0):
    buf = C.create_string_buffer(16384)
    _lib.check(_lib.load().st2_probe_box(buf, len(buf), level), "st2_probe_box")
    return json.loads(buf.value.decode())


XS_HALO = 32
FUSED_MAX_C, FUSED_K3_MAX_C = 64, 128
XS_MIN_L = 256
XS_MIN_C_PLAIN = 64


def prefer_fused(pro, C_in, ks):
    return pro != PRO_NONE and (C_in <= FUSED_MAX_C or (ks <= 3 and C_in <= FUSED_K3_MAX_C))


def conv_path():
    return _hooks.conv_path


class XsTensor:

    def __init__(self, data, C, L, halo, x_scale=F16S_X_SCALE):
        self.data, self.C, self.L, self.halo, self.x_scale = data, C, L, halo, x_scale

    @property
    def cg(self):
        return self.data.shape[2]

    @property
    def Lp(self):
        return self.data.shape[3]


def xs_row_slots(L):
    return XS_HALO + (max(L, 1) + 1 + 511) // 512 * 512 + 96


def activate(x, *, pro=PRO_NONE, slope=0.0, stats=None, gamma=None, beta=None, gamma_plus_one=False, alpha=None,
              c_pad=32, gb_seg=0, x_scale=None, lengths=None):
    lp = _chk_len(lengths, "lengths", _nb(x), x)
    if lengths is not None and pro == PRO_COLNORM:
        raise _lib.St2Error("activate: per-row lengths are not defined for PRO_COLNORM (st2_act_split_len)")
    lib = _lib.load()
    _chk(x, "x", 3)
    B, Cc, L = x.shape
    cg = (Cc + c_pad - 1) // c_pad * c_pad // 8
    Lp = xs_row_slots(L)
    data = torch.empty((B, 2, cg, Lp, 8), device=x.device, dtype=torch.float16)
    gbs = _chk_prologue(pro, B, Cc, L, stats, gamma, beta, alpha, gb_seg)
    xsc = float(x_scale) if x_scale else x_scale_for(pro)
    _lib.check(lib.st2_act_split_len(x.data_ptr(), x.stride(0), x.stride(1), B, Cc, L, pro, slope, _ptr(stats),
                                     _ptr(gamma), _ptr(beta), gbs, int(gb_seg), 1 if gamma_plus_one else 0, _ptr(alpha),
                                     xsc, data.data_ptr(), cg, Lp, XS_HALO, lp, _stream()), "st2_act_split_len")
    return XsTensor(data, Cc, L, XS_HALO, xsc)


def new_part(B, C, nt, device):
    return torch.empty((B * C * nt * 3,), device=device, dtype=torch.float32)


def stats_finalize(part, B, C, nt, L, cols=128, eps=1e-5, out=None, lengths=None, len_div=1):
    if lengths is None:
        len_div = 1
    elif len_div <= 0 or (B * C) % len_div:
        raise _lib.St2Error("stats_finalize: len_div=%d does not divide the %d rows" % (len_div, B * C))
    lp = _chk_len(lengths, "lengths", B * C // len_div, part)
    lib = _lib.load()
    assert part.numel() >= B * C * nt * 3 and part.is_contiguous()
    if out is None:
        out = torch.empty((B, C, 2), device=part.device, dtype=torch.float32)
    _lib.check(lib.st2_stats_finalize_len(part.data_ptr(), B * C, nt, L, eps, out.data_ptr(), int(cols), lp, int(len_div),
                                          _stream()), "st2_stats_finalize_len")
    return out


def conv1d_xs(xs, wt, C_out, ks, *, dil=1, pad_left=0, L_out=None, bias=None, out=None, res=None, res_shift=0,
              res2=None, div=1.0, act=ACT_NONE, act_split=0, act_slope=0.0, want_stats=False, part_cols=None, y_len=None):
    if y_len is not None:
        _chk_len(y_len, "y_len", xs.data.shape[0] if isinstance(xs, XsTensor) else -1, xs.data if isinstance(xs, XsTensor) else None)
    lib = _lib.load()
    assert isinstance(xs, XsTensor) and isinstance(wt, SplitConvWeight)
    B, C_in, L_in = xs.data.shape[0], xs.C, xs.L
    _chk_split_weight(wt, C_in, C_out, ks)
    if L_out is None:
        L_out = L_in
    if out is None:
        out = torch.empty((B, C_out, L_out), device=xs.data.device, dtype=torch.float32)
    _chk(out, "out", 3)
    assert out.shape == (B, C_out, L_out), (out.shape, (B, C_out, L_out))
    d = ConvDesc()
    d.B, d.C_in, d.C_out, d.L_in, d.L_out, d.ks, d.dil, d.pad_left = B, C_in, C_out, L_in, L_out, ks, dil, pad_left
    d.xs, d.xs_cg, d.xs_lp, d.xs_halo = xs.data.data_ptr(), xs.cg, xs.Lp, xs.halo
    d.wq, d.wq_co_pad, d.wq_cin_pad = wt.wq.data_ptr(), wt.co_pad, wt.cin_pad
    d.x_scale, d.out_scale, d.w_row_scale = xs.x_scale, 1.0 / xs.x_scale, wt.row_scale.data_ptr()
    _chk(bias, "bias", 1)
    d.bias = _ptr(bias)
    d.y, d.y_bs, d.y_cs = out.data_ptr(), out.stride(0), out.stride(1)
    d.y_len = _ptr(y_len)
    _fill_epilogue(d, B, C_out, L_out, res, res_shift, res2, div, act, act_split, act_slope)
    part = None
    if want_stats:
        pc = part_cols or lib.st2_conv1d_xs_part_cols(C.byref(d))
        nt = (L_out + pc - 1) // pc
        part = new_part(B, C_out, nt, out.device)
        d.part, d.part_nt, d.part_cols = part.data_ptr(), nt, pc
    _launch_conv(lib.st2_conv1d_xs, "st2_conv1d_xs", d)
    if want_stats:
        return out, stats_finalize(part, B, C_out, nt, L_out, cols=d.part_cols or 128, lengths=y_len, len_div=C_out)
    return out


def _fill_epilogue(d, B, C_out, L_out, res, res_shift, res2, div, act, act_split, act_slope):
    if res is not None:
        _chk(res, "res", 3)
        assert res.shape[0] == B and res.shape[1] == C_out and res.shape[2] == (L_out + (1 << res_shift) - 1 >> res_shift)
        d.res, d.res_bs, d.res_cs, d.res_shift = res.data_ptr(), res.stride(0), res.stride(1), res_shift
    if res2 is not None:
        _chk(res2, "res2", 3)
        assert res2.shape == (B, C_out, L_out)
        d.res2, d.res2_bs, d.res2_cs = res2.data_ptr(), res2.stride(0), res2.stride(1)
    d.div = div
    d.act, d.act_split, d.act_slope = act, act_split, act_slope


def _launch_conv(fn, fname, d):
    _lib.check(fn(C.byref(d), _stream()), fname)


def conv1d(x, wt, C_out, ks, *, dil=1, pad_left=0, L_out=None, bias=None, out=None,
           pro=PRO_NONE, slope=0.0, stats=None, gamma=None, beta=None, gamma_plus_one=False, alpha=None,
           res=None, res_shift=0, res2=None, div=1.0, act=ACT_NONE, act_split=0, act_slope=0.0, want_stats=False,
           gb_seg=0, x_scale=None, x_len=None, y_len=None):
    _chk_len(x_len, "x_len", _nb(x), x)
    _chk_len(y_len, "y_len", _nb(x), x)
    lib = _lib.load()
    _chk(x, "x", 3)
    B, C_in, L_in = x.shape
    split = isinstance(wt, SplitConvWeight)
    if (split and pad_left <= XS_HALO and L_in >= XS_MIN_L and (pro != PRO_NONE or C_in >= XS_MIN_C_PLAIN)
            and conv_path() == "xs" and not prefer_fused(pro, C_in, ks)):
        xs = activate(x, pro=pro, slope=slope, stats=stats, gamma=gamma, beta=beta,
                      gamma_plus_one=gamma_plus_one, alpha=alpha, gb_seg=gb_seg, x_scale=x_scale, lengths=x_len)
        return conv1d_xs(xs, wt, C_out, ks, dil=dil, pad_left=pad_left, L_out=L_out, bias=bias, out=out, res=res,
                         res_shift=res_shift, res2=res2, div=div, act=act, act_split=act_split, act_slope=act_slope,
                         want_stats=want_stats, y_len=y_len)
    if gb_seg:
        raise _lib.St2Error("gb_seg (per-segment affine of a token-merged view) exists on the st2_act_split + "
                            "st2_conv1d_xs path only; this call routes to the fused kernel")
    if split:
        _chk_split_weight(wt, C_in, C_out, ks)
    else:
        _chk(wt, "wt", 2)
        if wt.shape[0] != C_in * ks or not wt.is_contiguous():
            raise _lib.St2Error("packed weight has shape %s, expected [%d, >=%d]" % (tuple(wt.shape), C_in * ks,
                                                                                      C_out))
    if L_out is None:
        L_out = L_in
    if out is None:
        out = torch.empty((B, C_out, L_out), device=x.device, dtype=torch.float32)
    _chk(out, "out", 3)
    assert out.shape == (B, C_out, L_out), (out.shape, (B, C_out, L_out))
    d = ConvDesc()
    d.B, d.C_in, d.C_out, d.L_in, d.L_out, d.ks, d.dil, d.pad_left = B, C_in, C_out, L_in, L_out, ks, dil, pad_left
    d.x, d.x_bs, d.x_cs = x.data_ptr(), x.stride(0), x.stride(1)
    if split:
        d.wq, d.wq_co_pad, d.wq_cin_pad = wt.wq.data_ptr(), wt.co_pad, wt.cin_pad
        d.x_scale = float(x_scale) if x_scale else x_scale_for(pro)
        d.out_scale, d.w_row_scale = 1.0 / d.x_scale, wt.row_scale.data_ptr()
        fn, fname = lib.st2_conv1d_f16s, "st2_conv1d_f16s"
    else:
        d.wt, d.w_ld = wt.data_ptr(), wt.shape[1]
        fn, fname = lib.st2_conv1d, "st2_conv1d"
    _chk(bias, "bias", 1)
    d.bias = _ptr(bias)
    d.y, d.y_bs, d.y_cs = out.data_ptr(), out.stride(0), out.stride(1)
    d.x_len, d.y_len = _ptr(x_len), _ptr(y_len)
    d.pro, d.slope = pro, slope
    gbs = _chk_prologue(pro, B, C_in, L_in, stats, gamma, beta, alpha, 0)
    if pro in _PRO_NORM:
        d.stats, d.gamma, d.beta, d.gb_bs = stats.data_ptr(), gamma.data_ptr(), beta.data_ptr(), gbs
        d.gamma_plus_one = 1 if gamma_plus_one else 0
    if pro in _PRO_SNAKE:
        d.alpha = alpha.data_ptr()
    _fill_epilogue(d, B, C_out, L_out, res, res_shift, res2, div, act, act_split, act_slope)
    ws = part = None
    if split and want_stats:
        nt = (L_out + 127) // 128
        part = new_part(B, C_out, nt, out.device)
        d.part, d.part_nt = part.data_ptr(), nt
    elif split:
        nb = lib.st2_conv1d_f16s_splitk_bytes(C.byref(d))
        if nb > 0:
            ws = torch.empty((nb,), device=x.device, dtype=torch.uint8)
            d.splitk_ws, d.splitk_ws_bytes = ws.data_ptr(), nb
    _launch_conv(fn, fname, d)
    if want_stats:
        if part is not None:
            return out, stats_finalize(part, B, C_out, nt, L_out, lengths=y_len, len_div=C_out)
        return out, instnorm_stats(out, lengths=y_len)
    return out


def conv1d_direct(x, w, bias, stride, pad, L_out=None, out=None, x_len=None, y_len=None):
    xlp = _chk_len(x_len, "x_len", _nb(x), x)
    ylp = _chk_len(y_len, "y_len", _nb(x), x)
    lib = _lib.load()
    _chk(x, "x", 3)
    _chk(w, "w", 3)
    _chk(bias, "bias", 1)
    assert w.is_contiguous()
    B, C_in, L_in = x.shape
    C_out, C_in_w, ks = w.shape
    assert C_in_w == C_in
    if L_out is None:
        L_out = (L_in + 2 * pad - ks) // stride + 1
    if out is None:
        out = torch.empty((B, C_out, L_out), device=x.device, dtype=torch.float32)
    _chk(out, "out", 3)
    _lib.check(lib.st2_conv1d_direct_len(x.data_ptr(), x.stride(0), x.stride(1), w.data_ptr(), _ptr(bias), out.data_ptr(),
                                         out.stride(0), out.stride(1), B, C_in, C_out, L_in, L_out, ks, stride, pad,
                                         xlp, ylp, _stream()), "st2_conv1d_direct_len")
    return out


def phase_split(x, stride, pad, Lu):
    lib = _lib.load()
    _chk(x, "x", 3)
    B, Cc, L = x.shape
    xp = torch.empty((B, Cc * stride, Lu), device=x.device, dtype=torch.float32)
    _lib.check(lib.st2_phase_split(x.data_ptr(), x.stride(0), x.stride(1), B, Cc, L, stride, pad, xp.data_ptr(),
                                   xp.stride(0), xp.stride(1), Lu, _stream()), "st2_phase_split")
    return xp


def instnorm_stats(x, eps=1e-5, out=None, lengths=None):
    lp = _chk_len(lengths, "lengths", _nb(x), x)
    lib = _lib.load()
    _chk(x, "x", 3)
    B, Cc, L = x.shape
    if out is None:
        out = torch.empty((B, Cc, 2), device=x.device, dtype=torch.float32)
    _lib.check(lib.st2_instnorm_stats_len(x.data_ptr(), x.stride(0), x.stride(1), B, Cc, L, eps, out.data_ptr(), lp,
                                          _stream()), "st2_instnorm_stats_len")
    return out


def colnorm_stats(x, eps=1e-5, out=None):
    lib = _lib.load()
    _chk(x, "x", 3)
    B, Cc, L = x.shape
    if out is None:
        out = torch.empty((B, L, 2), device=x.device, dtype=torch.float32)
    _lib.check(lib.st2_colnorm_stats(x.data_ptr(), x.stride(0), x.stride(1), B, Cc, L, eps, out.data_ptr(),
                                     _stream()), "st2_colnorm_stats")
    return out


def style_fc(s, wt, bias, act=ACT_NONE, out=None):
    lib = _lib.load()
    _chk(s, "s", 2)
    _chk(wt, "wt", 2)
    _chk(bias, "bias", 1)
    assert s.is_contiguous() and wt.is_contiguous()
    B, K = s.shape
    assert wt.shape[0] == K
    J = wt.shape[1]
    if out is None:
        out = torch.empty((B, J), device=s.device, dtype=torch.float32)
    _lib.check(lib.st2_style_fc(s.data_ptr(), B, K, wt.data_ptr(), _ptr(bias), J, act, out.data_ptr(), _stream()),
               "st2_style_fc")
    return out


CVT_TILE = 1024


def convt_interleave(phases, C_out, stride, pad, L_raw, bias=None, add=None, reflect_left=False, out=None,
                     want_stats=False, q_len=None, out_len=None):
    if (q_len is None) != (out_len is None):
        raise _lib.St2Error("convt_interleave: q_len and out_len go together")
    qlp = _chk_len(q_len, "q_len", _nb(phases), phases)
    olp = _chk_len(out_len, "out_len", _nb(phases), phases)
    lib = _lib.load()
    _chk(phases, "phases", 3)
    _chk(bias, "bias", 1)
    _chk(add, "add", 3)
    B, RC, Lq = phases.shape
    assert RC == stride * C_out
    L_out = L_raw + (1 if reflect_left else 0)
    if out is None:
        out = torch.empty((B, C_out, L_out), device=phases.device, dtype=torch.float32)
    if add is not None:
        assert add.shape == (B, C_out, L_out), (add.shape, (B, C_out, L_out))
    a_bs, a_cs = (add.stride(0), add.stride(1)) if add is not None else (0, 0)
    part, nt = None, 0
    if want_stats:
        nt = (L_out + CVT_TILE - 1) // CVT_TILE
        part = new_part(B, C_out, nt, phases.device)
    _lib.check(lib.st2_convt_interleave_stats_len(phases.data_ptr(), phases.stride(0), phases.stride(1), Lq, _ptr(bias),
                                                  _ptr(add), a_bs, a_cs, out.data_ptr(), out.stride(0), out.stride(1), B,
                                                  C_out, stride, pad, L_raw, 1 if reflect_left else 0, _ptr(part), nt,
                                                  qlp, olp, _stream()), "st2_convt_interleave_stats_len")
    if want_stats:
        return out, stats_finalize(part, B, C_out, nt, L_out, cols=CVT_TILE, lengths=out_len, len_div=C_out)
    return out


def adain_leaky_pool(x, stats, gamma, beta, slope, w, bias, out=None, lengths=None):
    lp = _chk_len(lengths, "lengths", _nb(x), x)
    lib = _lib.load()
    _chk(x, "x", 3)
    _chk(stats, "stats", 3)
    _chk(gamma, "gamma", 2)
    _chk(beta, "beta", 2)
    _chk(w, "w", 2)
    _chk(bias, "bias", 1)
    B, Cc, L = x.shape
    assert w.shape == (Cc, 3) and w.is_contiguous() and gamma.stride(0) == beta.stride(0)
    if out is None:
        out = torch.empty((B, Cc, 2 * L), device=x.device, dtype=torch.float32)
    _lib.check(lib.st2_adain_leaky_pool_len(x.data_ptr(), x.stride(0), x.stride(1), stats.data_ptr(), gamma.data_ptr(),
                                            beta.data_ptr(), gamma.stride(0), slope, w.data_ptr(), _ptr(bias),
                                            out.data_ptr(), out.stride(0), out.stride(1), B, Cc, L, lp, _stream()),
               "st2_adain_leaky_pool_len")
    return out


def har_source(f0, U, noise, lin_w, lin_b, sine_amp=0.1, noise_std=0.003, voiced_threshold=10.0,
               sample_rate=24000.0, f_len=None, out=None):
    lp = _chk_len(f_len, "f_len", _nb(f0, 2), f0)
    lib = _lib.load()
    _chk(f0, "f0", 2)
    _chk(noise, "noise", 3)
    _chk(lin_w, "lin_w")
    _chk(lin_b, "lin_b")
    B, F = f0.shape
    H = noise.shape[2]
    assert f0.is_contiguous() and noise.is_contiguous() and noise.shape == (B, F * U, H)
    assert lin_w.numel() == H and lin_w.is_contiguous()
    scratch = torch.empty((B, H, F), device=f0.device, dtype=torch.float32)
    if out is None:
        out = torch.empty((B, F * U), device=f0.device, dtype=torch.float32)
    _chk(out, "out", 2)
    assert out.shape == (B, F * U) and out.is_contiguous()
    _lib.check(lib.st2_har_source_len(f0.data_ptr(), B, F, U, H, noise.data_ptr(), lin_w.data_ptr(), lin_b.data_ptr(),
                                      sine_amp, noise_std, voiced_threshold, sample_rate, scratch.data_ptr(),
                                      out.data_ptr(), lp, _stream()), "st2_har_source_len")
    return out


def stft_mag_phase(x, n_fft, hop, lengths=None, out=None):
    lp = _chk_len(lengths, "lengths", _nb(x, 2), x)
    lib = _lib.load()
    _chk(x, "x", 2)
    assert x.is_contiguous()
    B, L = x.shape
    M = L // hop + 1
# ... 345 lines not shown
```

Before: 5155.

## Fuse act_split passes sharing one input into a multi-set kernel

Adds a multi-set act_split kernel that reads the input activation once and writes 2-3 prologue-transformed hi/lo f16 plane sets with different gamma/beta/alpha. The decoder MRF resblock heads and the diffusion sampler's q/kv convs now use it instead of separate act_split launches. This cuts repeated input reads and kernel launches. The noise branch also computes instance-norm stats in the noise conv epilogue so the resblock can take precomputed stats. The cost is holding several plane buffers at once, which raises peak workspace.

```diff
diff --git a/include/st2.h b/include/st2.h
--- a/include/st2.h
+++ b/include/st2.h
@@ -83,6 +83,15 @@
                       int32_t pro, float slope, const float* stats, const float* gamma, const float* beta, int64_t gb_bs,
                       int32_t gb_seg, int32_t gamma_plus_one, const float* alpha, float x_scale,
                       void* xs, int32_t xs_cg, int32_t Lp, int32_t halo, const int32_t* len, void* stream);
+typedef struct st2_act_set {
+  const float* gamma; const float* beta; const float* alpha;
+  float x_scale;
+  void* xs;
+} st2_act_set;
+int st2_act_split_multi(const float* x, int64_t x_bs, int32_t x_cs, int32_t B, int32_t C, int32_t L,
+                        int32_t pro, float slope, const float* stats, int64_t gb_bs, int32_t gb_seg, int32_t gamma_plus_one,
+                        int32_t xs_cg, int32_t Lp, int32_t halo, const int32_t* len, int32_t n, const st2_act_set* sets,
+                        void* stream);
 int st2_conv1d_xs_part_cols(const st2_conv_desc* d);
 int st2_stats_finalize(const float* part, int32_t rows, int32_t nt, int32_t L, float eps, float* stats, int32_t cols, void* stream);
 int st2_stats_finalize_len(const float* part, int32_t rows, int32_t nt, int32_t L, float eps, float* stats, int32_t cols,
diff --git a/styletts2_amd/_lib.py b/styletts2_amd/_lib.py
--- a/styletts2_amd/_lib.py
+++ b/styletts2_amd/_lib.py
@@ -75,6 +75,10 @@
 class DecoderTaps(C.Structure):
     _fields_ = [("encode", f32p), ("front", f32p), ("har_source", f32p), ("har", f32p), ("stage", f32p * 4),
                 ("spec_phase", f32p)]
+
+
+class ActSet(C.Structure):
+    _fields_ = [("gamma", f32p), ("beta", f32p), ("alpha", f32p), ("x_scale", C.c_float), ("xs", C.c_void_p)]
 
 
 SAMPLER_TABLE_COLS = 11
@@ -196,6 +200,9 @@
     "st2_act_split_len": (C.c_int, [f32p, C.c_int64, C.c_int32, C.c_int32, C.c_int32, C.c_int32, C.c_int32, C.c_float,
                                     f32p, f32p, f32p, C.c_int64, C.c_int32, C.c_int32, f32p, C.c_float, f32p, C.c_int32,
                                     C.c_int32, C.c_int32, C.c_void_p, C.c_void_p]),
+    "st2_act_split_multi": (C.c_int, [f32p, C.c_int64, C.c_int32, C.c_int32, C.c_int32, C.c_int32, C.c_int32, C.c_float,
+                                      f32p, C.c_int64, C.c_int32, C.c_int32, C.c_int32, C.c_int32, C.c_int32, C.c_void_p,
+                                      C.c_int32, C.POINTER(ActSet), C.c_void_p]),
     "st2_stats_finalize_len": (C.c_int, [f32p, C.c_int32, C.c_int32, C.c_int32, C.c_float, f32p, C.c_int32, C.c_void_p,
                                          C.c_int32, C.c_void_p]),
     "st2_instnorm_stats_len": (C.c_int, [f32p, C.c_int64, C.c_int32, C.c_int32, C.c_int32, C.c_int32, C.c_float, f32p,
diff --git a/styletts2_amd/csrc/st2_actsplit.hip b/styletts2_amd/csrc/st2_actsplit.hip
--- a/styletts2_amd/csrc/st2_actsplit.hip
+++ b/styletts2_amd/csrc/st2_actsplit.hip
@@ -22,18 +22,8 @@
 #ifndef ST2_ACT_NT
 #define ST2_ACT_NT 3
 #endif
-template <int PRO>
-__global__ __launch_bounds__(256) void act_split_kernel(const ActArgs a) {
-  const int pos = blockIdx.x * 256 + threadIdx.x;
-  if (pos >= a.Lp) return;
-  const int cg = blockIdx.y;
-  const int b = blockIdx.z;
-  const int l = pos - a.halo;
-  const int Lb = a.len ? min(a.len[b], a.L) : a.L;
-  const bool lok = l >= 0 && l < Lb;
-  const int lc = min(max(l, 0), a.L - 1);
+static __device__ __forceinline__ void act_load_slot(const ActArgs& a, int b, int cg, int lc, float (&v)[8]) {
   const float* xb = a.x + (int64_t)b * a.x_bs + lc;
-  float v[8];
 #pragma unroll
   for (int e = 0; e < 8; ++e) {
     const int ci = min(cg * 8 + e, a.C - 1);
@@ -43,12 +33,11 @@
     v[e] = xb[(int64_t)ci * a.x_cs];
 #endif
   }
-  float cmean = 0.f, crstd = 1.f;
-  if constexpr (PRO == ST2_PRO_COLNORM) {
-    const float* st = a.stats + ((int64_t)b * a.L + lc) * 2;
-    cmean = st[0];
-    crstd = st[1];
-  }
+}
+
+template <int PRO>
+static __device__ __forceinline__ bool act_split_store_slot(const ActArgs& a, const float (&v)[8], int b, int cg, int pos, int lc,
+                                                            bool lok, float cmean, float crstd) {
   st2_h8 hi, lo;
   bool sat = false;
 #pragma unroll
@@ -88,7 +77,6 @@
     hi[e] = h;
     lo[e] = (_Float16)(uc - (float)h);
   }
-  if (__any(sat) && (threadIdx.x & 63) == 0) st2_raise_status(a.status, ST2_STATUS_F16_RANGE);
   const int64_t plane = (int64_t)a.xs_cg * a.Lp;
   st2_h8* dst = a.xs + ((int64_t)b * 2 * a.xs_cg + cg) * a.Lp + pos;
 #if ST2_ACT_NT & 2
@@ -98,6 +86,69 @@
   dst[0] = hi;
   dst[plane] = lo;
 #endif
+  return sat;
+}
+
+template <int PRO>
+__global__ __launch_bounds__(256) void act_split_kernel(const ActArgs a) {
+  const int pos = blockIdx.x * 256 + threadIdx.x;
+  if (pos >= a.Lp) return;
+  const int cg = blockIdx.y;
+  const int b = blockIdx.z;
+  const int l = pos - a.halo;
+  const int Lb = a.len ? min(a.len[b], a.L) : a.L;
+  const bool lok = l >= 0 && l < Lb;
+  const int lc = min(max(l, 0), a.L - 1);
+  float v[8];
+  act_load_slot(a, b, cg, lc, v);
+  float cmean = 0.f, crstd = 1.f;
+  if constexpr (PRO == ST2_PRO_COLNORM) {
+    const float* st = a.stats + ((int64_t)b * a.L + lc) * 2;
+    cmean = st[0];
+    crstd = st[1];
+  }
+  const bool sat = act_split_store_slot<PRO>(a, v, b, cg, pos, lc, lok, cmean, crstd);
+  if (__any(sat) && (threadIdx.x & 63) == 0) st2_raise_status(a.status, ST2_STATUS_F16_RANGE);
+}
+
+struct ActSetDev {
+  const float* gamma; const float* beta; const float* alpha;
+  float x_scale;
+  st2_h8* xs;
+};
+template <int N>
+struct ActArgsMulti {
+  ActArgs a;
+  ActSetDev set[N];
+};
+
+template <int PRO, int N>
+__global__ __launch_bounds__(256) void act_split_multi_kernel(const ActArgsMulti<N> m) {
+  const ActArgs& a = m.a;
+  const int pos = blockIdx.x * 256 + threadIdx.x;
+  if (pos >= a.Lp) return;
+  const int cg = blockIdx.y;
+  const int b = blockIdx.z;
+  const int l = pos - a.halo;
+  const int Lb = a.len ? min(a.len[b], a.L) : a.L;
+  const bool lok = l >= 0 && l < Lb;
+  const int lc = min(max(l, 0), a.L - 1);
+  float v[8];
+  act_load_slot(a, b, cg, lc, v);
+  float cmean = 0.f, crstd = 1.f;
+  if constexpr (PRO == ST2_PRO_COLNORM) {
+    const float* st = a.stats + ((int64_t)b * a.L + lc) * 2;
+    cmean = st[0];
+    crstd = st[1];
+  }
+  bool sat = false;
+#pragma unroll
+  for (int i = 0; i < N; ++i) {
+    ActArgs s = a;
+    s.gamma = m.set[i].gamma; s.beta = m.set[i].beta; s.alpha = m.set[i].alpha; s.x_scale = m.set[i].x_scale; s.xs = m.set[i].xs;
+    sat |= act_split_store_slot<PRO>(s, v, b, cg, pos, lc, lok, cmean, crstd);
+  }
+  if (__any(sat) && (threadIdx.x & 63) == 0) st2_raise_status(a.status, ST2_STATUS_F16_RANGE);
 }
 
 __global__ __launch_bounds__(256) void stats_finalize_kernel(const float* __restrict__ part, int rows, int nt, int L_max,
@@ -209,7 +260,18 @@
   hipLaunchKernelGGL((act_split_kernel<PRO>), dim3(st2_cdiv(a.Lp, 256), a.xs_cg, B), dim3(256), 0, s, a);
 }
 
-}
+template <int PRO, int N>
+void launch_act_multi(const ActArgs& a, const st2_act_set* sets, int B, hipStream_t s) {
+  ActArgsMulti<N> m;
+  m.a = a;
+  for (int i = 0; i < N; ++i)
+    m.set[i] = {sets[i].gamma, sets[i].beta, sets[i].alpha, sets[i].x_scale, reinterpret_cast<st2_h8*>(sets[i].xs)};
+  hipLaunchKernelGGL((act_split_multi_kernel<PRO, N>), dim3(st2_cdiv(a.Lp, 256), a.xs_cg, B), dim3(256), 0, s, m);
+}
+
+}
+
+bool st2_headroom_active() { return g_headroom; }
 
 extern "C" int st2_act_split(const float* x, int64_t x_bs, int32_t x_cs, int32_t B, int32_t C, int32_t L, int32_t pro,
                              float slope, const float* stats, const float* gamma, const float* beta, int64_t gb_bs,
@@ -259,6 +321,54 @@
   return 0;
 }
 
+extern "C" int st2_act_split_multi(const float* x, int64_t x_bs, int32_t x_cs, int32_t B, int32_t C, int32_t L, int32_t pro,
+                                   float slope, const float* stats, int64_t gb_bs, int32_t gb_seg, int32_t gamma_plus_one,
+                                   int32_t xs_cg, int32_t Lp, int32_t halo, const int32_t* len, int32_t n,
+                                   const st2_act_set* sets, void* stream) {
+  ST2_REQUIRE(x && sets && B > 0 && C > 0 && L > 0, "st2_act_split_multi: bad arguments");
+  ST2_REQUIRE(B <= 65535 && xs_cg <= 65535, "st2_act_split_multi: grid too large");
+  ST2_REQUIRE(xs_cg * 8 >= C, "st2_act_split_multi: xs_cg=%d groups cannot hold C=%d channels", xs_cg, C);
+  ST2_REQUIRE(halo >= 0 && Lp >= L + halo, "st2_act_split_multi: Lp=%d too small for L=%d + halo=%d", Lp, L, halo);
+  ST2_REQUIRE((pro == ST2_PRO_ADAIN_SNAKE && (n == 2 || n == 3)) || (pro == ST2_PRO_COLNORM && n == 2),
+              "st2_act_split_multi: prologue %d with %d plane sets is not built (ADAIN_SNAKE: 2 or 3, COLNORM: 2)", pro, n);
+  ST2_REQUIRE(stats, "st2_act_split_multi: prologue %d needs stats", pro);
+  ST2_REQUIRE(gb_seg >= 0 && (gb_seg == 0 || pro == ST2_PRO_COLNORM), "st2_act_split_multi: gb_seg=%d is for ST2_PRO_COLNORM", gb_seg);
+  ST2_REQUIRE(!len || pro != ST2_PRO_COLNORM, "st2_act_split_multi: per-row lengths are not defined for ST2_PRO_COLNORM");
+  const int64_t set_bytes = (int64_t)B * 2 * xs_cg * Lp * 16;
+  for (int i = 0; i < n; ++i) {
+    ST2_REQUIRE(sets[i].gamma && sets[i].beta && sets[i].xs, "st2_act_split_multi: set %d needs gamma / beta / xs", i);
+    ST2_REQUIRE(pro != ST2_PRO_ADAIN_SNAKE || sets[i].alpha, "st2_act_split_multi: set %d: snake needs alpha", i);
+    ST2_REQUIRE(sets[i].x_scale > 0.f, "st2_act_split_multi: set %d: x_scale must be set", i);
+    ST2_REQUIRE((reinterpret_cast<uintptr_t>(sets[i].xs) & 15) == 0, "st2_act_split_multi: set %d: xs must be 16-byte aligned", i);
+    for (int j = 0; j < i; ++j) {
+      const char* pi = static_cast<const char*>(sets[i].xs);
+      const char* pj = static_cast<const char*>(sets[j].xs);
+      ST2_REQUIRE(pi + set_bytes <= pj || pj + set_bytes <= pi, "st2_act_split_multi: plane sets %d and %d overlap", j, i);
+    }
+  }
+  ActArgs a;
+  a.x = x; a.x_bs = x_bs; a.x_cs = x_cs; a.C = C; a.L = L; a.slope = slope;
+  a.stats = stats; a.gamma = nullptr; a.beta = nullptr; a.gb_bs = gb_bs; a.gb_seg = gb_seg; a.gamma_plus_one = gamma_plus_one;
+  a.alpha = nullptr; a.x_scale = 0.f;
+  a.xs = nullptr; a.xs_cg = xs_cg; a.Lp = Lp; a.halo = halo;
+  a.len = len;
+  a.status = st2_status_device_ptr();
+  hipStream_t s = reinterpret_cast<hipStream_t>(stream);
+  if (pro == ST2_PRO_COLNORM) launch_act_multi<ST2_PRO_COLNORM, 2>(a, sets, B, s);
+  else if (n == 2) launch_act_multi<ST2_PRO_ADAIN_SNAKE, 2>(a, sets, B, s);
+  else launch_act_multi<ST2_PRO_ADAIN_SNAKE, 3>(a, sets, B, s);
+  ST2_CHECK_LAUNCH("st2_act_split_multi");
+  if (g_headroom) {
+    for (int i = 0; i < n; ++i) {
+      ActArgs r = a;
+      r.x_scale = sets[i].x_scale; r.xs = reinterpret_cast<st2_h8*>(sets[i].xs);
+      headroom_record(0, r, B, s);
+      if (!g_hr.empty()) g_hr.back().pro = pro;
+    }
+  }
+  return 0;
+}
+
 int st2_headroom_of_fused_conv(const st2_conv_desc& d, hipStream_t s) {
   if (!g_headroom || !d.x) return 0;
   {
diff --git a/styletts2_amd/csrc/st2_common.h b/styletts2_amd/csrc/st2_common.h
--- a/styletts2_amd/csrc/st2_common.h
+++ b/styletts2_amd/csrc/st2_common.h
@@ -7,6 +7,7 @@
 void st2_set_error(const char* fmt, ...);
 int st2_stream_cu_count(void* stream);
 void st2_headroom_set_site(const void* engine, int site);
+bool st2_headroom_active();
 int* st2_status_device_ptr();
 
 __device__ __forceinline__ void st2_raise_status(int* status, int bit) {
diff --git a/styletts2_amd/csrc/st2_engine.hip b/styletts2_amd/csrc/st2_engine.hip
--- a/styletts2_amd/csrc/st2_engine.hip
+++ b/styletts2_amd/csrc/st2_engine.hip
@@ -757,12 +757,61 @@
     RUN(c, g_be.instnorm_stats(x.p, x.bs, x.cs, x.B, x.C, x.L, 1e-5f, stats, c.stream));
 }
 
-void conv(Ctx& c, const st2_engine& e, const View& x, const SplitW& w, const View& y, const ConvOpt& o) {
+bool conv_takes_xs(const View& x, const SplitW& w, const ConvOpt& o) {
+  const bool prefer_fused = o.pro != ST2_PRO_NONE && (x.C <= FUSED_MAX_C || (w.ks <= 3 && x.C <= FUSED_K3_MAX_C));
+  return o.pad_left <= XS_HALO && x.L >= XS_MIN_L && (o.pro != ST2_PRO_NONE || x.C >= XS_MIN_C_PLAIN) && !prefer_fused;
+}
+
+struct XsPlanes {
+  void* xs = nullptr;
+  int cg = 0, Lp = 0;
+  float x_scale = 0.f;
+};
+
+float conv_x_scale(const st2_engine& e, const SplitW& w, const ConvOpt& o) { return e.x_scale(w.site, x_scale_for(o.pro)); }
+
+XsPlanes alloc_planes(Ctx& c, const st2_engine& e, const View& x, const SplitW& w, const ConvOpt& o) {
+  XsPlanes pl;
+  pl.cg = (x.C + 31) / 32 * 32 / 8;
+  pl.Lp = xs_row_slots(x.L);
+  pl.x_scale = conv_x_scale(e, w, o);
+  pl.xs = c.a.alloc((int64_t)x.B * 2 * pl.cg * pl.Lp * 16);
+  return pl;
+}
+
+XsPlanes make_planes(Ctx& c, const st2_engine& e, const View& x, const SplitW& w, const ConvOpt& o) {
+  const XsPlanes pl = alloc_planes(c, e, x, w, o);
+  if (!c.dry) st2_headroom_set_site(&e, w.site);
+  if (x.len)
+    RUN(c, g_be.act_split_len(x.p, x.bs, x.cs, x.B, x.C, x.L, o.pro, o.slope, o.stats, o.gamma, o.beta, o.gb_bs, o.gb_seg,
+                              o.gamma_plus_one, o.alpha, pl.x_scale, pl.xs, pl.cg, pl.Lp, XS_HALO, x.len, c.stream));
+  else
+    RUN(c, g_be.act_split(x.p, x.bs, x.cs, x.B, x.C, x.L, o.pro, o.slope, o.stats, o.gamma, o.beta, o.gb_bs, o.gb_seg,
+                          o.gamma_plus_one, o.alpha, pl.x_scale, pl.xs, pl.cg, pl.Lp, XS_HALO, c.stream));
+  if (!c.dry) st2_headroom_set_site(nullptr, -1);
+  return pl;
+}
+
+bool g_multi_native = true;
+bool multi_split_ok(const Ctx& c) { return c.dry || (g_multi_native && !st2_headroom_active()); }
+
+void make_planes_multi(Ctx& c, const st2_engine& e, const View& x, int n, const SplitW* const* w, const ConvOpt* o,
+                       XsPlanes* pl) {
+  st2_act_set sets[3];
+  for (int i = 0; i < n; ++i) {
+    pl[i] = alloc_planes(c, e, x, *w[i], o[i]);
+    sets[i] = {o[i].gamma, o[i].beta, o[i].alpha, pl[i].x_scale, pl[i].xs};
+  }
+  RUN(c, st2_act_split_multi(x.p, x.bs, x.cs, x.B, x.C, x.L, o[0].pro, o[0].slope, o[0].stats, o[0].gb_bs, o[0].gb_seg,
+                             o[0].gamma_plus_one, pl[0].cg, pl[0].Lp, XS_HALO, x.len, n, sets, c.stream));
+}
+
+void conv_run(Ctx& c, const st2_engine& e, const View& x, const SplitW& w, const View& y, const ConvOpt& o, const XsPlanes* pl) {
   st2_conv_desc d;
   memset(&d, 0, sizeof(d));
   d.B = x.B; d.C_in = x.C; d.C_out = y.C; d.L_in = x.L; d.L_out = y.L; d.ks = w.ks; d.dil = o.dil; d.pad_left = o.pad_left;
   d.wq = e.P<const void>(w.wq); d.wq_co_pad = w.co_pad; d.wq_cin_pad = w.cin_pad;
-  d.x_scale = e.x_scale(w.site, x_scale_for(o.pro));
+  d.x_scale = pl ? pl->x_scale : conv_x_scale(e, w, o);
   d.out_scale = 1.0f / d.x_scale;
   if (!c.dry) st2_headroom_set_site(&e, w.site);
   d.w_row_scale = e.F(w.row_scale);
@@ -773,25 +822,8 @@
   d.div = o.div;
   d.act = o.act; d.act_split = o.act_split; d.act_slope = o.act_slope;
   d.x_len = x.len; d.y_len = y.len;
-  if (w.C_in != x.C || w.C_out != y.C) {
-    if (c.rc == 0) { st2_set_error("engine: conv weight is %d->%d, call has %d->%d", w.C_in, w.C_out, x.C, y.C); c.rc = 1; }
-    return;
-  }
-  const bool prefer_fused = o.pro != ST2_PRO_NONE && (x.C <= FUSED_MAX_C || (w.ks <= 3 && x.C <= FUSED_K3_MAX_C));
-  const bool use_xs = o.pad_left <= XS_HALO && x.L >= XS_MIN_L && (o.pro != ST2_PRO_NONE || x.C >= XS_MIN_C_PLAIN) &&
-                      !prefer_fused;
-  const int64_t mark = c.a.off;
-  if (use_xs) {
-    const int cg = (x.C + 31) / 32 * 32 / 8;
-    const int Lp = xs_row_slots(x.L);
-    void* xs = c.a.alloc((int64_t)x.B * 2 * cg * Lp * 16);
-    if (x.len)
-      RUN(c, g_be.act_split_len(x.p, x.bs, x.cs, x.B, x.C, x.L, o.pro, o.slope, o.stats, o.gamma, o.beta, o.gb_bs, o.gb_seg,
-                                o.gamma_plus_one, o.alpha, d.x_scale, xs, cg, Lp, XS_HALO, x.len, c.stream));
-    else
-      RUN(c, g_be.act_split(x.p, x.bs, x.cs, x.B, x.C, x.L, o.pro, o.slope, o.stats, o.gamma, o.beta, o.gb_bs, o.gb_seg,
-                            o.gamma_plus_one, o.alpha, d.x_scale, xs, cg, Lp, XS_HALO, c.stream));
-    d.xs = xs; d.xs_cg = cg; d.xs_lp = Lp; d.xs_halo = XS_HALO;
+  if (pl) {
+    d.xs = pl->xs; d.xs_cg = pl->cg; d.xs_lp = pl->Lp; d.xs_halo = XS_HALO;
     float* part = nullptr;
     int nt = 0;
     if (o.stats_out) {
@@ -803,10 +835,6 @@
     RUN(c, g_be.conv1d_xs(&d, c.stream));
     if (o.stats_out) finalize_stats(c, part, y, nt, o.stats_out, d.part_cols);
   } else {
-    if (o.gb_seg > 0) {
-      if (c.rc == 0) { st2_set_error("engine: a per-segment affine (gb_seg) needs the act_split + xs path"); c.rc = 1; }
-      return;
-    }
     d.x = x.p; d.x_bs = x.bs; d.x_cs = x.cs;
     d.pro = o.pro; d.slope = o.slope;
     d.stats = o.stats; d.gamma = o.gamma; d.beta = o.beta; d.gb_bs = o.gb_bs; d.gamma_plus_one = o.gamma_plus_one;
@@ -827,8 +855,29 @@
     RUN(c, g_be.conv1d_f16s(&d, c.stream));
     if (o.stats_out) finalize_stats(c, part, y, nt, o.stats_out, 128);
   }
+  if (!c.dry) st2_headroom_set_site(nullptr, -1);
+}
+
+void conv(Ctx& c, const st2_engine& e, const View& x, const SplitW& w, const View& y, const ConvOpt& o,
+          const XsPlanes* given = nullptr) {
+  if (w.C_in != x.C || w.C_out != y.C) {
+    if (c.rc == 0) { st2_set_error("engine: conv weight is %d->%d, call has %d->%d", w.C_in, w.C_out, x.C, y.C); c.rc = 1; }
+    return;
+  }
+  const int64_t mark = c.a.off;
+  if (given) {
+    conv_run(c, e, x, w, y, o, given);
+  } else if (conv_takes_xs(x, w, o)) {
+    const XsPlanes pl = make_planes(c, e, x, w, o);
+    conv_run(c, e, x, w, y, o, &pl);
+  } else {
+    if (o.gb_seg > 0) {
+      if (c.rc == 0) { st2_set_error("engine: a per-segment affine (gb_seg) needs the act_split + xs path"); c.rc = 1; }
+      return;
+    }
+    conv_run(c, e, x, w, y, o, nullptr);
+  }
   c.a.off = mark;
-  if (!c.dry) st2_headroom_set_site(nullptr, -1);
 }
 
 float* new_stats(Ctx& c, int B, int C) { return c.a.f32((int64_t)B * C * 2); }
@@ -848,12 +897,14 @@
 extern "C" int st2_debug_set_backend(void* const* table, int32_t entries) {
   if (!table) {
     g_be = kHipBackend;
+    g_multi_native = true;
     return 0;
   }
   ST2_REQUIRE(entries == ST2_BACKEND_ENTRIES || entries == ST2_BACKEND_ENTRIES_V22,
               "st2_debug_set_backend: %d entries, expected %d (or %d: the slots before ABI v23)", entries,
               (int)ST2_BACKEND_ENTRIES, (int)ST2_BACKEND_ENTRIES_V22);
   for (int i = 0; i < entries; ++i) ST2_REQUIRE(table[i] != nullptr, "st2_debug_set_backend: entry %d is null", i);
+  g_multi_native = false;
 #define SLOT(field, slot) g_be.field = reinterpret_cast<decltype(g_be.field)>(table[slot])
   SLOT(conv1d_f16s, ST2_BE_CONV1D_F16S); SLOT(conv1d_xs, ST2_BE_CONV1D_XS); SLOT(act_split, ST2_BE_ACT_SPLIT);
   SLOT(stats_finalize, ST2_BE_STATS_FINALIZE); SLOT(conv1d_direct, ST2_BE_CONV1D_DIRECT);
diff --git a/styletts2_amd/csrc/st2_plan_decoder.inc b/styletts2_amd/csrc/st2_plan_decoder.inc
--- a/styletts2_amd/csrc/st2_plan_decoder.inc
+++ b/styletts2_amd/csrc/st2_plan_decoder.inc
@@ -10,8 +10,17 @@
   const float* beta(int off, int channels) const { return h + off + channels; }
 };
 
+ConvOpt resblock1_head_opt(const DecRun& r, const PResBlock1& p, const float* x_stats) {
+  const int d = p.dil[0];
+  ConvOpt o;
+  o.dil = d; o.pad_left = (p.ks * d - d) / 2; o.pro = ST2_PRO_ADAIN_SNAKE;
+  o.stats = x_stats; o.gamma = r.gamma(p.ad1[0]); o.beta = r.beta(p.ad1[0], p.channels); o.gb_bs = r.J;
+  o.alpha = r.e.F(p.a1[0]);
+  return o;
+}
+
 View run_resblock1(DecRun& r, const PResBlock1& p, View x, const float* x_stats, View mrf_acc, bool mrf_last, int n_mrf,
-                   View out) {
+                   View out, const XsPlanes* head = nullptr) {
   Ctx& c = r.c;
   const int C = p.channels, ks = p.ks, B = x.B, L = x.L;
   const float* st = x_stats;
@@ -30,7 +39,7 @@
     o1.dil = d; o1.pad_left = (ks * d - d) / 2; o1.bias = r.e.F(p.c1[i].bias); o1.pro = ST2_PRO_ADAIN_SNAKE;
     o1.stats = st; o1.gamma = r.gamma(p.ad1[i]); o1.beta = r.beta(p.ad1[i], C); o1.gb_bs = r.J;
     o1.alpha = r.e.F(p.a1[i]); o1.stats_out = st2;
-    conv(c, r.e, x, p.c1[i].w, xt, o1);
+    conv(c, r.e, x, p.c1[i].w, xt, o1, i == 0 ? head : nullptr);
     const bool last = i == 2;
     ConvOpt o2;
     o2.dil = 1; o2.pad_left = (ks - 1) / 2; o2.bias = r.e.F(p.c2[i].bias); o2.pro = ST2_PRO_ADAIN_SNAKE;
@@ -252,8 +261,9 @@
       const int64_t m = c.a.off;
       View xs0 = new_ncl(c, B, C, L_out).with_len(len_o);
       const int stride_f0 = g.noise_stride[i];
+      float* st_src = new_stats(c, B, C);
       ConvOpt o;
-      o.bias = e.F(g.noise_b[i]);
+      o.bias = e.F(g.noise_b[i]); o.stats_out = st_src;
       if (stride_f0 > 1) {
         const int pad_f0 = (stride_f0 + 1) / 2;
         const int L_ns = (har.L + 2 * pad_f0 - 2 * stride_f0) / stride_f0 + 1;
@@ -266,7 +276,7 @@
         conv(c, e, har, g.noise_wt[i], xs0, o);
       }
       View nul;
-      run_resblock1(r, g.noise_res[i], xs0, nullptr, nul, false, nk, xs_src);
+      run_resblock1(r, g.noise_res[i], xs0, st_src, nul, false, nk, xs_src);
       c.a.off = m;
     }
     View xu = new_ncl(c, B, C, L_out).with_len(len_o);
@@ -291,12 +301,36 @@
       c.a.off = m;
     }
     View acc[2] = {new_ncl(c, B, C, L_out).with_len(len_o), new_ncl(c, B, C, L_out).with_len(len_o)};
+    constexpr int MAX_NK = 8;
+    XsPlanes head[MAX_NK];
+    bool has_head[MAX_NK] = {};
+    if (multi_split_ok(c)) {
+      int idx[MAX_NK], n = 0;
+      for (int j = 0; j < nk && j < MAX_NK; ++j) {
+        const PResBlock1& p = g.resblocks[(size_t)i * nk + j];
+        if (conv_takes_xs(xu, p.c1[0].w, resblock1_head_opt(r, p, st))) idx[n++] = j;
+      }
+      for (int k0 = 0; n - k0 >= 2; k0 += 3) {
+        const int m = std::min(n - k0, 3);
+        const SplitW* w[3];
+        ConvOpt o[3];
+        XsPlanes pl[3];
+        for (int k = 0; k < m; ++k) {
+          const PResBlock1& p = g.resblocks[(size_t)i * nk + idx[k0 + k]];
+          w[k] = &p.c1[0].w;
+          o[k] = resblock1_head_opt(r, p, st);
+        }
+        make_planes_multi(c, e, xu, m, w, o, pl);
+        for (int k = 0; k < m; ++k) { head[idx[k0 + k]] = pl[k]; has_head[idx[k0 + k]] = true; }
+      }
+    }
     View prev;
     for (int j = 0; j < nk; ++j) {
       const int64_t m = c.a.off;
       const bool lastk = j + 1 == nk;
       View out = lastk ? x_next : acc[j & 1];
-      run_resblock1(r, g.resblocks[(size_t)i * nk + j], xu, st, prev, lastk, nk, out);
+      run_resblock1(r, g.resblocks[(size_t)i * nk + j], xu, st, prev, lastk, nk, out,
+                    (j < MAX_NK && has_head[j]) ? &head[j] : nullptr);
       prev = out;
       c.a.off = m;
     }
diff --git a/styletts2_amd/csrc/st2_plan_sampler.inc b/styletts2_amd/csrc/st2_plan_sampler.inc
--- a/styletts2_amd/csrc/st2_plan_sampler.inc
+++ b/styletts2_amd/csrc/st2_plan_sampler.inc
@@ -81,8 +81,19 @@
     if (seg) o1.gb_seg = o2.gb_seg = N;
     const bool per_utt = cfg.multispeaker && !seg;
     View Xv = per_utt ? X : dn_cv(s, X), qv = per_utt ? qkv : dn_cv(s, qkv);
-    conv(c, e, Xv, b.q, qv.rows(0, mid), o1);
-    conv(c, e, Xv, b.kv, qv.rows(mid, 3 * mid), o2);
+    if (multi_split_ok(c) && conv_takes_xs(Xv, b.q, o1) && conv_takes_xs(Xv, b.kv, o2)) {
+      const int64_t pm = c.a.off;
+      const SplitW* w[2] = {&b.q, &b.kv};
+      const ConvOpt o[2] = {o1, o2};
+      XsPlanes pl[2];
+      make_planes_multi(c, e, Xv, 2, w, o, pl);
+      conv(c, e, Xv, b.q, qv.rows(0, mid), o1, &pl[0]);
+      conv(c, e, Xv, b.kv, qv.rows(mid, 3 * mid), o2, &pl[1]);
+      c.a.off = pm;
+    } else {
+      conv(c, e, Xv, b.q, qv.rows(0, mid), o1);
+      conv(c, e, Xv, b.kv, qv.rows(mid, 3 * mid), o2);
+    }
     View att = dn_alloc(s, mid);
     View q = qkv.rows(0, mid), k = qkv.rows(mid, 2 * mid), v = qkv.rows(2 * mid, 3 * mid);
     RUN(c, g_be.attention_keylen(q.p, k.p, v.p, q.bs, q.cs, att.p, att.bs, att.cs, B, cfg.dn_heads, cfg.dn_head_features,
diff --git a/styletts2_amd/decoder.py b/styletts2_amd/decoder.py
--- a/styletts2_amd/decoder.py
+++ b/styletts2_amd/decoder.py
@@ -206,10 +206,11 @@
                 pad_f0 = (stride_f0 + 1) // 2
                 L_ns = (har.shape[2] + 2 * pad_f0 - 2 * stride_f0) // stride_f0 + 1
                 harp = ops.phase_split(har, stride_f0, pad_f0, L_ns + 1)
-                xs = ops.conv1d(harp, pk.noise_wt[i], C, 2, pad_left=0, L_out=L_ns, bias=pk.noise_b[i])
+                xs, st_src = ops.conv1d(harp, pk.noise_wt[i], C, 2, pad_left=0, L_out=L_ns, bias=pk.noise_b[i],
+                                        want_stats=True)
             else:
-                xs = ops.conv1d(har, pk.noise_wt[i], C, 1, bias=pk.noise_b[i])
-            xs = run_resblock1(pk.noise_res[i], bank, h, xs)
+                xs, st_src = ops.conv1d(har, pk.noise_wt[i], C, 1, bias=pk.noise_b[i], want_stats=True)
+            xs = run_resblock1(pk.noise_res[i], bank, h, xs, x_stats=st_src)
             L_in = x.shape[2]
             if ist:
                 pad, L_raw = (k - u) // 2, (L_in - 1) * u - 2 * ((k - u) // 2) + k
diff --git a/styletts2_amd/ops.py b/styletts2_amd/ops.py
--- a/styletts2_amd/ops.py
+++ b/styletts2_amd/ops.py
@@ -310,6 +310,32 @@
                                      _ptr(gamma), _ptr(beta), gbs, int(gb_seg), 1 if gamma_plus_one else 0, _ptr(alpha),
                                      xsc, data.data_ptr(), cg, Lp, XS_HALO, lp, _stream()), "st2_act_split_len")
     return XsTensor(data, Cc, L, XS_HALO, xsc)
+
+
+def act_split_multi(x, sets, *, pro, stats, slope=0.0, gamma_plus_one=False, c_pad=32, gb_seg=0, lengths=None):
+    lp = _chk_len(lengths, "lengths", _nb(x), x)
+    lib = _lib.load()
+    _chk(x, "x", 3)
+    B, Cc, L = x.shape
+    cg = (Cc + c_pad - 1) // c_pad * c_pad // 8
+    Lp = xs_row_slots(L)
+    n = len(sets)
+    arr = (_lib.ActSet * max(n, 1))()
+    outs, gbs = [], None
+    for i, st in enumerate(sets):
+        g = _chk_prologue(pro, B, Cc, L, stats, st["gamma"], st["beta"], st.get("alpha"), gb_seg)
+        if gbs is not None and g != gbs:
+            raise _lib.St2Error("act_split_multi: the sets' gamma / beta must share one batch stride (%d vs %d)" % (gbs, g))
+        gbs = g
+        xsc = float(st.get("x_scale") or x_scale_for(pro))
+        data = torch.empty((B, 2, cg, Lp, 8), device=x.device, dtype=torch.float16)
+        arr[i].gamma, arr[i].beta, arr[i].alpha = _ptr(st["gamma"]), _ptr(st["beta"]), _ptr(st.get("alpha"))
+        arr[i].x_scale, arr[i].xs = xsc, data.data_ptr()
+        outs.append(XsTensor(data, Cc, L, XS_HALO, xsc))
+    _lib.check(lib.st2_act_split_multi(x.data_ptr(), x.stride(0), x.stride(1), B, Cc, L, pro, slope, _ptr(stats), gbs or 0,
+                                       int(gb_seg), 1 if gamma_plus_one else 0, cg, Lp, XS_HALO, lp, n, arr, _stream()),
+               "st2_act_split_multi")
+    return outs
 
 
 def new_part(B, C, nt, device):
```

Result: no change. 5176 (median of 6 runs) (+0.4%).
